# adajel/KNP-EMI-DG

Hardware: AMD Instinct MI355X
Metric: DoF-updates/sec per PDE timestep (higher is better)
Workload: dtype f64; 1 GPU; 3D idealized 4-axon mesh r=2 (995328 tets, 11943936 P1-DG DoFs: phi + K,Cl solved, Na eliminated), HH membranes + stimulus, full splitting step; parallelism=slab1

## Files before the change

### include/knpemi_hip.h

```cpp
#ifndef KNPEMI_HIP_H
#define KNPEMI_HIP_H
#include <stddef.h>
#include <stdint.h>

#ifdef __cplusplus
extern "C" {
#endif

typedef struct knp_ctx knp_ctx;

enum knp_field {
    KNP_F_PHI = 0,
    KNP_F_C = 1,
    KNP_F_C_PREV = 2,
    KNP_F_C_ELIM = 3,
    KNP_F_PHI_M = 4,
    KNP_F_I_CH = 5,
    KNP_F_E = 6,
    KNP_F_KAPPA = 7,
    KNP_F_DNPHI = 8,
    KNP_F_B_EMI = 9,
    KNP_F_B_KNP = 10,
    KNP_F_X = 11,
    KNP_F_Y = 12,
    KNP_F_FACET_TMP = 13,
    KNP_F_COUNT = 14
};

int knp_ctx_create(knp_ctx** out, int device, int dim, int degree, int n_ions,
                   int64_t nv, int64_t nc, int64_t nc_owned, int64_t nf,
                   const double* coords, const int32_t* cells, const uint32_t* cell_tags,
                   const int32_t* facet_cells, const int8_t* facet_local, const uint32_t* facet_tags,
                   int n_membrane_tags, const uint32_t* membrane_tags);
void knp_ctx_destroy(knp_ctx* ctx);
const char* knp_last_error(knp_ctx* ctx);

int knp_set_params(knp_ctx* ctx, double C_M, double dt, double F, double R, double T, double C_phi,
                   double tau_emi, double tau_knp, const double* z, const double* D, const double* rho,
                   const double* fsrc, int splitting);

int knp_set_geometry_classes(knp_ctx* ctx, int ncls, const uint16_t* cls, const double* table);

int knp_set_mms(knp_ctx* ctx, const double* C, const double* extra_emi, const double* extra_knp);

int knp_set_source(knp_ctx* ctx, const double* src);

enum knp_tab_slot {
    KNP_TAB_CELL_STIFF = 0,
    KNP_TAB_CELL_RHS_EMI = 1,
    KNP_TAB_CELL_MASS = 2,
    KNP_TAB_FACET_EMI = 3,
    KNP_TAB_FACET_MEM = 4,
    KNP_TAB_FACET_KNP = 5,
    KNP_TAB_FACET_RHS_EMI = 6,
    KNP_TAB_FACET_MEM_LIN = 7,
    KNP_TAB_FACET_MEM_KNP = 8,
    KNP_TAB_FACET_AVG = 9,
    KNP_TAB_FACET_NERNST = 10
};
int knp_set_tabulation(knp_ctx* ctx, int slot, int nloc, int nq, const double* w, const double* B, const double* dB);

int64_t knp_field_size(knp_ctx* ctx, int field);
int knp_upload(knp_ctx* ctx, int field, const double* src, int64_t offset, int64_t count);
int knp_download(knp_ctx* ctx, int field, double* dst, int64_t offset, int64_t count);
int knp_copy_field(knp_ctx* ctx, int dst_field, int src_field);

enum knp_debug_table_id {
    KNP_DT_CELLS = 0,
    KNP_DT_NBR = 1,
    KNP_DT_FLAG = 2,
    KNP_DT_CFACET = 3,
    KNP_DT_MF = 4,
    KNP_DT_HB_SRC = 5,
    KNP_DT_HB_LOC = 6,
    KNP_DT_META = 7
};
int64_t knp_debug_table_size(knp_ctx* ctx, int which);
int knp_debug_table(knp_ctx* ctx, int which, void* out, int64_t nbytes);

int knp_update_kappa(knp_ctx* ctx);
int knp_update_dnphi(knp_ctx* ctx);

int knp_emi_apply(knp_ctx* ctx, int fx, int fy);
int knp_knp_apply(knp_ctx* ctx, int fx, int fy);

int knp_emi_rhs(knp_ctx* ctx);
int knp_knp_rhs(knp_ctx* ctx);

int knp_emi_residual_target(knp_ctx* ctx, double r_abs);
int knp_knp_early_stop(knp_ctx* ctx, double factor);
int knp_knp_load_measure(knp_ctx* ctx, double* out);
int knp_emi_solve(knp_ctx* ctx, double rtol, double atol, int maxit, int check_every, int* niter, double* res);
int knp_knp_solve(knp_ctx* ctx, double rtol, double atol, int maxit, int min_it, int check_every, int* niter, double* res);
int knp_set_knp_krylov(knp_ctx* ctx, int method, int restart);
int knp_set_emi_dg_smoother(knp_ctx* ctx, int chebyshev);

int knp_amg_begin(knp_ctx* ctx, int which, int64_t ncg, const int32_t* dg2cg, const int32_t* cg_ptr, const int32_t* cg_idx);
int knp_amg_columns(knp_ctx* ctx, int which, int ncol);
int knp_amg_level(knp_ctx* ctx, int which, int64_t n, const int32_t* rowptrA, const int32_t* colA, const double* valA,
                  const double* dinv, double rho, int cheb_degree, double cheb_lower, int64_t ncoarse,
                  const int32_t* rowptrP, const int32_t* colP, const double* valP,
                  const int32_t* rowptrR, const int32_t* colR, const double* valR);
int knp_amg_finish(knp_ctx* ctx, int which, int64_t n, const double* pinv);
int knp_amg_finish_f32(knp_ctx* ctx, int which, int64_t n, const float* pinv);
int knp_amg_clear(knp_ctx* ctx, int which);
int knp_amg_interface(knp_ctx* ctx, int64_t n_local, int npeers, const int32_t* peers, const int64_t* counts, const int32_t* idx,
                      int64_t nuniq, const int32_t* uvtx, const int32_t* aptr, const int32_t* asrc);
int knp_amg_dist0(knp_ctx* ctx, int which);

int knp_step_updates(knp_ctx* ctx);
int knp_nernst(knp_ctx* ctx);
int knp_picard_updates(knp_ctx* ctx);
int knp_max_abs_diff(knp_ctx* ctx, int field_a, int field_b, double* out);
#define KNP_FACET_TMP_SLOTS 4
int knp_facet_trace(knp_ctx* ctx, int field, int species, int side, int slot);

int knp_rec_create(knp_ctx* ctx, int64_t capacity, int64_t n_points, const int32_t* point_cell, const double* point_w,
                   int64_t n_sets, const int64_t* set_ptr, const int32_t* set_facet, const double* set_w,
                   int n_regions, const uint8_t* region, const double* vol);
int knp_rec_sample(knp_ctx* ctx, double t);
int knp_rec_read(knp_ctx* ctx, int64_t* n_rows, double* t_out, double* rows_out);
int64_t knp_rec_channels(knp_ctx* ctx);
int knp_rec_add_states(knp_ctx* ctx, int64_t n_channels, const int64_t* chan_ptr, const int32_t* entry_handle, const int64_t* entry_row,
                       const int32_t* entry_col, const double* entry_w);
int knp_rec_add_map(knp_ctx* ctx, int64_t n, const int32_t* facets, double threshold, double repolarisation);
int knp_rec_map_arm(knp_ctx* ctx, double t0);
int knp_rec_map_read(knp_ctx* ctx, int64_t n, double* t_act, double* t_repol, double* peak, double* t_peak, int32_t* n_up);
int knp_rec_destroy(knp_ctx* ctx);
// ... 10 lines not shown
int64_t knp_state_describe(knp_ctx* ctx, knp_state_block* out, int64_t cap, int64_t* bytes);
int knp_state_save(knp_ctx* ctx, void* host_buf, size_t bytes);
int knp_state_load(knp_ctx* ctx, const void* host_buf, size_t bytes);
int knp_state_timing(knp_ctx* ctx, float* pack_ms, float* copy_ms);

int knp_ode_create(knp_ctx* ctx, int model, int64_t n, const int32_t* facets, int ns, int np, const double* states,
                   const double* params);
int knp_ode_table(knp_ctx* ctx, int handle, int what, int upload, double* host);
int knp_ode_exchange(knp_ctx* ctx, int handle, int what, int col, int field, int64_t offset, int to_facet);
int knp_ode_exchange_multi(knp_ctx* ctx, int handle, int n, const int32_t* what, const int32_t* col, const int32_t* field,
                           const int64_t* offset, int to_facet);
int knp_ode_set_stimulus(knp_ctx* ctx, int handle, int n_entries, const int32_t* cols, const double* values, const uint8_t* mask);
int knp_ode_step(knp_ctx* ctx, int handle, double t0, double dt, double rtol, double atol);
int knp_ode_rtc_compile(const char* src, const char* name, void** code, size_t* size, char* log, size_t logcap);
void knp_ode_rtc_free(void* code);
int knp_ode_register(knp_ctx* ctx, const void* code, size_t size, const char* kernel_name, int ns, int np);

int knp_host_spgemm(int64_t n, int64_t m, const int32_t* Ap, const int32_t* Aj, const double* Ax, const int32_t* Bp, const int32_t* Bj,
                    const double* Bx, int32_t* Cp, int32_t** Cj, double** Cx, int nthreads);
int knp_host_spmv(int64_t n, const int32_t* Ap, const int32_t* Aj, const double* Ax, const double* x, double* y, int nthreads);
void knp_host_free(void* p);
int knp_host_cell_gram(int64_t nc, int dim, const double* coords, const int32_t* cells, double* vol, double* G, int nthreads);
int knp_host_segment_sum(int64_t nseg, const int64_t* starts, const int64_t* order, const double* src, double* out, int nthreads);
int64_t knp_host_build_facets(int64_t nc, int nv, const int32_t* cells, int32_t* cell_facets, int32_t* facets, int32_t* facet_cells,
                              int8_t* facet_local);
int64_t knp_host_geometry_classes(int64_t nc, const double* coords, const int32_t* cells, const int32_t* nbr, const int8_t* nbj, double quantum,
                                  int64_t max_classes, int32_t* cls, int64_t* first, int nthreads);
int knp_host_block_pattern(int64_t nc, int nd, int64_t n, const int32_t* dof, int64_t* order, int64_t* starts, int32_t* cols, int32_t* indptr,
                           int64_t* nseg, int nthreads);
int knp_host_sym_to_f32(int64_t n, const double* a, float* out, double* maxabs, int nthreads);
int64_t knp_host_mis2_aggregate(int64_t n, const int32_t* indptr, const int32_t* indices, const double* key, int64_t* agg, int nthreads);
int knp_host_morton_order(int64_t n, int d, const double* pts, const int32_t* conn, int nv, const double* scale, int64_t* order, int nthreads);
int knp_host_cell_extent_median(int64_t nc, int nv, int d, const double* coords, const int32_t* cells, double* out);
int knp_host_cell_neighbours(int64_t nc, int nv, const int32_t* cell_facets, const int32_t* facet_cells, const int8_t* facet_local, int32_t* nb,
                             int8_t* nj, int nthreads);
int knp_host_box_marks(int64_t n, int d, const double* coords, const int32_t* conn, int nv, const double* a, const double* b, double eps, int mode,
                       uint8_t* out, int nthreads);
int knp_host_strength(int64_t n, const int32_t* Ap, const int32_t* Aj, const double* Ax, const double* diag, double theta, int32_t* Sp, int32_t** Sj,
                      int nthreads);
int knp_host_smooth_prolongator(int64_t n, int64_t m, const int32_t* Ap, const int32_t* Aj, const double* Ax, const double* v, const int32_t* Pp,
                                const int32_t* Pj, const double* Px, int32_t* Cp, int32_t** Cj, double** Cx, int nthreads);
int knp_host_truncate_prolongator(int64_t n, const int32_t* Pp, const int32_t* Pj, const double* Px, double trunc, const double* Bc, int32_t* Tp,
                                  int32_t** Tj, double** Tx, int nthreads);

int knp_sync(knp_ctx* ctx);
int knp_timer_begin(knp_ctx* ctx);
int knp_timer_end(knp_ctx* ctx, float* ms);
int knp_bench_apply(knp_ctx* ctx, int which, int reps, float* avg_ms);
int knp_apply_timing(knp_ctx* ctx, int enable);
int knp_apply_timing_read(knp_ctx* ctx, int which, float* avg_ms, int* count);

int knp_apply_variant(knp_ctx* ctx, int which);

int knp_probe_facet_contraction(knp_ctx* ctx, int variant, int64_t ncol, int reps, const double* in, double* out, float* avg_ms);

int knp_comm_unique_id(char* out128);
int knp_comm_init(knp_ctx* ctx, int rank, int nranks, const char* id128);
int knp_comm_init_halo(knp_ctx* ctx, const char* id128);
int knp_comm_init_shm(knp_ctx* ctx, int rank, int nranks, const char* name, int64_t red_doubles, int64_t out_doubles);
int knp_set_interior(knp_ctx* ctx, int64_t n_interior);
int knp_halo_tables(knp_ctx* ctx, int npeers, const int32_t* peers, const int64_t* send_counts,
                    const int32_t* send_cells, const int64_t* recv_offsets, const int64_t* recv_counts);
int knp_halo_exchange(knp_ctx* ctx, int field);
int knp_allreduce_sum(knp_ctx* ctx, double* values, int n);

#ifdef __cplusplus
}
#endif
#endif
```

### knp-emi-dg_amd/csrc/abi.hip

```cpp
#include "../../include/knpemi_hip.h"
#include "knpemi_internal.hpp"
#include <chrono>
#include <thread>
#include <cstdio>
#include <cstdlib>
#include "krylov.hpp"
#include <cstring>
#include <unordered_map>
#include <algorithm>
#include <cmath>

namespace {

struct Fields {
    double* f[KNP_F_COUNT] = {nullptr};
    int64_t n[KNP_F_COUNT] = {0};
    bjreal *binv_emi = nullptr, *binv_knp = nullptr;
    double *r = nullptr, *z = nullptr, *p = nullptr, *w = nullptr, *rhat = nullptr, *v = nullptr, *y = nullptr;
    double *hist_emi = nullptr, *hist_knp = nullptr;
    int bj_age_emi = 0, bj_age_knp = 0;
    double* tmp_knp = nullptr;
    double bj_lmax_knp = 0.0;
    int bj_lmax_age = 0;
    int it_ref_knp = 0, it_ref_emi = 0;
// ... 252 lines not shown
    stamp("mesh tables on the device");
    if (dim == 3 && degree == 1 && nc_owned > 0 && nc < (int64_t(1) << 29)) {
        const int64_t B = KNP_HALO_BLK, nblk = (nc_owned + B - 1) / B;
        std::vector<int32_t> hcnt(nblk, 0);
        std::vector<std::vector<int32_t>> lists((size_t)nblk);
        std::vector<uint16_t> hloc((size_t)nc_owned * 4, 0);
        int hmax = 0;
        for (int64_t b = 0; b < nblk; ++b) {
            auto& L = lists[(size_t)b];
            for (int64_t k = b * B; k < std::min(nc_owned, (b + 1) * B); ++k)
                for (int a = 0; a < 4; ++a) {
                    const uint32_t kind = (fb[k * 4 + a] >> 2) & 3u;
                    const int64_t nbk = nbr[k * 4 + a];
                    if ((kind != FK_SIPG && kind != FK_MEMBRANE) || nbk < 0) continue;
                    if (nbk / B == b) { hloc[k * 4 + a] = (uint16_t)(nbk - b * B); continue; }
                    hloc[k * 4 + a] = (uint16_t)(B + L.size());
                    L.push_back((int32_t)(nbk * 4 + (fb[k * 4 + a] & 3u)));
                }
            hmax = std::max(hmax, (int)L.size());
        }
        int64_t long0 = nblk;
        for (int64_t b = 0; b < nblk; ++b)
            if ((int64_t)lists[(size_t)b].size() > B) { long0 = b; break; }
        hmax = 0;
        for (int64_t b = 0; b < long0; ++b) hmax = std::max(hmax, (int)lists[(size_t)b].size());
        const int hs = ((hmax + 7) / 8) * 8;
        if (hs > 0 && long0 > 0) {
            std::vector<int32_t> hsrc((size_t)nblk * hs, -1);
            for (int64_t b = 0; b < long0; ++b) std::copy(lists[(size_t)b].begin(), lists[(size_t)b].end(), hsrc.begin() + b * hs);
            rc |= dev_alloc_copy(c, &m.hb_src, hsrc.data(), hsrc.size());
            rc |= dev_alloc_copy(c, &m.hb_loc, hloc.data(), hloc.size());
            rc |= dev_zeros(c, &c->halo_ctr, KNP_HALO_CTR_INTS);
            m.hb_stride = hs;
            m.hb_long0 = long0;
        }
    }
    if (rc) { g_err = c->err; delete c; return -2; }
    stamp("halo lists");

    Fields* fl = new Fields();
    const int64_t ndof = nc * ND, ns = c->p.n_sys;
    const int64_t sizes[KNP_F_COUNT] = {ndof, ns * ndof, ns * ndof, ndof, nf, n_ions * nf, n_ions * nf, ndof, ndof,
                                        ndof, ns * ndof, ns * ndof, ns * ndof, (int64_t)KNP_FACET_TMP_SLOTS * nf};
    for (int i = 0; i < KNP_F_COUNT; ++i) {
        fl->n[i] = sizes[i];
        rc |= dev_zeros(c, &fl->f[i], sizes[i]);
    }
    rc |= dev_zeros(c, &fl->binv_emi, ndof * ND);
    rc |= dev_zeros(c, &fl->binv_knp, ns * ndof * ND);
    double** wk[] = {&fl->r, &fl->z, &fl->p, &fl->w, &fl->rhat, &fl->v, &fl->y};
    for (auto pp : wk) rc |= dev_zeros(c, pp, ns * ndof);
    rc |= dev_zeros(c, &c->D, (size_t)n_ions * nc);
    rc |= dev_zeros(c, &c->rho, nc);
    c->partial_blocks = grid_for(nc_owned) + 8;
    rc |= dev_zeros(c, &c->partial, (size_t)c->partial_blocks * KNP_MAX_SYS * KNP_MAX_RED);
    rc |= dev_zeros(c, &c->scal, KNP_SCAL_DOUBLES);
    if (!rc && hipMalloc((void**)&c->status, sizeof(int) * KNP_STATUS_WORDS) != hipSuccess) rc = -2;
    if (!rc) hipMemset(c->status, 0, sizeof(int) * KNP_STATUS_WORDS);
    if (!rc && hipHostMalloc(&c->pinned, 4096) != hipSuccess) rc = -2;
    if (rc) { g_err = "device allocation failed: " + c->err; delete fl; delete c; return -2; }
    if (dev_alloc_copy(c, &fl->ivol, ivol.data(), ivol.size())) { g_err = "device allocation failed: " + c->err; delete fl; delete c; return -2; }
    g_fields[c] = fl;
    *out = c;
    stamp("fields allocated");
    return 0;
}

void knp_ctx_destroy(knp_ctx* c) {
    if (!c) return;
    hipSetDevice(c->device);
    hipDeviceSynchronize();
    for (auto& H : c->amg) amg_free(H);
    for (auto st : c->aux_streams) hipStreamDestroy(st);
    for (auto ev : c->aux_events) hipEventDestroy(ev);
    if (c->fork_event) hipEventDestroy(c->fork_event);
    ode_destroy_all(c);
    rec_destroy(c);
    state_destroy(c);
    tab_free(c);
    Fields* fl = g_fields[c];
    if (fl) {
        for (int i = 0; i < KNP_F_COUNT; ++i) hipFree(fl->f[i]);
        hipFree(fl->binv_emi); hipFree(fl->binv_knp); hipFree(fl->bj_idx); hipFree(fl->bj_tab); hipFree(fl->ivol);
        double* wk[] = {fl->r, fl->z, fl->p, fl->w, fl->rhat, fl->v, fl->y, fl->hist_emi, fl->hist_knp, fl->tmp_knp, fl->tmp_emi};
        for (auto p : wk) hipFree(p);
        delete fl;
        g_fields.erase(c);
    }
    ring_u_free(c);
    hipFree(c->m.hb_src); hipFree(c->m.hb_loc);
    hipFree(c->m.cls); hipFree(c->m.cls_table); hipFree(c->m.cls_ext); hipFree(c->m.coords); hipFree(c->m.h); hipFree(c->m.cells); hipFree(c->m.nbr); hipFree(c->m.fflag); hipFree(c->m.cfacet); hipFree(c->m.mf);
    hipFree(c->mat); hipFree(c->nmat4); hipFree(c->dtab); hipFree(c->halo_ctr);
    hipFree(c->D); hipFree(c->rho); hipFree(c->fsrc); hipFree(c->mms_C); hipFree(c->extra_emi); hipFree(c->extra_knp); hipFree(c->partial); hipFree(c->scal); hipFree(c->status); hipFree(c->gm_V);
    hipFree(c->halo_send_idx); hipFree(c->halo_sendbuf);
    if (c->pinned) hipHostFree(c->pinned);
    if (c->ev0) hipEventDestroy(c->ev0);
    if (c->ev1) hipEventDestroy(c->ev1);

    for (int w = 0; w < 2; ++w)
        for (auto& pr : c->tev[w]) { hipEventDestroy(pr.first); hipEventDestroy(pr.second); }
    comm_destroy(c);
    if (c->stream) hipStreamDestroy(c->stream);
    delete c;
}

int knp_set_params(knp_ctx* c, double C_M, double dt, double Fc, double R, double T, double C_phi, double tau_emi,
                   double tau_knp, const double* z, const double* D, const double* rho, const double* fsrc, int splitting) {
    if (!c || !z || !D) return -1;
    Params& p = c->p;
    p.C_M = C_M; p.dt = dt; p.F = Fc; p.R = R; p.T = T; p.C_phi = C_phi; p.psi = Fc / (R * T);
    p.tau_emi = tau_emi; p.tau_knp = tau_knp; p.splitting = splitting;
    if (splitting == 2 && !c->mms_C) { c->err = "MMS mode needs knp_set_mms first"; return -1; }
    if (g_fields.count(c)) reset_lagged(F(c));
    for (int i = 0; i < p.n_ions; ++i) {
        p.z[i] = z[i];
        if (z[i] == 0.0) { c->err = "ion valence z must be non-zero"; return -1; }
    }
    if (!(dt > 0.0)) { c->err = "dt must be positive"; return -1; }
    HIPCHK(c, hipMemcpy(c->D, D, sizeof(double) * p.n_ions * c->m.nc, hipMemcpyHostToDevice));
    if (g_fields.count(c)) F(c)->bj_tab_state = 0;
    {
        const int64_t nc = c->m.nc;
        const int ni = p.n_ions;
        c->h_mat.assign((size_t)nc, 0);
        std::vector<double> seen;
        bool ok = true;
        for (int64_t k = 0; k < nc && ok; ++k) {
            const int nm = (int)(seen.size() / ni);
            int id = -1;
            for (int q = nm - 1; q >= 0 && id < 0; --q) {
                bool same = true;
                for (int i = 0; i < ni && same; ++i) same = seen[(size_t)q * ni + i] == D[(int64_t)i * nc + k];
                if (same) id = q;
            }
            if (id < 0) {
                if (nm >= 256) { ok = false; break; }
                for (int i = 0; i < ni; ++i) seen.push_back(D[(int64_t)i * nc + k]);
                id = nm;
            }
            c->h_mat[(size_t)k] = (uint16_t)id;
        }
        if (!ok) c->h_mat.clear();
    }
    c->nmat = 0;
    if (c->m.dim == 3 && c->degree == 1 && c->m.hb_stride) {
        const int64_t nc = c->m.nc;
// ... 90 lines not shown
    c->m.ncls = ncls;
    return 0;
}

int knp_set_source(knp_ctx* c, const double* src) {
    if (!c) return -1;
    if (c->p.splitting == 2) { c->err = "knp_set_source: the manufactured-solution mode sets its own data terms"; return -1; }
    const int64_t n = (int64_t)c->p.n_sys * c->m.nc * c->nd;
    if (!src) {
        hipFree(c->extra_knp);
        c->extra_knp = nullptr;
        return 0;
    }
    if (!c->extra_knp) HIPCHK(c, hipMalloc((void**)&c->extra_knp, sizeof(double) * n));
    HIPCHK(c, hipMemcpy(c->extra_knp, src, sizeof(double) * n, hipMemcpyHostToDevice));
    return 0;
}

int knp_set_mms(knp_ctx* c, const double* C, const double* extra_emi, const double* extra_knp) {
    if (!c) return -1;
    const int64_t ndof = c->m.nc * c->nd, ns = c->p.n_sys;
    hipFree(c->mms_C); hipFree(c->extra_emi); hipFree(c->extra_knp);
    c->mms_C = c->extra_emi = c->extra_knp = nullptr;
    if (C) {
        HIPCHK(c, hipMalloc((void**)&c->mms_C, sizeof(double) * ns * c->m.nc));
        HIPCHK(c, hipMemcpy(c->mms_C, C, sizeof(double) * ns * c->m.nc, hipMemcpyHostToDevice));
    }
    if (extra_emi) {
        HIPCHK(c, hipMalloc((void**)&c->extra_emi, sizeof(double) * ndof));
        HIPCHK(c, hipMemcpy(c->extra_emi, extra_emi, sizeof(double) * ndof, hipMemcpyHostToDevice));
    }
    if (extra_knp) {
        HIPCHK(c, hipMalloc((void**)&c->extra_knp, sizeof(double) * ns * ndof));
        HIPCHK(c, hipMemcpy(c->extra_knp, extra_knp, sizeof(double) * ns * ndof, hipMemcpyHostToDevice));
    }
    return 0;
}

int64_t knp_field_size(knp_ctx* c, int field) { return chk_field(c, field) ? -1 : F(c)->n[field]; }

static int64_t debug_table_ptr(knp_ctx* c, int which, const void** p) {
    const MeshDev& m = c->m;
    const int64_t NV = m.dim + 1;
    const int64_t nblk = (m.nc_owned + KNP_HALO_BLK - 1) / KNP_HALO_BLK;
    switch (which) {
        case KNP_DT_CELLS: *p = m.cells; return m.nc * NV * 4;
        case KNP_DT_NBR: *p = m.nbr; return m.nc * NV * 4;
        case KNP_DT_FLAG: *p = m.fflag; return m.nc * 4;
        case KNP_DT_CFACET: *p = m.cfacet; return m.nc * NV * 4;
        case KNP_DT_MF: *p = m.mf; return m.nmf * 6 * 4;
        case KNP_DT_HB_SRC: *p = m.hb_src; return m.hb_src ? nblk * m.hb_stride * 4 : 0;
        case KNP_DT_HB_LOC: *p = m.hb_loc; return m.hb_loc ? m.nc_owned * 4 * 2 : 0;
        case KNP_DT_META: *p = nullptr; return 8 * 8;
        default: return -1;
    }
}
int64_t knp_debug_table_size(knp_ctx* c, int which) {
    const void* p = nullptr;
    return c ? debug_table_ptr(c, which, &p) : -1;
}
int knp_debug_table(knp_ctx* c, int which, void* out, int64_t nbytes) {
    if (!c) return -1;
    const void* p = nullptr;
    const int64_t n = debug_table_ptr(c, which, &p);
    if (n < 0 || nbytes != n || (n && !out)) { c->err = "debug_table: unknown table or size mismatch"; return -1; }
    if (which == KNP_DT_META) {
        const int64_t meta[8] = {c->m.nc, c->m.nc_owned, c->m.nf, c->m.nmf, c->m.hb_stride, c->m.hb_long0, c->m.n_interior, c->m.dim};
        memcpy(out, meta, sizeof(meta));
        return 0;
    }
    if (n) HIPCHK(c, hipMemcpy(out, p, (size_t)n, hipMemcpyDeviceToHost));
    return 0;
}

int knp_upload(knp_ctx* c, int field, const double* src, int64_t offset, int64_t count) {
    if (chk_field(c, field)) return -1;
    if (offset < 0 || count < 0 || offset + count > F(c)->n[field]) { c->err = "upload range out of bounds"; return -1; }
    HIPCHK(c, hipMemcpyAsync(F(c)->f[field] + offset, src, sizeof(double) * count, hipMemcpyHostToDevice, c->stream));
    HIPCHK(c, hipStreamSynchronize(c->stream));
    if (field == KNP_F_C || field == KNP_F_C_ELIM || field == KNP_F_PHI || field == KNP_F_KAPPA) reset_lagged(F(c));
    if (field == KNP_F_PHI) { F(c)->nh_emi = 0; c->last_peclet = -1.0f; }
    if (field == KNP_F_C) F(c)->nh_knp = 0;
    return 0;
}

int knp_download(knp_ctx* c, int field, double* dst, int64_t offset, int64_t count) {
    if (chk_field(c, field)) return -1;
    if (offset < 0 || count < 0 || offset + count > F(c)->n[field]) { c->err = "download range out of bounds"; return -1; }
    HIPCHK(c, hipMemcpyAsync(dst, F(c)->f[field] + offset, sizeof(double) * count, hipMemcpyDeviceToHost, c->stream));
    HIPCHK(c, hipStreamSynchronize(c->stream));
    return 0;
}

int knp_copy_field(knp_ctx* c, int dst, int src) {
    if (chk_field(c, dst) || chk_field(c, src)) return -1;
    if (F(c)->n[dst] != F(c)->n[src]) { c->err = "copy_field: size mismatch"; return -1; }
    HIPCHK(c, hipMemcpyAsync(F(c)->f[dst], F(c)->f[src], sizeof(double) * F(c)->n[src], hipMemcpyDeviceToDevice, c->stream));
    return 0;
}

int knp_update_kappa(knp_ctx* c) {
    if (!c) return -1;
    Fields* f = F(c);
    return launch_kappa(c, f->f[KNP_F_C], f->f[KNP_F_C_ELIM], f->f[KNP_F_KAPPA]);
}

// ... 6 lines not shown
        pe = (float)(scale * (hi - lo));
        if (!(pe >= 0.0f)) pe = 3.0e38f;
    }
#pragma unroll
    for (int off = 32; off > 0; off >>= 1) pe = fmaxf(pe, __shfl_down(pe, off, 64));
    __shared__ float s_pe[4];
    if ((threadIdx.x & 63) == 0) s_pe[threadIdx.x >> 6] = pe;
    __syncthreads();
    if (threadIdx.x == 0) {
        pe = fmaxf(fmaxf(s_pe[0], s_pe[1]), fmaxf(s_pe[2], s_pe[3]));
        const int bits = __float_as_int(pe);
        if (bits > __atomic_load_n(out, __ATOMIC_RELAXED)) atomicMax(out, bits);
    }
}

int knp_update_dnphi(knp_ctx* c) {
    if (!c) return -1;
    Fields* f = F(c);
    double zmax = 0.0;
    for (int i = 0; i < c->p.n_sys; ++i) zmax = std::max(zmax, std::fabs(c->p.z[i]));
    HIPCHK(c, hipMemsetAsync(c->status + KNP_PECLET_SLOT, 0, sizeof(int), c->stream));
    if (c->m.nc_owned)
        hipLaunchKernelGGL(k_cell_peclet, dim3((unsigned)((c->m.nc_owned + 255) / 256)), dim3(256), 0, c->stream, c->m.nc_owned, c->nd,
                           (const double*)f->f[KNP_F_PHI], c->p.psi * zmax, c->status + KNP_PECLET_SLOT);
    HIPCHK(c, hipGetLastError());
    if (c->dist) { int rc = allreduce_max_word(c, c->status + KNP_PECLET_SLOT); if (rc) return rc; }
    return launch_dnphi(c, f->f[KNP_F_PHI], f->f[KNP_F_DNPHI]);
}

int knp_allreduce_sum(knp_ctx* c, double* values, int n) {
    if (!c || !values) return -1;
    return allreduce_sum_host(c, values, n);
}

static int chk_vec(knp_ctx* c, int fx, int fy, int64_t need) {
    if (chk_field(c, fx) || chk_field(c, fy)) return -1;
    if (fx == fy) { c->err = "apply: input and output fields must differ"; return -1; }
    if (F(c)->n[fx] < need || F(c)->n[fy] < need) { c->err = "apply: field too small for this operator"; return -1; }
    return 0;
}

int knp_emi_apply(knp_ctx* c, int fx, int fy) {
    if (!c) return -1;
    if (chk_vec(c, fx, fy, c->m.nc * c->nd)) return -1;
    Fields* f = F(c);
    return dist_apply(c, 0, f->f[fx], f->f[KNP_F_KAPPA], f->f[fy]);
}

int knp_knp_apply(knp_ctx* c, int fx, int fy) {
    if (!c) return -1;
    if (chk_vec(c, fx, fy, (int64_t)c->p.n_sys * c->m.nc * c->nd)) return -1;
    Fields* f = F(c);
    return dist_apply(c, 1, f->f[fx], f->f[KNP_F_DNPHI], f->f[fy]);
}

int knp_emi_rhs(knp_ctx* c) {
    if (!c) return -1;
    Fields* f = F(c);
    return launch_emi_rhs(c, f->f[KNP_F_C], f->f[KNP_F_C_ELIM], f->f[KNP_F_PHI_M], f->f[KNP_F_I_CH], f->f[KNP_F_B_EMI]);
}

int knp_knp_rhs(knp_ctx* c) {
    if (!c) return -1;
    Fields* f = F(c);
    return launch_knp_rhs(c, f->f[KNP_F_C], f->f[KNP_F_C_PREV], f->f[KNP_F_C_ELIM], f->f[KNP_F_PHI], f->f[KNP_F_PHI_M],
                          f->f[KNP_F_I_CH], f->f[KNP_F_B_KNP]);
}

int knp_emi_residual_target(knp_ctx* c, double r_abs) {
    if (!c || !(r_abs >= 0.0)) return -1;
    F(c)->emi_r_abs = r_abs;
    return 0;
}

int knp_knp_early_stop(knp_ctx* c, double factor) {
    if (!c || !(factor >= 0.0) || factor >= 1.0) { if (c) c->err = "knp_knp_early_stop: factor must be in [0, 1)"; return -1; }
    c->knp_early = factor;
    return 0;
}

int knp_knp_load_measure(knp_ctx* c, double* out) {
    if (!c || !out) return -1;
    Fields* f = F(c);
    const bool d8 = env_int("KNP_KNP_NORM2", 0) != 1;
    return load_measure(c, f->f[KNP_F_B_KNP], f->ivol, d8, out);
}

int knp_emi_solve(knp_ctx* c, double rtol, double atol, int maxit, int check_every, int* niter, double* res) {
    if (!c || !niter || !res) return -1;
    Fields* f = F(c);
    static const int bj_lag = env_int("KNP_BJ_LAG", 8);
    int rc = 0;
    if (f->bj_age_emi % (bj_lag > 0 ? bj_lag : 1) == 0) rc = launch_emi_blockjacobi(c, f->f[KNP_F_KAPPA], f->binv_emi);
    ++f->bj_age_emi;
    if (rc) return rc;
    if ((rc = extrapolate_guess(c, f->f[KNP_F_PHI], &f->hist_emi, &f->nh_emi, f->n[KNP_F_PHI], true))) return rc;
    KrylovVecs kv{};
    kv.x = f->f[KNP_F_PHI]; kv.b = f->f[KNP_F_B_EMI]; kv.coef = f->f[KNP_F_KAPPA]; kv.binv = f->binv_emi;
    kv.ivol = f->ivol; kv.r_abs = f->emi_r_abs;
    kv.d8 = env_int("KNP_KNP_NORM2", 0) != 1;
    kv.r = f->r; kv.z = f->z; kv.p = f->p; kv.w = f->w; kv.rhat = f->rhat; kv.v = f->v; kv.y = f->y;
    static const int cheb_env_emi = env_int("KNP_EMI_CHEB", -1);
    const int cheb_emi = cheb_env_emi >= 0 ? cheb_env_emi : (c->emi_dg_cheb >= 0 ? c->emi_dg_cheb : (c->degree == 1 ? 1 : 0));
    if (cheb_emi && c->amg.size() && c->amg[0].ready) {
        if (!f->tmp_emi) HIPCHK(c, hipMalloc((void**)&f->tmp_emi, sizeof(double) * f->n[KNP_F_PHI]));
        kv.tmp = f->tmp_emi;
// ... 357 lines not shown
```

### knp-emi-dg_amd/csrc/apply_p1.hip

```cpp
#include "apply_p1_direct.hpp"
#include "apply_p1_cls.hpp"
#include "apply_p1_halo.hpp"
#include "apply_plan.hpp"

static_assert(APPLY_PLAN_BLK == KNP_HALO_BLK, "the plan counts head cells in blocks of the halo tables");

static inline int64_t grid8(int64_t n) { return ((grid_for(n) + 7) / 8) * 8; }

struct ApplyTimerScope {
    knp_ctx* c; int which; bool on;
    ApplyTimerScope(knp_ctx* ctx, int w) : c(ctx), which(w), on(ctx->time_applies) {
        if (!on) return;
        auto& pool = c->tev[which];
        if (c->tev_used[which] == pool.size()) {
            hipEvent_t a, b;
            if (hipEventCreate(&a) != hipSuccess || hipEventCreate(&b) != hipSuccess) { on = false; return; }
            pool.push_back({a, b});
        }
        hipEventRecord(pool[c->tev_used[which]].first, c->stream);
    }
    ~ApplyTimerScope() {
        if (!on) return;
        hipEventRecord(c->tev[which][c->tev_used[which]].second, c->stream);
        ++c->tev_used[which];
// ... 42 lines not shown
            case AF_RING_U: rc = ring_u_emi_apply(c, m, x, kappa, y, halo_reserve_cus(c)); break;
            case AF_CLS:
                hipLaunchKernelGGL((k_emi_apply_cls_staged<3, 256>), g, dim3(KNP_BLOCK), 0, c->stream, m, x, kappa, y, c->p.C_phi, c->p.tau_emi);
                HIPCHK(c, hipGetLastError());
                break;
            default: DISPATCH_DIM(c, k_emi_apply, g, m, x, kappa, y, c->p.C_phi, c->p.tau_emi);
        }
        if (rc) return rc;
    }
    return 0;
}

int launch_knp_apply(knp_ctx* c, const double* x, const double* gphi, double* y) {
    ApplyTimerScope t(c, 1);
    if (c->degree != 1) return p2_assembled(c) ? tab_apply(c, 1, x, y) : p2_knp_apply(c, x, gphi, y);
    if (c->m.c_end - c->m.c_begin <= 0) return 0;
    const KnpArgs ka = make_knp_args(c);
    size_t halo_lds = 0;
    const ApplyInputs in = apply_inputs(c, 1, &halo_lds);
    ApplySegment seg[2];
    const int nseg = apply_segments(plan_apply(in, 1), c->m.c_begin, c->m.c_end, seg);
    for (int i = 0; i < nseg; ++i) {
        MeshDev m = c->m;
        m.c_begin = seg[i].begin; m.c_end = seg[i].end;
        const dim3 g((unsigned)grid8(m.c_end - m.c_begin)), b(KNP_BLOCK);
        int rc = 0;
        switch (seg[i].family) {
            case AF_RING_KNP: rc = ring_knp_apply(c, m, x, gphi, y, ka, halo_reserve_cus(c)); break;
            case AF_RING_U: rc = ring_u_knp_apply(c, m, x, gphi, y, ka, halo_reserve_cus(c)); break;
            case AF_HALO:
            case AF_HALO_MAT: rc = knp_halo_launch(c, m, x, gphi, y, ka, halo_lds, in.halo_mat, halo_reserve_cus(c)); break;
            case AF_CLS:
                dispatch_nsys<3>(c->p.n_sys, [&](auto ns) {
                    hipLaunchKernelGGL((k_knp_apply_cls_staged<3, decltype(ns)::value, 256>), g, b, 0, c->stream, m, x, gphi, c->D, y, ka);
                    return 0;
                });
                HIPCHK(c, hipGetLastError());
                break;
            default:
                rc = dispatch_nsys<4>(c->p.n_sys, [&](auto ns) {
                    constexpr int NS = decltype(ns)::value;
                    if (c->m.dim == 3) hipLaunchKernelGGL((k_knp_apply<3, NS>), g, b, 0, c->stream, m, x, gphi, c->D, y, ka);
                    else hipLaunchKernelGGL((k_knp_apply<2, NS>), g, b, 0, c->stream, m, x, gphi, c->D, y, ka);
                    return 0;
                });
                if (rc) { c->err = "knp_apply supports 1..4 solved species"; return -1; }
                HIPCHK(c, hipGetLastError());
        }
        if (rc) return rc;
    }
    return 0;
}

int launch_emi_blockjacobi(knp_ctx* c, const double* kappa, bjreal* binv) {
    if (c->degree != 1) return p2_assembled(c) ? tab_block_inverse(c, 0, binv) : p2_block_inverse(c, 0, kappa, binv);
    const double shift = 0.0;
    DISPATCH_DIM(c, k_emi_blockjacobi, dim3((unsigned)grid_for(c->m.nc_owned)), c->m, kappa, binv, c->p.C_phi, c->p.tau_emi, shift);
    return 0;
}

int launch_knp_blockjacobi(knp_ctx* c, const double* gphi, bjreal* binv) {
    if (c->degree != 1) return p2_assembled(c) ? tab_block_inverse(c, 1, binv) : p2_block_inverse(c, 1, gphi, binv);
    const dim3 g((unsigned)grid_for(c->m.nc_owned), (unsigned)c->p.n_sys);
    DISPATCH_DIM(c, k_knp_blockjacobi, g, c->m, gphi, c->D, binv, make_knp_args(c));
    return 0;
}

int launch_neighbour_materials(knp_ctx* c) {
    const int64_t n = c->m.nc * 4;
    hipLaunchKernelGGL(k_neighbour_materials, dim3((unsigned)((n + 255) / 256)), dim3(256), 0, c->stream, c->m.nc, c->m.nbr, c->mat, c->nmat4);
    HIPCHK(c, hipGetLastError());
    HIPCHK(c, hipStreamSynchronize(c->stream));
    return 0;
}

int launch_dnphi(knp_ctx* c, const double* phi, double* gphi) {
    if (c->degree != 1) {
        if (p2_assembled(c)) return tab_assemble_knp(c, phi);
        HIPCHK(c, hipMemcpyAsync(gphi, phi, sizeof(double) * c->m.nc * c->nd, hipMemcpyDeviceToDevice, c->stream));
        return 0;
    }
    DISPATCH_DIM(c, k_gphi, dim3((unsigned)grid_for(c->m.nc)), c->m, phi, gphi);
    return 0;
}
```

### knp-emi-dg_amd/csrc/apply_plan.hpp

```cpp
#pragma once
#include <algorithm>
#include <cstdint>

enum ApplyFamily : int {
    AF_COORD = 0,
    AF_CLS = 1,
    AF_HALO = 2,
    AF_RING_EMI = 3,
    AF_HALO_MAT = 6,
    AF_RING_KNP = 7,
    AF_P2 = 8,
    AF_P2_ASSEMBLED = 9,
    AF_RING_U = 10
};

constexpr int64_t APPLY_PLAN_BLK = 256;
constexpr int64_t APPLY_ALL_CELLS = INT64_MAX;

struct ApplyInputs {
    int degree = 1, dim = 3;
    bool p2_assembled = false;
    bool cls = false;
    int ncls = 0, ncls_max = 0;
    int n_sys = 1;
    int64_t hb_long0 = 0;
    bool ring = false;
    int64_t ring_u_cells = 0;
    bool halo = false, halo_mat = false;
};

struct ApplyPlan { ApplyFamily head; int64_t head_cells; ApplyFamily tail; };

inline ApplyPlan plan_apply(const ApplyInputs& in, int which) {
    if (in.degree != 1) {
        const ApplyFamily f = in.p2_assembled ? AF_P2_ASSEMBLED : AF_P2;
        return {f, APPLY_ALL_CELLS, f};
    }
    const bool classed = in.dim == 3 && in.cls && in.ncls <= in.ncls_max && (which == 0 || in.n_sys <= 3);
    const ApplyFamily tail = classed ? AF_CLS : AF_COORD;
    const int64_t short_list_cells = in.hb_long0 * APPLY_PLAN_BLK;
    if (in.ring) return {which == 1 ? AF_RING_KNP : AF_RING_EMI, short_list_cells, tail};
    if (in.ring_u_cells > 0) return {AF_RING_U, in.ring_u_cells, tail};
    if (which == 1 && in.halo) return {in.halo_mat ? AF_HALO_MAT : AF_HALO, short_list_cells, tail};
    return {tail, APPLY_ALL_CELLS, tail};
}

struct ApplySegment { ApplyFamily family; int64_t begin, end; };

inline int apply_segments(const ApplyPlan& p, int64_t begin, int64_t end, ApplySegment seg[2]) {
    int n = 0;
    if (begin < end && begin < p.head_cells) {
        seg[n++] = {p.head, begin, std::min(end, p.head_cells)};
        begin = seg[0].end;
    }
    if (begin < end) seg[n++] = {p.tail, begin, end};
    return n;
}
```

### knp-emi-dg_amd/csrc/apply_ring.hip

```cpp
#include "cell_geom.hpp"
#include "ring_common.hpp"
#include <algorithm>
#include <cstdlib>
#include <map>

namespace {

using namespace ring;
constexpr int RH = 224;
constexpr int RHX = RH / 32;
constexpr int RENT = RB + RH;
constexpr int RSLOTS = 3;
constexpr int RLISTB = 1024;
constexpr int RNLIST = 4;
constexpr int RLOADERS = 4;
constexpr int META_F = 0, META_L = 1024, META_N = 3072, META_C = 4096, META_M = 5120, META_KNP = 6144, META_EMI = 5120;
constexpr int RCLS = 43;

__device__ __forceinline__ void dma_list(const MeshDev& m, int64_t b, unsigned dst, int lane) {
    const int off = lane * 4 < m.hb_stride ? lane * 4 : 0;
    glds16(m.hb_src + b * m.hb_stride + off, dst);
}
__device__ __forceinline__ void class_gram(const lds_double* rec, CellGeom<3>& K) {
    K.vol = rec[0];
    int q = 1;
#pragma unroll
    for (int a = 0; a < 4; ++a)
#pragma unroll
        for (int b = a; b < 4; ++b) { K.G[a][b] = rec[q]; K.G[b][a] = rec[q]; ++q; }
}

template <int NS> struct KnpRing {
    static constexpr int XB = RENT * 32;
    static constexpr int G0 = NS * XB;
    static constexpr int GH0 = G0 + RB * 32;
    static constexpr int META0 = GH0 + 4096;
    static constexpr int SLOT = META0 + META_KNP;
    static constexpr int NDATA = NS * 8 + NS * RHX + 8 + 4 + 6;
    static_assert(NDATA <= 63, "vmcnt is a 6-bit counter");
};

template <int NS, int I>
__device__ __forceinline__ void knp_facet_ring(const CellGeom<3>& K, uint32_t flags, unsigned loc, unsigned dsel, const double (*xv)[4],
                                               const double (*gx)[4], const double* gp, const double* Dk, const double* hvD,
                                               const double* zpsi, double tau,
                                               const lds_double* X, const lds_double* G, const lds_double* sD, const lds_double* ft,
                                               double (*y)[4]) {
    constexpr int D = 3, NV = 4;
    const uint32_t fb = (flags >> (8 * I)) & 0xffu;
    if (((fb >> 2) & 3u) != FK_SIPG) return;
    const unsigned j = fb & 3u;
    const double gr = ft[8 * I], pen_geo = ft[8 * I + 4], nLI_DV = ft[8 * I + 5];
    double cf[D];
#pragma unroll
// ... 11 lines not shown
    const double up_nb = fmax(-gp_nb, 0.0) * nLI_DV;
    const double penA = tau * pen_geo;
    const double hv = 0.5 * K.vol;
#pragma unroll
    for (int k = 0; k < NS; ++k) {
        double xr[NV], xf[D];
        lds_row(X + (unsigned)k * (RENT * NV), loc, xr);
        const double xap = pick_apex<D>(xr, (int)j);
#pragma unroll
        for (int mm = 0; mm < D; ++mm) xf[mm] = pick_facet<D>(xr, mm, (int)j);
        const double Dn = sD[(unsigned)k * KNP_MAX_MAT + dsel];
        const double s_own = gx[k][I];
        double s_nb = xap * gr;
#pragma unroll
        for (int mm = 0; mm < D; ++mm) s_nb = fma(xf[mm], cf[mm], s_nb);
        const double zp = zpsi[k];
        const double c_own = Dk[k] * fma(-zp, up_own, penA);
        const double c_nb = Dn * fma(-zp, up_nb, penA);
        double sdu = 0.0, w[D], sw = 0.0;
#pragma unroll
        for (int mm = 0; mm < D; ++mm) {
            const double xo = xv[k][mm + (mm >= I)];
            sdu += xo - xf[mm];
            w[mm] = fma(c_own, xo, -c_nb * xf[mm]);
            sw += w[mm];
        }
        const double t1m = fma(FacetConst<D>::mass, sw, hv * fma(Dk[k], s_own, Dn * s_nb));
        const double t2 = hvD[k] * sdu;
#pragma unroll
        for (int a = 0; a < NV; ++a) y[k][a] = fma(K.G[a][I], t2, y[k][a]);
#pragma unroll
        for (int mm = 0; mm < D; ++mm) y[k][mm + (mm >= I)] += fma(FacetConst<D>::mass, w[mm], t1m);
    }
}

struct CellMeta { uint32_t flags, nm; uint2 lw; unsigned cls, mymat; };
typedef __attribute__((address_space(3))) uint32_t lds_u32;
typedef __attribute__((address_space(3))) uint16_t lds_u16;
typedef __attribute__((address_space(3))) uint8_t lds_u8;
__device__ __forceinline__ CellMeta read_meta(const char* meta, unsigned t, bool knp) {
    CellMeta q;
    q.flags = ((const lds_u32*)(meta + META_F))[t];
    q.lw.x = ((const lds_u32*)(meta + META_L))[2 * t];
    q.lw.y = ((const lds_u32*)(meta + META_L))[2 * t + 1];
    q.cls = ((const lds_u16*)(meta + META_C))[t];
    q.nm = 0; q.mymat = 0;
    if (knp) {
        q.nm = ((const lds_u32*)(meta + META_N))[t];
        q.mymat = ((const lds_u8*)(meta + META_M))[t];
    }
    return q;
}

template <int NS, int NG>
__global__ __launch_bounds__(RB * NG + 64 * RLOADERS) void k_knp_apply_ring(MeshDev m, const double* __restrict__ x, const double* __restrict__ gphi,
                                                                 double* __restrict__ yout, KnpArgs ka, const uint8_t* __restrict__ mat,
                                                                 const uint8_t* __restrict__ nmat4, const double* __restrict__ dtab, int dbg) {
    typedef KnpRing<NS> R;
    constexpr int NV = 4, KS = NS / NG, NTHREADS = RB * NG + 64 * RLOADERS;
    static_assert(KS * NG == NS, "species split evenly over the consumer groups");
    extern __shared__ __attribute__((aligned(16))) char smem[];
    char* s_list = smem + RSLOTS * R::SLOT;
    double* s_cls = reinterpret_cast<double*>(s_list + RNLIST * RLISTB);
    double* s_D = s_cls + m.ncls * RCLS;
    const unsigned base = __builtin_amdgcn_readfirstlane((unsigned)(size_t)(lds_char*)smem);
    const unsigned list0 = base + RSLOTS * R::SLOT;
    const int wave = __builtin_amdgcn_readfirstlane((int)(threadIdx.x >> 6));
    const int lane = threadIdx.x & 63;
    const RingWalk w(m);
    if (w.blk(0) < 0) return;
    for (int i = threadIdx.x; i < m.ncls * 11; i += NTHREADS) s_cls[(i / 11) * RCLS + (i % 11)] = m.cls_table[(i / 11) * KNP_CLS_STRIDE + (i % 11)];
    for (int i = threadIdx.x; i < m.ncls * KNP_CLS_EXT; i += NTHREADS) s_cls[(i / KNP_CLS_EXT) * RCLS + 11 + (i % KNP_CLS_EXT)] = m.cls_ext[i];
    if (threadIdx.x < NS * KNP_MAX_MAT) s_D[threadIdx.x] = dtab[threadIdx.x];
    if (wave >= 4 * NG) {
        const int lw = wave - 4 * NG;
        constexpr int N0 = 8 + 3, N1 = (NS > 1 ? 8 : 0) + 3, N2 = 8 + 4, N3 = NS * RHX;
        auto list_dma = [&](int64_t n) {
            const int64_t b = w.blk(n);
            if (lw == 0 && b >= 0) dma_list(m, b, list0 + (unsigned)(n & (RNLIST - 1)) * RLISTB, lane);
        };
        auto data_dma = [&](int64_t n) {
            const int64_t b = w.blk(n);
            if (dbg & 4) return;
            const unsigned slot = base + (unsigned)(n % RSLOTS) * R::SLOT;
            const lds_int* L = (const lds_int*)(s_list + (n & (RNLIST - 1)) * RLISTB);
            const int64_t c0 = b * RB;
            if (lw == 0) {
                dma_own_rows(x, c0, m.nc, slot, lane);
                glds16(m.fflag + c0 + 4 * lane, slot + R::META0 + META_F);
                glds16(m.hb_loc + (c0 + 2 * lane) * 4, slot + R::META0 + META_L);
                glds16(m.hb_loc + (c0 + 128 + 2 * lane) * 4, slot + R::META0 + META_L + 1024);
            } else if (lw == 1) {
                if (NS > 1) dma_own_rows(x + m.nc * NV, c0, m.nc, slot + R::XB, lane);
                glds16(m.cls + c0 + 8 * lane, slot + R::META0 + META_C);
                glds16(nmat4 + (c0 + 4 * lane) * 4, slot + R::META0 + META_N);
                glds16(mat + c0 + 16 * lane, slot + R::META0 + META_M);
            } else if (lw == 2) {
                dma_own_rows(gphi, c0, m.nc, slot + R::G0, lane);
#pragma unroll
                for (int p = 0; p < 4; ++p) {
                    const int e = p * 64 + lane;
                    const int src = e < m.hb_stride ? L[e] : -1;
                    int64_t Kp = src >= 0 ? (int64_t)(src >> 2) : 0;
                    const int j = src >= 0 ? (src & 3) : 0;
                    if (dbg & 1) Kp = c0 + e < m.nc ? c0 + e : 0;
                    glds16(gphi + Kp * NV + (j >> 1) * 2, slot + R::GH0 + p * 1024);
                }
            } else {
#pragma unroll
                for (int p = 0; p < RHX; ++p) {
                    int64_t Kp = list_cell(L, p * 32 + (lane >> 1), m.hb_stride);
                    if (dbg & 1) Kp = c0 + p * 32 + (lane >> 1) < m.nc ? c0 + p * 32 + (lane >> 1) : 0;
#pragma unroll
                    for (int k = 0; k < NS; ++k) glds16(x + (int64_t)k * m.nc * NV + Kp * NV + swz_half(lane), slot + k * R::XB + RB * 32 + p * 1024);
                }
            }
        };
        auto wait_older = [&]() {
            if (lw == 0) wait_vm<N0>(); else if (lw == 1) wait_vm<N1>(); else if (lw == 2) wait_vm<N2>(); else wait_vm<N3>();
        };
        list_dma(0); list_dma(1);
        wait_vm<0>();
        ring_barrier();
        data_dma(0);
        list_dma(2);
        if (w.blk(1) >= 0) { data_dma(1); wait_older(); } else wait_vm<0>();
        ring_barrier();
        for (int64_t n = 0; w.blk(n) >= 0; ++n) {
            list_dma(n + 3);
            if (w.blk(n + 2) >= 0) { data_dma(n + 2); wait_older(); }
            else wait_vm<0>();
            ring_barrier();
        }
        return;
    }
    const unsigned t = threadIdx.x & (RB - 1);
    const int k0 = (wave >> 2) * KS;
    double zpsi[KS];
#pragma unroll
    for (int k = 0; k < KS; ++k) zpsi[k] = ka.z[k0 + k] * ka.psi;
    ring_barrier();
    ring_barrier();
    for (int64_t n = 0;; ++n) {
        const int64_t b = w.blk(n);
        if (b < 0) break;
        const int64_t c = b * RB + t;
        if (c >= m.c_begin && c < m.c_end) {
            const char* slot = smem + (n % RSLOTS) * R::SLOT;
            const CellMeta cur = read_meta(slot + R::META0, t, true);
            const lds_double* X = (const lds_double*)slot + k0 * (RENT * NV);
            const lds_double* G = (const lds_double*)(slot + R::G0);
            const lds_double* rec = TO_LDS(s_cls) + cur.cls * RCLS;
            const lds_double* sD = TO_LDS(s_D) + k0 * KNP_MAX_MAT;
            CellGeom<3> K;
            class_gram(rec, K);
            double xv[KS][NV], y[KS][NV], gp[NV], Dk[KS];
            lds_row(G, t, gp);
#pragma unroll
            for (int k = 0; k < KS; ++k) {
                lds_row(X + k * (RENT * NV), t, xv[k]);
                Dk[k] = sD[k * KNP_MAX_MAT + cur.mymat];
            }
            const double mw = ka.inv_dt * K.vol / 20.0;
            double gx[KS][NV], hvD[KS];
#pragma unroll
            for (int k = 0; k < KS; ++k) hvD[k] = 0.5 * K.vol * Dk[k];
#pragma unroll
            for (int k = 0; k < KS; ++k) {
                double sx = 0.0;
#pragma unroll
                for (int a = 0; a < NV; ++a) sx += xv[k][a];
                const double drift = zpsi[k] * Dk[k] * K.vol * sx / (double)NV;
                const double dv = Dk[k] * K.vol;
#pragma unroll
                for (int a = 0; a < NV; ++a) {
                    double sacc = 0.0;
#pragma unroll
                    for (int bb = 0; bb < NV; ++bb) sacc = fma(xv[k][bb], K.G[bb][a], sacc);
                    gx[k][a] = sacc;
                    y[k][a] = fma(mw, sx + xv[k][a], fma(dv, sacc, drift * gp[a]));
                }
            }
            const lds_double* ft = rec + 11;
            if (!(dbg & 2)) {
            knp_facet_ring<KS, 0>(K, cur.flags, cur.lw.x & 0xffffu, cur.nm & 0xffu, xv, gx, gp, Dk, hvD, zpsi, ka.tau, X, G, sD, ft, y);
            knp_facet_ring<KS, 1>(K, cur.flags, cur.lw.x >> 16, (cur.nm >> 8) & 0xffu, xv, gx, gp, Dk, hvD, zpsi, ka.tau, X, G, sD, ft, y);
            knp_facet_ring<KS, 2>(K, cur.flags, cur.lw.y & 0xffffu, (cur.nm >> 16) & 0xffu, xv, gx, gp, Dk, hvD, zpsi, ka.tau, X, G, sD, ft, y);
            knp_facet_ring<KS, 3>(K, cur.flags, cur.lw.y >> 16, cur.nm >> 24, xv, gx, gp, Dk, hvD, zpsi, ka.tau, X, G, sD, ft, y);
            }
#pragma unroll
            for (int k = 0; k < KS; ++k) store_nodal<3>(yout + (int64_t)(k0 + k) * m.nc * NV, c, y[k]);
        }
        ring_barrier();
    }
}

struct EmiRing {
    static constexpr int XB = RENT * 32;
    static constexpr int META0 = 2 * XB;
    static constexpr int SLOT = META0 + META_EMI;
    static constexpr int NDATA = 8 + 8 + 2 * RHX + 4;
};

template <int I>
__device__ __forceinline__ void emi_facet_ring(const CellGeom<3>& K, uint32_t flags, unsigned loc, const double* xv, const double* gx,
                                               const double* kv, double C_phi, double tau, const lds_double* X, const lds_double* KA,
                                               const lds_double* ft, double* y) {
    constexpr int D = 3, NV = 4;
    const uint32_t fb = (flags >> (8 * I)) & 0xffu;
    const uint32_t kind = (fb >> 2) & 3u;
    if (kind >= FK_EXTERIOR) return;
    const unsigned j = fb & 3u;
    double xr[NV], kr[NV], xf[D], knf[D];
    lds_row(X, loc, xr);
    lds_row(KA, loc, kr);
    const double xap = pick_apex<D>(xr, (int)j);
#pragma unroll
    for (int mm = 0; mm < D; ++mm) {
        xf[mm] = pick_facet<D>(xr, mm, (int)j);
        knf[mm] = pick_facet<D>(kr, mm, (int)j);
    }
    double du[D], sdu = 0.0;
#pragma unroll
    for (int mm = 0; mm < D; ++mm) {
        du[mm] = xv[mm + (mm >= I)] - xf[mm];
        sdu += du[mm];
    }
    const double sqG_DV = ft[8 * I + 6];
    if (kind == FK_MEMBRANE) {
        const double w = C_phi * sqG_DV * FacetConst<D>::mass;
#pragma unroll
        for (int mm = 0; mm < D; ++mm) y[mm + (mm >= I)] = fma(w, sdu + du[mm], y[mm + (mm >= I)]);
        return;
    }
    const double gr = ft[8 * I];
    const double s_own = gx[I];
    double s_nb = xap * gr;
#pragma unroll
    for (int mm = 0; mm < D; ++mm) s_nb = fma(xf[mm], ft[8 * I + 1 + mm], s_nb);
    double kf[D], sk = 0.0, skn = 0.0, q = 0.0;
#pragma unroll
    for (int mm = 0; mm < D; ++mm) {
        kf[mm] = kv[mm + (mm >= I)];
        sk += kf[mm];
        skn += knf[mm];
        q = fma(kf[mm], sdu + du[mm], q);
    }
    const double hm = 0.5 * (double)D * K.vol * FacetConst<D>::mass;
    q *= hm;
#pragma unroll
    for (int a = 0; a < NV; ++a) y[a] = fma(K.G[a][I], q, y[a]);
    const double pw = tau * ft[8 * I + 4] * FacetConst<D>::trip;
    double kb[D], skb = 0.0, skd = 0.0;
#pragma unroll
    for (int mm = 0; mm < D; ++mm) {
        kb[mm] = 0.5 * (kf[mm] + knf[mm]);
        skb += kb[mm];
        skd = fma(kb[mm], du[mm], skd);
    }
    const double bs = fma(skb, sdu, skd);
#pragma unroll
    for (int mm = 0; mm < D; ++mm) {
        const double t1 = hm * fma(s_own, sk + kf[mm], s_nb * (skn + knf[mm]));
        const double t3 = pw * (bs + fma(kb[mm], sdu, du[mm] * fma(2.0, kb[mm], skb)));
        y[mm + (mm >= I)] += t1 + t3;
    }
}

constexpr int EMI_SLOTS = 4;
__global__ __launch_bounds__(2 * RB + 64 * RLOADERS) void k_emi_apply_ring(MeshDev m, const double* __restrict__ x, const double* __restrict__ kappa,
                                                                double* __restrict__ yout, double C_phi, double tau) {
    typedef EmiRing R;
    constexpr int NV = 4, NTHREADS = 2 * RB + 64 * RLOADERS;
    extern __shared__ __attribute__((aligned(16))) char smem[];
    char* s_list = smem + EMI_SLOTS * R::SLOT;
    double* s_cls = reinterpret_cast<double*>(s_list + RNLIST * RLISTB);
    const unsigned base = __builtin_amdgcn_readfirstlane((unsigned)(size_t)(lds_char*)smem);
    const unsigned list0 = base + EMI_SLOTS * R::SLOT;
    const int wave = __builtin_amdgcn_readfirstlane((int)(threadIdx.x >> 6));
    const int lane = threadIdx.x & 63;
    const RingWalk w(m);
    if (w.blk(0) < 0) return;
    for (int i = threadIdx.x; i < m.ncls * 11; i += NTHREADS) s_cls[(i / 11) * RCLS + (i % 11)] = m.cls_table[(i / 11) * KNP_CLS_STRIDE + (i % 11)];
    for (int i = threadIdx.x; i < m.ncls * KNP_CLS_EXT; i += NTHREADS) s_cls[(i / KNP_CLS_EXT) * RCLS + 11 + (i % KNP_CLS_EXT)] = m.cls_ext[i];
    if (wave >= 8) {
        const int lw = wave - 8;
        constexpr int N0 = 8, N1 = 8, N2 = RHX + 2, N3 = RHX + 2;
        auto list_dma = [&](int64_t n) {
            const int64_t b = w.blk(n);
            if (lw == 0 && b >= 0) dma_list(m, b, list0 + (unsigned)(n & (RNLIST - 1)) * RLISTB, lane);
        };
        auto data_dma = [&](int64_t n) {
            const int64_t c0 = w.blk(n) * RB;
            const unsigned slot = base + (unsigned)(n & (EMI_SLOTS - 1)) * R::SLOT;
            const lds_int* L = (const lds_int*)(s_list + (n & (RNLIST - 1)) * RLISTB);
            if (lw == 0) dma_own_rows(x, c0, m.nc, slot, lane);
            else if (lw == 1) dma_own_rows(kappa, c0, m.nc, slot + R::XB, lane);
            else {
                const double* v = lw == 2 ? x : kappa;
                const unsigned dst = slot + (lw == 2 ? 0 : R::XB) + RB * 32;
#pragma unroll
                for (int p = 0; p < RHX; ++p) glds16(v + list_cell(L, p * 32 + (lane >> 1), m.hb_stride) * NV + swz_half(lane), dst + p * 1024);
                if (lw == 2) {
                    glds16(m.fflag + c0 + 4 * lane, slot + R::META0 + META_F);
                    glds16(m.cls + c0 + 8 * lane, slot + R::META0 + META_C);
                } else {
                    glds16(m.hb_loc + (c0 + 2 * lane) * 4, slot + R::META0 + META_L);
                    glds16(m.hb_loc + (c0 + 128 + 2 * lane) * 4, slot + R::META0 + META_L + 1024);
                }
            }
        };
        auto wait_older = [&]() {
            if (lw == 0) wait_vm<N0>(); else if (lw == 1) wait_vm<N1>(); else if (lw == 2) wait_vm<N2>(); else wait_vm<N3>();
        };
        list_dma(0); list_dma(1);
        wait_vm<0>();
        ring_barrier();
        data_dma(0);
        list_dma(2);
        if (w.blk(1) >= 0) { data_dma(1); wait_older(); } else wait_vm<0>();
        ring_barrier();
        for (int64_t n = 0;; ++n) {
            if (w.blk(n) < 0) { wait_vm<0>(); ring_barrier(); break; }
            list_dma(n + 3);
            if (w.blk(n + 2) >= 0) { data_dma(n + 2); wait_older(); }
            else wait_vm<0>();
            ring_barrier();
        }
        return;
    }
    const unsigned t = threadIdx.x & (RB - 1);
    const int g = wave >> 2;
    ring_barrier();
    ring_barrier();
    CellGeom<3> K;
    double xv[NV], kv[NV], yv[NV], gx[NV];
    const lds_double *X = nullptr, *KA = nullptr, *ft = nullptr;
    CellMeta cur;
    cur.flags = 0; cur.lw = make_uint2(0u, 0u); cur.cls = 0; cur.nm = 0; cur.mymat = 0;
    int64_t ccur = -1;
    bool valid = false;
    for (int64_t n = 0;; ++n) {
        const int64_t b = w.blk(n);
        if ((n & 1) == g) {
            if (b >= 0) {
                ccur = b * RB + t;
                valid = ccur >= m.c_begin && ccur < m.c_end;
                if (valid) {
                    const char* slot = smem + (n & (EMI_SLOTS - 1)) * R::SLOT;
                    cur = read_meta(slot + R::META0, t, false);
                    X = (const lds_double*)slot;
                    KA = (const lds_double*)(slot + R::XB);
                    const lds_double* rec = TO_LDS(s_cls) + cur.cls * RCLS;
                    ft = rec + 11;
                    class_gram(rec, K);
                    lds_row(X, t, xv);
                    lds_row(KA, t, kv);
                    double kbar = 0.0;
#pragma unroll
                    for (int a = 0; a < NV; ++a) kbar += kv[a];
                    kbar *= K.vol / (double)NV;
#pragma unroll
                    for (int a = 0; a < NV; ++a) {
                        double sa = 0.0;
#pragma unroll
                        for (int bb = 0; bb < NV; ++bb) sa = fma(xv[bb], K.G[bb][a], sa);
                        gx[a] = sa;
                        yv[a] = kbar * sa;
                    }
                    emi_facet_ring<0>(K, cur.flags, cur.lw.x & 0xffffu, xv, gx, kv, C_phi, tau, X, KA, ft, yv);
                    emi_facet_ring<1>(K, cur.flags, cur.lw.x >> 16, xv, gx, kv, C_phi, tau, X, KA, ft, yv);
                }
            }
        } else if (n >= 1 && valid) {
            emi_facet_ring<2>(K, cur.flags, cur.lw.y & 0xffffu, xv, gx, kv, C_phi, tau, X, KA, ft, yv);
            emi_facet_ring<3>(K, cur.flags, cur.lw.y >> 16, xv, gx, kv, C_phi, tau, X, KA, ft, yv);
            store_nodal<3>(yout, ccur, yv);
        }
        ring_barrier();
        if (b < 0) break;
    }
}

}

static size_t ring_lds_bytes(const knp_ctx* c, int which) {
    const size_t tables = RNLIST * RLISTB + sizeof(double) * (size_t)c->m.ncls * RCLS;
    if (which == 0) return (size_t)EMI_SLOTS * EmiRing::SLOT + tables;
    const size_t slot = c->p.n_sys == 1 ? KnpRing<1>::SLOT : KnpRing<2>::SLOT;
    return (size_t)RSLOTS * slot + tables + sizeof(double) * (size_t)c->p.n_sys * KNP_MAX_MAT;
}

bool ring_usable(const knp_ctx* c, int which) {
    if (c->degree != 1 || c->m.dim != 3 || !c->m.cls || c->m.ncls > CLS_MAX_LDS || !c->m.hb_src || c->m.hb_stride <= 0 || c->m.hb_stride > RH) return false;
    if (env_int("KNP_APPLY_RING", 1) == 0 || ring_lds_bytes(c, which) > RING_MAX_LDS) return false;
    if (which == 0) return env_int("KNP_EMI_RING", 1) != 0;
    return c->nmat > 0 && c->p.n_sys <= 2 && env_int("KNP_APPLY_MAT", 1) != 0 && env_int("KNP_APPLY_HALO", 1) != 0;
}

int ring_emi_apply(knp_ctx* c, const MeshDev& m, const double* x, const double* kappa, double* y, int reserve_cus) {
    const size_t lds = ring_lds_bytes(c, 0);
    if (!grant_lds(k_emi_apply_ring, lds)) { c->err = "hipFuncSetAttribute(k_emi_apply_ring) failed"; return -2; }
    hipLaunchKernelGGL(k_emi_apply_ring, ring_grid(m, c->device, reserve_cus), dim3(2 * RB + 64 * RLOADERS), lds, c->stream, m, x, kappa, y, c->p.C_phi, c->p.tau_emi);
    HIPCHK(c, hipGetLastError());
    return 0;
}

int ring_knp_apply(knp_ctx* c, const MeshDev& m, const double* x, const double* gphi, double* y, const KnpArgs& ka, int reserve_cus) {
    const int ns = c->p.n_sys;
    const size_t lds = ring_lds_bytes(c, 1);
    const dim3 g = ring_grid(m, c->device, reserve_cus);
    const bool split = ns == 2 && env_int("KNP_RING_SPLIT", 0) != 0;
#define RING_KNP_LAUNCH(NS_, NG_)                                                                                                     \
    do {                                                                                                                              \
        if (!grant_lds(k_knp_apply_ring<NS_, NG_>, lds)) { c->err = "hipFuncSetAttribute(k_knp_apply_ring) failed"; return -2; }  \
        hipLaunchKernelGGL((k_knp_apply_ring<NS_, NG_>), g, dim3(RB * NG_ + 64 * RLOADERS), lds, c->stream, m, x, gphi, y, ka, (const uint8_t*)c->mat,  \
                           (const uint8_t*)c->nmat4, (const double*)c->dtab, env_int("KNP_RING_DEBUG", 0));                     \
    } while (0)
    if (ns == 1) RING_KNP_LAUNCH(1, 1);
    else if (split) RING_KNP_LAUNCH(2, 2);
    else RING_KNP_LAUNCH(2, 1);
#undef RING_KNP_LAUNCH
    HIPCHK(c, hipGetLastError());
    return 0;
}
```

### knp-emi-dg_amd/csrc/cell_geom.hpp

```cpp
#pragma once
#include "knpemi_internal.hpp"

__device__ __forceinline__ double fast_rcp(double x) {
    double r = __builtin_amdgcn_rcp(x);
    r = fma(fma(-x, r, 1.0), r, r);
    r = fma(fma(-x, r, 1.0), r, r);
    return r;
}
__device__ __forceinline__ double fast_sqrt(double x) {
    double r = __builtin_amdgcn_rsq(x);
    double g = x * r, h = 0.5 * r;
    double e = fma(-h, g, 0.5);
    g = fma(g, e, g);
    h = fma(h, e, h);
    e = fma(-h, g, 0.5);
    g = fma(g, e, g);
    h = fma(h, e, h);
    g = fma(fma(-g, g, x), h, g);
    return g;
}

template <int D> struct CellGeom {
    static constexpr int NV = D + 1;
    double X0[D];
    double g[NV][D];
    double G[NV][NV];
    double vol;
};

template <int D> __device__ __forceinline__ void load_vertex(const double* __restrict__ coords, int v, double* out);
template <> __device__ __forceinline__ void load_vertex<3>(const double* __restrict__ coords, int v, double* out) {
    const double2 a = *reinterpret_cast<const double2*>(coords + 4 * (int64_t)v);
    const double b = coords[4 * (int64_t)v + 2];
    out[0] = a.x; out[1] = a.y; out[2] = b;
}
template <> __device__ __forceinline__ void load_vertex<2>(const double* __restrict__ coords, int v, double* out) {
    const double2 a = *reinterpret_cast<const double2*>(coords + 2 * (int64_t)v);
    out[0] = a.x; out[1] = a.y;
}

template <int D> __device__ __forceinline__ double dotD(const double* a, const double* b) {
    double s = a[0] * b[0];
#pragma unroll
    for (int k = 1; k < D; ++k) s = fma(a[k], b[k], s);
    return s;
}

template <int D> __device__ __forceinline__ void load_nodal(const double* __restrict__ p, int64_t c, double* v);
template <> __device__ __forceinline__ void load_nodal<3>(const double* __restrict__ p, int64_t c, double* v) {
    const double2 a = *reinterpret_cast<const double2*>(p + 4 * c);
    const double2 b = *reinterpret_cast<const double2*>(p + 4 * c + 2);
    v[0] = a.x; v[1] = a.y; v[2] = b.x; v[3] = b.y;
}
template <> __device__ __forceinline__ void load_nodal<2>(const double* __restrict__ p, int64_t c, double* v) {
    v[0] = p[3 * c]; v[1] = p[3 * c + 1]; v[2] = p[3 * c + 2];
}
template <int D> __device__ __forceinline__ void store_nodal(double* __restrict__ p, int64_t c, const double* v);
template <> __device__ __forceinline__ void store_nodal<3>(double* __restrict__ p, int64_t c, const double* v) {
    *reinterpret_cast<double2*>(p + 4 * c) = make_double2(v[0], v[1]);
    *reinterpret_cast<double2*>(p + 4 * c + 2) = make_double2(v[2], v[3]);
}
template <> __device__ __forceinline__ void store_nodal<2>(double* __restrict__ p, int64_t c, const double* v) {
    p[3 * c] = v[0]; p[3 * c + 1] = v[1]; p[3 * c + 2] = v[2];
}

template <int D> __device__ __forceinline__ void load_cell_ints(const int32_t* __restrict__ p, int64_t c, int* v);
template <> __device__ __forceinline__ void load_cell_ints<3>(const int32_t* __restrict__ p, int64_t c, int* v) {
    const int4 a = *reinterpret_cast<const int4*>(p + 4 * c);
    v[0] = a.x; v[1] = a.y; v[2] = a.z; v[3] = a.w;
}
template <> __device__ __forceinline__ void load_cell_ints<2>(const int32_t* __restrict__ p, int64_t c, int* v) {
    v[0] = p[3 * c]; v[1] = p[3 * c + 1]; v[2] = p[3 * c + 2];
// ... 116 lines not shown
```

### knp-emi-dg_amd/csrc/comm.hip

```cpp
#include "../../include/knpemi_hip.h"
#include "knpemi_internal.hpp"
#include "krylov.hpp"
#include <rccl/rccl.h>
#include <atomic>
#include <chrono>
#include <cstring>
#include <cstdlib>
#include <fcntl.h>
#include <sched.h>
#include <sys/mman.h>
#include <unistd.h>

#define NCCLCHK(ctx, call)                                                         \
    do {                                                                           \
        ncclResult_t r_ = (call);                                                  \
        if (r_ != ncclSuccess) {                                                   \
            (ctx)->err = std::string(#call) + ": " + ncclGetErrorString(r_);       \
            return -6;                                                             \
        }                                                                          \
    } while (0)

static_assert(sizeof(ncclUniqueId) <= 128, "unique id must fit the ABI buffer");

static void shm_destroy(knp_ctx* c);
// ... 267 lines not shown
    delete s;
    c->shm = nullptr;
}

int halo_exchange(knp_ctx* c, double* v, int nfields) {
    if (!c->dist) return 0;
    if (c->shm) {
        if (nfields > KNP_MAX_SYS) { c->err = "halo exchange: too many fields"; return -1; }
        return shm_halo_exchange(c, v, nfields, c->stream);
    }
    if (c->halo_peer.empty()) return 0;
    if (!c->comm) { c->err = "halo exchange without communicator"; return -6; }
    return halo_exchange_on(c, v, nfields, c->stream, (ncclComm_t)c->comm);
}

int dist_apply(knp_ctx* c, int which, double* x, const double* coef, double* y) {
    auto launch = [&]() { return which == 0 ? launch_emi_apply(c, x, coef, y) : launch_knp_apply(c, x, coef, y); };
    if (!c->dist) {
        const char* fs = getenv("KNP_FORCE_SPLIT");
        if (!(fs && atoi(fs) == 1) || c->m.n_interior >= c->m.nc_owned) return launch();
        const int64_t n_own = c->m.nc_owned;
        c->m.c_begin = 0; c->m.c_end = c->m.n_interior;
        int rc = launch();
        c->m.c_begin = c->m.n_interior; c->m.c_end = n_own;
        if (!rc) rc = launch();
        c->m.c_begin = 0; c->m.c_end = n_own;
        return rc;
    }
    const int nfields = which == 0 ? 1 : c->p.n_sys;
    int rc;
    const bool overlap = c->halo_stream && (c->shm || (c->comm_halo && !c->halo_peer.empty()));
    if (!overlap) {
        if ((rc = halo_exchange(c, x, nfields))) return rc;
        return launch();
    }
    HIPCHK(c, hipEventRecord(c->halo_ready, c->stream));
    HIPCHK(c, hipStreamWaitEvent(c->halo_stream, c->halo_ready, 0));
    const int64_t n_own = c->m.nc_owned;
    c->m.c_begin = 0; c->m.c_end = c->m.n_interior;
    rc = launch();
    c->m.c_begin = 0; c->m.c_end = n_own;
    if (rc) return rc;
    if (c->shm) rc = shm_halo_exchange(c, x, nfields, c->halo_stream);
    else rc = halo_exchange_on(c, x, nfields, c->halo_stream, (ncclComm_t)c->comm_halo);
    if (rc) return rc;
    HIPCHK(c, hipEventRecord(c->halo_done, c->halo_stream));
    HIPCHK(c, hipStreamWaitEvent(c->stream, c->halo_done, 0));
    c->m.c_begin = c->m.n_interior; c->m.c_end = n_own;
    rc = launch();
    c->m.c_begin = 0; c->m.c_end = n_own;
    return rc;
}

static int halo_exchange_on(knp_ctx* c, double* v, int nfields, hipStream_t st, ncclComm_t comm) {
    if (nfields > KNP_MAX_SYS) { c->err = "halo exchange: too many fields"; return -1; }
    const int NV = c->nd;
    const int64_t stride = c->m.nc * NV;
    const int np = (int)c->halo_peer.size();
    for (int p = 0; p < np; ++p) {
        const int64_t cnt = c->halo_send_cnt[p];
        if (!cnt) continue;
        const int64_t n = cnt * NV;
        hipLaunchKernelGGL(k_halo_pack, dim3((unsigned)((n + 255) / 256)), dim3(256), 0, st, (const double*)v,
                           (const int32_t*)(c->halo_send_idx + c->halo_send_off[p]), cnt, nfields, stride, NV,
                           c->halo_sendbuf + c->halo_send_off[p] * KNP_MAX_SYS * NV);
    }
    HIPCHK(c, hipGetLastError());
    NCCLCHK(c, ncclGroupStart());
    for (int p = 0; p < np; ++p) {
        const int peer = c->halo_peer[p];
        for (int f = 0; f < nfields && c->halo_send_cnt[p]; ++f)
            NCCLCHK(c, ncclSend(c->halo_sendbuf + c->halo_send_off[p] * KNP_MAX_SYS * NV + (int64_t)f * c->halo_send_cnt[p] * NV,
                                (size_t)(c->halo_send_cnt[p] * NV), ncclDouble, peer, comm, st));
        for (int f = 0; f < nfields && c->halo_recv_cnt[p]; ++f)
            NCCLCHK(c, ncclRecv(v + (int64_t)f * stride + c->halo_recv_off[p] * NV, (size_t)(c->halo_recv_cnt[p] * NV), ncclDouble,
                                peer, comm, st));
    }
    NCCLCHK(c, ncclGroupEnd());
    return 0;
}

static hipError_t create_halo_stream(knp_ctx* c) {
    int lo = 0, hi = 0;
    if (hipDeviceGetStreamPriorityRange(&lo, &hi) != hipSuccess) { lo = hi = 0; }
    return hipStreamCreateWithPriority(&c->halo_stream, hipStreamNonBlocking, hi);
}

extern "C" {

int knp_comm_unique_id(char* out128) {
    if (!out128) return -1;
    ncclUniqueId id;
    if (ncclGetUniqueId(&id) != ncclSuccess) return -6;
    memset(out128, 0, 128);
    memcpy(out128, &id, sizeof(id));
    return 0;
}

int knp_comm_init(knp_ctx* c, int rank, int nranks, const char* id128) {
    if (!c || !id128 || nranks < 1 || rank < 0 || rank >= nranks) return -1;
    c->rank = rank;
    c->nranks = nranks;
    if (nranks == 1 && env_int("KNP_FORCE_COMM", 0) != 1) return 0;
    ncclUniqueId id;
    memcpy(&id, id128, sizeof(id));
    HIPCHK(c, hipSetDevice(c->device));
// ... 166 lines not shown
```

### knp-emi-dg_amd/csrc/knpemi_internal.hpp

```cpp
#pragma once
#include <hip/hip_runtime.h>
#include <cstdint>
#include <cstdlib>
#include <string>
#include <type_traits>
#include <vector>
#include <map>
#include "amg.hpp"

typedef float bjreal;

#define KNP_MAX_IONS 8
#define KNP_MAX_SYS 7
#define KNP_BLOCK 256
#define KNP_MAX_RED 8
#define KNP_ODE_FAIL_SLOT (2 * KNP_MAX_SYS)
#define KNP_PECLET_SLOT (2 * KNP_MAX_SYS + 1)
#define KNP_STATUS_WORDS (2 * KNP_MAX_SYS + 2)

enum : uint32_t { FK_SIPG = 0u, FK_MEMBRANE = 1u, FK_EXTERIOR = 2u, FK_INACTIVE = 3u };

struct MeshDev {
    int dim = 0;
    int64_t nv = 0, nc = 0, nc_owned = 0, nf = 0, nmf = 0;
// ... 63 lines not shown
    std::vector<uint8_t> h_mf_mask;
    int* halo_ctr = nullptr;
    int halo_flip[2] = {0, 0};
    double* rho = nullptr;
    double* fsrc = nullptr;
    double* mms_C = nullptr;
    double* extra_emi = nullptr;
    double* extra_knp = nullptr;
    TabRule tab[KNP_TAB_COUNT];
    double* tab_mem[KNP_TAB_COUNT] = {nullptr};
    double* blk_emi = nullptr;
    double* blk_knp = nullptr;
    std::map<int, double*> vecs;
    std::map<int, int64_t> vlen;
    int next_handle = 1;
    double* partial = nullptr;
    int64_t partial_blocks = 0;
    double* scal = nullptr;
    int* status = nullptr;
    void* pinned = nullptr;
    hipEvent_t ev0 = nullptr, ev1 = nullptr;
    int emi_dg_cheb = -1;
    int knp_krylov = 0;
    int gm_restart = 30;
    double* gm_V = nullptr;
    int gm_alloc = 0;
    int last_it_emi = 0, last_it_knp = 0;
    double knp_early = 0.0;
    float last_peclet = -1.0f;
    std::vector<AmgHierarchy> amg;
    std::vector<hipStream_t> aux_streams;
    std::vector<hipEvent_t> aux_events;
    hipEvent_t fork_event = nullptr;
    void* comm = nullptr;
    void* comm_halo = nullptr;
    void* shm = nullptr;
    hipStream_t halo_stream = nullptr;
    hipEvent_t halo_ready = nullptr, halo_done = nullptr;
    int rank = 0, nranks = 1;
    bool dist = false;
    std::vector<int> halo_peer;
    std::vector<int64_t> halo_send_off, halo_send_cnt, halo_recv_off, halo_recv_cnt;
    int32_t* halo_send_idx = nullptr;
    double* halo_sendbuf = nullptr;
    int64_t halo_send_total = 0;
    std::vector<int> if_peer;
    std::vector<int64_t> if_off, if_cnt;
    int64_t if_total = 0, if_nuniq = 0;
    int32_t* if_idx = nullptr;
    int32_t* if_uvtx = nullptr;
    int32_t* if_aptr = nullptr;
    int32_t* if_asrc = nullptr;
    double *if_send = nullptr, *if_recv = nullptr;
    bool time_applies = false;
    std::vector<std::pair<hipEvent_t, hipEvent_t>> tev[2];
    size_t tev_used[2] = {0, 0};
    std::string err;
};

#define HIPCHK(ctx, call)                                                        \
    do {                                                                         \
        hipError_t e_ = (call);                                                  \
        if (e_ != hipSuccess) {                                                  \
            (ctx)->err = std::string(#call) + ": " + hipGetErrorString(e_);      \
            return -2;                                                           \
        }                                                                        \
    } while (0)

struct KnpArgs {
    int ns;
    double inv_dt, psi, tau;
    double z[KNP_MAX_SYS];
};
template <int D> struct FacetConst;
template <> struct FacetConst<3> { static constexpr double mass = 1.0 / 12.0, trip = 1.0 / 60.0; };
template <> struct FacetConst<2> { static constexpr double mass = 1.0 / 6.0, trip = 1.0 / 24.0; };

inline int env_int(const char* name, int dflt) {
    const char* v = getenv(name);
    return v ? atoi(v) : dflt;
}
inline bool env_flag(const char* name, bool dflt) { return env_int(name, dflt ? 1 : 0) != 0; }

inline int64_t grid_for(int64_t n) { return (n + KNP_BLOCK - 1) / KNP_BLOCK; }

#define DISPATCH_DIM(c, KERN, grid, ...)                                                         \
    do {                                                                                         \
        if ((c)->m.dim == 3) hipLaunchKernelGGL(KERN<3>, grid, dim3(KNP_BLOCK), 0, (c)->stream, __VA_ARGS__); \
        else hipLaunchKernelGGL(KERN<2>, grid, dim3(KNP_BLOCK), 0, (c)->stream, __VA_ARGS__);    \
        HIPCHK(c, hipGetLastError());                                                            \
    } while (0)

template <int MAXNS, typename F> int dispatch_nsys(int n_sys, F&& f) {
    static_assert(MAXNS >= 1 && MAXNS <= 4, "instances exist for at most four solved species");
    if (n_sys == 1) return f(std::integral_constant<int, 1>());
    if constexpr (MAXNS >= 2) if (n_sys == 2) return f(std::integral_constant<int, 2>());
    if constexpr (MAXNS >= 3) if (n_sys == 3) return f(std::integral_constant<int, 3>());
    if constexpr (MAXNS >= 4) if (n_sys == 4) return f(std::integral_constant<int, 4>());
    return -1;
}

int launch_emi_apply(knp_ctx* c, const double* x, const double* kappa, double* y);
int launch_knp_apply(knp_ctx* c, const double* x, const double* dnphi, double* y);
int launch_emi_blockjacobi(knp_ctx* c, const double* kappa, bjreal* binv);
int launch_knp_blockjacobi(knp_ctx* c, const double* dnphi, bjreal* binv);
int launch_dnphi(knp_ctx* c, const double* phi, double* dnphi);
int launch_neighbour_materials(knp_ctx* c);
int apply_variant(knp_ctx* c, int which);
int launch_kappa(knp_ctx* c, const double* cc, const double* celim, double* kappa);
int launch_emi_rhs(knp_ctx* c, const double* cc, const double* celim, const double* phiM,
                   const double* Ich, double* b);
int launch_knp_rhs(knp_ctx* c, const double* cc, const double* cprev, const double* celim,
                   const double* phi, const double* phiM, const double* Ich, double* b);
int launch_step_updates(knp_ctx* c, const double* cc, double* celim, const double* phi,
                        double* phiM, double* E);
int launch_facet_trace(knp_ctx* c, const double* nodal, int side, double* out);

int tab_kappa(knp_ctx* c, const double* cc, const double* celim, double* kappa);
int tab_assemble_knp(knp_ctx* c, const double* phi);
int tab_apply(knp_ctx* c, int which, const double* x, double* y);
int tab_block_inverse(knp_ctx* c, int which, bjreal* binv);
int tab_emi_rhs(knp_ctx* c, const double* cc, const double* celim, const double* phiM, const double* Ich, double* b);
int tab_knp_rhs(knp_ctx* c, const double* cc, const double* cprev, const double* celim, const double* phi, const double* phiM,
                const double* Ich, double* b);
int tab_step_updates(knp_ctx* c, const double* cc, double* celim, const double* phi, double* phiM, double* E, bool do_celim);
int tab_facet_trace(knp_ctx* c, const double* nodal, int side, double* out);
void tab_free(knp_ctx* c);
inline bool p2_assembled(const knp_ctx* c) { return c->p2_assembled; }

bool ring_usable(const knp_ctx* c, int which);
int64_t ring_u_cells(knp_ctx* c, int which);
void ring_u_free(knp_ctx* c);
int ring_u_emi_apply(knp_ctx* c, const MeshDev& m, const double* x, const double* kappa, double* y, int reserve_cus);
int ring_u_knp_apply(knp_ctx* c, const MeshDev& m, const double* x, const double* gphi, double* y, const KnpArgs& ka, int reserve_cus);
int ring_emi_apply(knp_ctx* c, const MeshDev& m, const double* x, const double* kappa, double* y, int reserve_cus);
int ring_knp_apply(knp_ctx* c, const MeshDev& m, const double* x, const double* gphi, double* y, const KnpArgs& ka, int reserve_cus);

int p2_emi_apply(knp_ctx* c, const double* x, const double* kappa, double* y);
int p2_knp_apply(knp_ctx* c, const double* x, const double* phi, double* y);
int p2_block_inverse(knp_ctx* c, int which, const double* coef, bjreal* binv);

int halo_exchange(knp_ctx* c, double* v, int nfields);
int dist_apply(knp_ctx* c, int which, double* x, const double* coef, double* y);

int launch_nernst_only(knp_ctx* c, const double* cc, const double* celim, double* E);
void comm_destroy(knp_ctx* c);
int allreduce_red(knp_ctx* c, double* red, int count);
int allreduce_max(knp_ctx* c, double* host_value);
int allreduce_max_word(knp_ctx* c, int* dev_word);
int allreduce_sum_host(knp_ctx* c, double* host_values, int n);
int interface_accumulate(knp_ctx* c, double* v, int64_t n, int ncol);
int max_abs_diff(knp_ctx* c, const double* a, const double* b, int nsys, double* out);
struct StateBlk {
    int id = 0, kind = 0, type = 0, ncomp = 1;
    int64_t count = 0, width = 1;
    void* dev = nullptr;
    std::vector<char> host;
    void (*apply)(knp_ctx*, int id, const char* data) = nullptr;
};
int fields_state_blocks(knp_ctx* c, std::vector<StateBlk>& out);
int fields_state_prepare_load(knp_ctx* c);
int ode_state_blocks(knp_ctx* c, std::vector<StateBlk>& out);
int rec_state_blocks(knp_ctx* c, std::vector<StateBlk>& out);
void state_destroy(knp_ctx* c);
template <typename T> inline void state_push_host(StateBlk& b, const T* v, int64_t n) {
    b.count = n;
    b.host.assign((const char*)v, (const char*)v + sizeof(T) * (size_t)n);
}

void rec_destroy(knp_ctx* c);
int ode_check_failed(knp_ctx* c);
```

### knp-emi-dg_amd/csrc/krylov.hip

```cpp
#include "krylov_reduce.hpp"
#include <cstdlib>
#include <cstring>

template <int NV> __device__ __forceinline__ void prolong_cell(const int32_t* __restrict__ dg2cg, const double* __restrict__ e,
                                                                int64_t c, double* add, int nil = 1) {
#pragma unroll
    for (int a = 0; a < NV; ++a) add[a] = e[(int64_t)dg2cg[c * NV + a] * nil];
}

#define SYS_PTR(p, s) ((p) + (int64_t)(s) * d.nc * NV)

template <int NV>
__global__ __launch_bounds__(KNP_BLOCK) void k_cg_init(VecDims d, const double* __restrict__ b, const double* __restrict__ w,
                                                       const bjreal* __restrict__ binv, double* __restrict__ r,
                                                       double* __restrict__ z, double* __restrict__ p, double* __restrict__ partial) {
    const int64_t c = (int64_t)blockIdx.x * KNP_BLOCK + threadIdx.x;
    double acc[4] = {0.0, 0.0, 0.0, 0.0};
    if (c < d.nc_owned) {
        double bv[NV], wv[NV], rv[NV], zv[NV], zb[NV];
        ldv<NV>(b, c, bv);
        ldv<NV>(w, c, wv);
#pragma unroll
        for (int a = 0; a < NV; ++a) rv[a] = bv[a] - wv[a];
        block_matvec<NV>(binv, c, rv, zv);
// ... 365 lines not shown
        stv<NV>(SYS_PTR(x, s), c, xv);
        stv<NV>(SYS_PTR(r, s), c, rv);
    }
    write_partials<2>(partial, d.nsys, acc);
}

__global__ __launch_bounds__(KNP_BLOCK) void k_max_abs_diff(int64_t n_owned, int64_t stride, int nsys, const double* __restrict__ a,
                                                            const double* __restrict__ b, double* __restrict__ partial) {
    __shared__ double lds[KNP_BLOCK / 64];
    double v = 0.0;
    for (int s = 0; s < nsys; ++s)
        for (int64_t i = (int64_t)blockIdx.x * KNP_BLOCK + threadIdx.x; i < n_owned; i += (int64_t)gridDim.x * KNP_BLOCK)
            v = fmax(v, fabs(a[s * stride + i] - b[s * stride + i]));
#pragma unroll
    for (int off = 32; off > 0; off >>= 1) v = fmax(v, __shfl_down(v, off, 64));
    if ((threadIdx.x & 63) == 0) lds[threadIdx.x >> 6] = v;
    __syncthreads();
    if (threadIdx.x == 0) {
        for (int w = 1; w < KNP_BLOCK / 64; ++w) v = fmax(v, lds[w]);
        partial[blockIdx.x] = v;
    }
}

int max_abs_diff(knp_ctx* c, const double* a, const double* b, int nsys, double* out) {
    const int nb = 256;
    const int64_t n_owned = c->m.nc_owned * c->nd, stride = c->m.nc * c->nd;
    hipLaunchKernelGGL(k_max_abs_diff, dim3(nb), dim3(KNP_BLOCK), 0, c->stream, n_owned, stride, nsys, a, b, c->partial);
    HIPCHK(c, hipGetLastError());
    std::vector<double> h(nb);
    HIPCHK(c, hipMemcpyAsync(h.data(), c->partial, sizeof(double) * nb, hipMemcpyDeviceToHost, c->stream));
    HIPCHK(c, hipStreamSynchronize(c->stream));
    double m = 0.0;
    for (double v : h) m = v > m ? v : m;
    if (c->dist) {
        int rc = allreduce_max(c, &m);
        if (rc) return rc;
    }
    *out = m;
    return 0;
}


template <typename F> static int dispatch_nd(knp_ctx* c, const char* unsupported, F&& f) {
    switch (c->nd) {
        case 3: return f(std::integral_constant<int, 3>());
        case 4: return f(std::integral_constant<int, 4>());
        case 6: return f(std::integral_constant<int, 6>());
        case 10: return f(std::integral_constant<int, 10>());
    }
    if (unsupported) c->err = unsupported;
    return -1;
}

static int finalize(knp_ctx* c, int op, int nsys, int nred, const StopTest& st, int aux = 0) {
    const int64_t nb = grid_for(c->m.nc_owned);
    double* red = krylov_red(c);
    const int dop = c->dist ? 0 : op;
    const bool deep = nb > 8192;
#define KNP_REDUCE(NR_)                                                                                                                  \
    do {                                                                                                                                 \
        if (deep) hipLaunchKernelGGL((k_reduce<NR_, 8>), dim3(nsys), dim3(KNP_REDUCE_BLOCK), 0, c->stream, c->partial, nb, nsys, red, dop,  \
                                     c->scal, c->status, st, aux);                                                                       \
        else hipLaunchKernelGGL((k_reduce<NR_, 4>), dim3(nsys), dim3(KNP_REDUCE_BLOCK), 0, c->stream, c->partial, nb, nsys, red, dop,       \
                                c->scal, c->status, st, aux);                                                                            \
    } while (0)
    switch (nred) {
        case 1: KNP_REDUCE(1); break;
        case 2: KNP_REDUCE(2); break;
        case 3: KNP_REDUCE(3); break;
        case 4: KNP_REDUCE(4); break;
        case 8: KNP_REDUCE(8); break;
        default: c->err = "finalize: unsupported number of partial sums"; return -1;
    }
#undef KNP_REDUCE
    if (c->dist) {
        int rc = allreduce_red(c, red, nsys * KNP_MAX_RED);
        if (rc) return rc;
        hipLaunchKernelGGL(k_scalar_op, dim3(1), dim3(64), 0, c->stream, op, nsys, red, c->scal, c->status, st, aux);
    }
    HIPCHK(c, hipGetLastError());
    return 0;
}

static int poll_status(knp_ctx* c, int nsys, int* host_status) {
    HIPCHK(c, hipMemcpyAsync(c->pinned, c->status, sizeof(int) * KNP_STATUS_WORDS, hipMemcpyDeviceToHost, c->stream));
    HIPCHK(c, hipStreamSynchronize(c->stream));
    for (int i = 0; i < 2 * nsys; ++i) host_status[i] = ((int*)c->pinned)[i];
    { int bits = ((int*)c->pinned)[KNP_PECLET_SLOT]; float pe; memcpy(&pe, &bits, sizeof(pe)); c->last_peclet = pe; }
    if (((int*)c->pinned)[KNP_ODE_FAIL_SLOT]) {
        hipMemsetAsync(c->status + KNP_ODE_FAIL_SLOT, 0, sizeof(int), c->stream);
        c->err = "ODE integrator did not reach the end time";
        return -4;
    }
    return 0;
}

static int poll_tail() {
    return env_int("KNP_POLL_TAIL", 1);
}
static inline int next_chunk(int it, int maxit, int check_every, int predicted) {
    int chunk = check_every;
    if (predicted > 0) {
        const int ahead = predicted - 1 - it;
        const int tail = poll_tail();
        chunk = ahead > 0 ? (ahead < 4 * check_every ? ahead : 4 * check_every)
                          : (tail > 0 ? tail : (predicted <= 2 ? 1 : 2));
    }
    return (maxit - it < chunk) ? (maxit - it) : chunk;
}

static bool knp_hybrid() {
    static const bool on = env_flag("KNP_HYBRID", true);
    return on;
}
template <bool EMI> static double bj_lmin_frac() {
    static const double v = getenv("KNP_BJ_LMIN") ? atof(getenv("KNP_BJ_LMIN")) : 0.05;
    return v;
}
template <bool EMI> static double bj_theta(const KrylovVecs& kv) { return 0.5 * (1.0 + bj_lmin_frac<EMI>()) * kv.bj_lmax; }

template <int NV, bool EMI>
static int bj_cheb2(knp_ctx* c, const VecDims& d, const KrylovVecs& kv, const double* r, double* y, bool use_status = true,
                    AmgHierarchy* Hfuse = nullptr, double ct_restrict = 0.0) {
    int rc;
    if ((rc = dist_apply(c, EMI ? 0 : 1, y, kv.coef, kv.tmp))) return rc;
    const double lmin_frac = bj_lmin_frac<EMI>();
    const double lmax = kv.bj_lmax, lmin = lmin_frac * lmax;
    const double theta = 0.5 * (lmax + lmin), delta = 0.5 * (lmax - lmin), sigma = theta / delta, rho0 = 1.0 / sigma;
    const double rho1 = 1.0 / (2.0 * sigma - rho0);
    const double cr = (1.0 + rho1 * rho0) / theta + 2.0 * rho1 / delta, ctt = (2.0 * rho1 / delta) / theta;
    const int* st = use_status ? (const int*)c->status : (const int*)nullptr;
    if (Hfuse) {
        AmgHierarchy& H = *Hfuse;
        if ((rc = amg_restrict_tiles_prepare(c, H))) return rc;
        hipLaunchKernelGGL(k_bj_cheb2_restrict<NV>, dim3((unsigned)H.ntiles, (unsigned)d.nsys), dim3(256), sizeof(double) * H.tile_cells * NV,
                           c->stream, d, st, kv.binv, r, (const double*)kv.tmp, y, cr, ctt, H.tile_cells, (const int32_t*)H.tile_off,
                           (const int32_t*)H.slot_ptr, (const uint16_t*)H.slot_idx, H.part, H.nslots, ct_restrict);
        return amg_restrict_finish(c, H);
    }
    const dim3 g((unsigned)grid_for(c->m.nc_owned), (unsigned)d.nsys), b(KNP_BLOCK);
    hipLaunchKernelGGL(k_bj_cheb2<NV>, g, b, 0, c->stream, d, st, kv.binv, r, (const double*)kv.tmp, y, cr, ctt);
    return 0;
}
static bool fuse_restrict(const knp_ctx* c, const KrylovVecs& kv, const AmgHierarchy& H, int nsys) {
    const bool on = env_flag("KNP_FUSE_RESTRICT", true);
    return on && kv.bj_lmax > 0.0 && H.ready && H.ntiles > 0 && H.ncol == nsys && H.tile_cells * c->nd * sizeof(double) <= 65536;
}

static bool fuse_update_restrict(const knp_ctx* c, const AmgHierarchy& H) {
    return env_flag("KNP_FUSE_CG_RESTRICT", true) && H.ready && H.ntiles > 0 && H.ncol == 1 && H.tile_cells * c->nd * sizeof(double) <= 65536;
}

template <int NV, bool EMI>
static int bj_lambda_max_impl(knp_ctx* c, KrylovVecs& kv, int iters, double* out) {
    const int ns = EMI ? 1 : c->p.n_sys;
    if (ns > 4) { *out = 0.0; return 0; }
    VecDims d{c->m.nc_owned, c->m.nc, ns, EMI ? nullptr : kv.bj_idx, EMI ? nullptr : kv.bj_tab, kv.ivol, 0};
    const dim3 g((unsigned)grid_for(c->m.nc_owned), (unsigned)ns), b(KNP_BLOCK);
    const int64_t n_owned = c->m.nc_owned * NV, stride = c->m.nc * NV;
    const dim3 gs((unsigned)((n_owned + 255) / 256), (unsigned)ns);
    int rc;
    HIPCHK(c, hipMemsetAsync(kv.z, 0, sizeof(double) * ns * stride, c->stream));
    HIPCHK(c, hipMemcpyAsync(kv.v, kv.b, sizeof(double) * ns * stride, hipMemcpyDeviceToDevice, c->stream));
    double lam = 0.0, nv = 0.0;
    if ((rc = max_abs_diff(c, kv.v, kv.z, ns, &nv))) return rc;
    if (!(nv > 0.0)) { *out = 0.0; return 0; }
    for (int it = 0; it < iters; ++it) {
        if ((rc = dist_apply(c, EMI ? 0 : 1, kv.v, kv.coef, kv.w))) return rc;
        for (int s = 0; s < ns; ++s)
            hipLaunchKernelGGL(k_bj_apply<NV>, dim3(g.x), b, 0, c->stream, d, (const bjreal*)kv.binv,
                               (const double*)(kv.w + (int64_t)s * stride), kv.y + (int64_t)s * stride, s);
        double ny = 0.0;
        if ((rc = max_abs_diff(c, kv.y, kv.z, ns, &ny))) return rc;
        lam = ny / nv;
        if (!(ny > 0.0)) break;
        const double a = 1.0 / ny;
        hipLaunchKernelGGL(k_scale_sys, gs, dim3(256), 0, c->stream, n_owned, stride, (const double*)kv.y, a, a, a, a, kv.v);
        nv = 1.0;
    }
    *out = lam;
    return 0;
}

int knp_bj_lambda_max(knp_ctx* c, KrylovVecs& kv, int iters, double* out, bool emi) {
    return dispatch_nd(c, nullptr, [&](auto nv) {
        constexpr int NV = decltype(nv)::value;
        return emi ? bj_lambda_max_impl<NV, true>(c, kv, iters, out) : bj_lambda_max_impl<NV, false>(c, kv, iters, out);
    });
}

template <int NV>
static int emi_precondition_residual(knp_ctx* c, const VecDims& d, const KrylovVecs& kv, AmgHierarchy* H) {
    const dim3 g((unsigned)grid_for(c->m.nc_owned)), b(KNP_BLOCK);
    const bool cheb = kv.bj_lmax > 0.0;
    int rc;
    if (H && !cheb && fuse_update_restrict(c, *H)) {
        if ((rc = amg_restrict_tiles_prepare(c, *H))) return rc;
        hipLaunchKernelGGL(k_cg_update_restrict<NV>, dim3((unsigned)H->ntiles), dim3(256), sizeof(double) * H->tile_cells * NV, c->stream, d,
                           c->scal, c->status, kv.p, kv.w, kv.binv, kv.x, kv.r, kv.z, H->tile_cells, (const int32_t*)H->tile_off,
                           (const int32_t*)H->slot_ptr, (const uint16_t*)H->slot_idx, H->part);
        if ((rc = amg_restrict_finish(c, *H))) return rc;
    } else {
        hipLaunchKernelGGL(k_cg_update<NV>, g, b, 0, c->stream, d, c->scal, c->status, kv.p, kv.w, kv.binv, kv.x, kv.r, kv.z, c->partial);
        if (!H) return 0;
        if (fuse_restrict(c, kv, *H, 1)) {
            if ((rc = bj_cheb2<NV, true>(c, d, kv, kv.r, kv.z, true, H, 0.0))) return rc;
        } else {
            if (cheb && (rc = bj_cheb2<NV, true>(c, d, kv, kv.r, kv.z))) return rc;
            if ((rc = amg_restrict_from_dg(c, *H, kv.r))) return rc;
        }
    }
    if ((rc = amg_vcycle(c, *H))) return rc;
    hipLaunchKernelGGL((k_prolong_dot<NV, 3>), g, b, 0, c->stream, d, c->status, 1, H->dg2cg, H->levels[0].x, kv.r, kv.z,
                       (const double*)nullptr, (double*)nullptr, c->partial);
    return 0;
}

template <int NV>
static int pcg_impl(knp_ctx* c, KrylovVecs& kv, double rtol, double atol, int maxit, int check_every, int* niter, double* res) {
    VecDims d{c->m.nc_owned, c->m.nc, 1, nullptr, nullptr, kv.ivol, (kv.d8 && kv.ivol) ? 1 : 0};
    const StopTest stop{rtol, atol, kv.r_abs, 0, d.d8};
    const dim3 g((unsigned)grid_for(c->m.nc_owned)), b(KNP_BLOCK);
    int rc;
    if ((rc = dist_apply(c, 0, kv.x, kv.coef, kv.w))) return rc;
    AmgHierarchy* H = (c->amg.size() && c->amg[0].ready) ? &c->amg[0] : nullptr;
    hipLaunchKernelGGL(k_cg_init<NV>, g, b, 0, c->stream, d, kv.b, kv.w, kv.binv, kv.r, kv.z, kv.p, c->partial);
    if (H) {
        hipLaunchKernelGGL(k_bj_apply<NV>, g, b, 0, c->stream, d, kv.binv, kv.b, kv.y);
        if (kv.bj_lmax > 0.0) {
            if ((rc = bj_cheb2<NV, true>(c, d, kv, kv.b, kv.y, false))) return rc;
            if ((rc = bj_cheb2<NV, true>(c, d, kv, kv.r, kv.z, false))) return rc;
        }
        if ((rc = amg_restrict_from_dg(c, *H, kv.b))) return rc;
        if ((rc = amg_vcycle(c, *H))) return rc;
        HIPCHK(c, hipMemcpyAsync(kv.v, H->levels[0].x, sizeof(double) * H->ncg, hipMemcpyDeviceToDevice, c->stream));
        if ((rc = amg_restrict_from_dg(c, *H, kv.r))) return rc;
        if ((rc = amg_vcycle(c, *H))) return rc;
        hipLaunchKernelGGL((k_prolong_dot<NV, 4>), g, b, 0, c->stream, d, c->status, 0, H->dg2cg, H->levels[0].x, kv.r, kv.z,
                           kv.v, kv.y, c->partial);
        HIPCHK(c, hipMemcpyAsync(kv.p, kv.z, sizeof(double) * c->m.nc * NV, hipMemcpyDeviceToDevice, c->stream));
    }
    if ((rc = finalize(c, OP_CG_INIT, 1, 4, stop))) return rc;
    if (kv.r_abs > 0.0) {
        hipLaunchKernelGGL(k_dot2<NV>, dim3(g.x, 1), b, 0, c->stream, d, kv.x, kv.w, (const double*)nullptr, (const double*)nullptr, c->partial,
                           c->status);
        if ((rc = finalize(c, OP_CG_XA, 1, 1, stop))) return rc;
    }
    int hs[2] = {0, 0};
    int it = 0;
    if ((rc = poll_status(c, 1, hs))) return rc;
    while (!hs[0] && it < maxit) {
        const int chunk = next_chunk(it, maxit, check_every, c->last_it_emi);
        for (int k = 0; k < chunk; ++k) {
            if ((rc = dist_apply(c, 0, kv.p, kv.coef, kv.w))) return rc;
            hipLaunchKernelGGL(k_dot2<NV>, dim3(g.x, 1), b, 0, c->stream, d, kv.p, kv.w, (const double*)nullptr,
                               (const double*)nullptr, c->partial, c->status);
            if ((rc = finalize(c, OP_CG_ALPHA, 1, 1, stop))) return rc;
            if ((rc = emi_precondition_residual<NV>(c, d, kv, H))) return rc;
            if ((rc = finalize(c, OP_CG_BETA, 1, 3, stop))) return rc;
            hipLaunchKernelGGL(k_cg_p<NV>, g, b, 0, c->stream, d, c->scal, c->status, kv.z, kv.p);
        }
        it += chunk;
        if ((rc = poll_status(c, 1, hs))) return rc;
    }
    double hscal[KS_N];
    HIPCHK(c, hipMemcpy(hscal, krylov_scal(c), sizeof(double) * KS_N, hipMemcpyDeviceToHost));
    *niter = hs[1];
    c->last_it_emi = hs[1];
    res[0] = kv.r_abs > 0.0 ? hscal[KS_CG_RN0] : hscal[KS_RES0];
    res[1] = kv.r_abs > 0.0 ? hscal[KS_RNORM] : hscal[KS_RES];
    res[2] = kv.r_abs > 0.0 ? hscal[KS_CG_EST] / sqrt(fmax(fmax(hscal[KS_CG_XA], hscal[KS_CG_SUM]), 1.0e-300)) : hscal[KS_BNORM];
    if (hs[0] == KS_NAN) { c->err = "EMI PCG: NaN residual"; return -4; }
    if (hs[0] != KS_CONVERGED) { c->err = "EMI PCG did not converge"; return -3; }
    return 0;
}

int pcg_solve(knp_ctx* c, KrylovVecs& kv, double rtol, double atol, int maxit, int check_every, int* niter, double* res) {
    if (check_every < 1) check_every = 1;
    return dispatch_nd(c, "pcg: unsupported dofs per cell",
                       [&](auto nv) { return pcg_impl<decltype(nv)::value>(c, kv, rtol, atol, maxit, check_every, niter, res); });
}

template <int NV>
static int knp_coarse_correction(knp_ctx* c, const VecDims& d, const double* in, double* out, const double* t = nullptr, double ct = 0.0,
                                 bool restricted = false) {
    const dim3 g1((unsigned)grid_for(c->m.nc_owned)), b(KNP_BLOCK);
    int active[KNP_MAX_SYS], na = 0;
    for (int s = 0; s < d.nsys; ++s)
        if ((int)c->amg.size() > 1 + s && c->amg[1 + s].ready) active[na++] = s;
    if (!na) return 0;
    int rc;
    if (c->amg[1].ready && c->amg[1].ncol == d.nsys) {
        AmgHierarchy& H = c->amg[1];
        if (!restricted && (rc = amg_restrict_from_dg(c, H, in, nullptr, d.nc * NV, t, ct))) return rc;
        if ((rc = amg_vcycle(c, H))) return rc;
        if (d.nsys % 2 == 0)
            hipLaunchKernelGGL(k_prolong_add_pair<NV>, dim3(g1.x, (unsigned)(d.nsys / 2)), b, 0, c->stream, d, c->status, H.dg2cg,
                               H.levels[0].x, H.ncg, out);
        else
            hipLaunchKernelGGL(k_prolong_add<NV>, dim3(g1.x, (unsigned)d.nsys), b, 0, c->stream, d, c->status, -1, H.dg2cg, H.levels[0].x,
                               H.ncg, out);
        return 0;
    }
    const bool fork = na > 1 && !c->dist && c->amg[1 + active[0]].graph_tried && c->amg[1 + active[0]].graph_exec;
    if (!fork) {
        for (int i = 0; i < na; ++i) {
            const int s = active[i];
            if ((rc = amg_restrict_from_dg(c, c->amg[1 + s], in + (int64_t)s * d.nc * NV, nullptr, 0, t ? t + (int64_t)s * d.nc * NV : nullptr, ct))) return rc;
        }
    } else {
        while ((int)c->aux_streams.size() < na - 1) {
            hipStream_t st; hipEvent_t ev;
            HIPCHK(c, hipStreamCreate(&st));
            HIPCHK(c, hipEventCreateWithFlags(&ev, hipEventDisableTiming));
            c->aux_streams.push_back(st);
            c->aux_events.push_back(ev);
        }
        if (!c->fork_event) HIPCHK(c, hipEventCreateWithFlags(&c->fork_event, hipEventDisableTiming));
        HIPCHK(c, hipEventRecord(c->fork_event, c->stream));
    }
    for (int i = na - 1; i >= 0; --i) {
        const int s = active[i];
        AmgHierarchy& H = c->amg[1 + s];
        hipStream_t st = nullptr;
        if (fork && i > 0 && H.graph_exec) {
            st = c->aux_streams[i - 1];
            HIPCHK(c, hipStreamWaitEvent(st, c->fork_event, 0));
        }
        if (fork && (rc = amg_restrict_from_dg(c, H, in + (int64_t)s * d.nc * NV, st, 0, t ? t + (int64_t)s * d.nc * NV : nullptr, ct))) return rc;
        if ((rc = amg_vcycle(c, H, st))) return rc;
        hipLaunchKernelGGL(k_prolong_add<NV>, g1, b, 0, st ? st : c->stream, d, c->status, s, H.dg2cg, H.levels[0].x, H.ncg,
                           out + (int64_t)s * d.nc * NV);
        if (st) HIPCHK(c, hipEventRecord(c->aux_events[i - 1], st));
    }
    for (int i = 1; i < na; ++i)
        if (fork && c->amg[1 + active[i]].graph_exec) HIPCHK(c, hipStreamWaitEvent(c->stream, c->aux_events[i - 1], 0));
    return 0;
}

template <int NV>
static int knp_precondition(knp_ctx* c, const VecDims& d, const KrylovVecs& kv, const double* in, double* out) {
    int rc;
    const bool hyb = kv.bj_lmax > 0.0 && knp_hybrid();
    const double ct = hyb ? 1.0 / bj_theta<false>(kv) : 0.0;
    const bool fuse = (int)c->amg.size() > 1 && fuse_restrict(c, kv, c->amg[1], d.nsys);
    if (kv.bj_lmax > 0.0 && (rc = bj_cheb2<NV, false>(c, d, kv, in, out, true, fuse ? &c->amg[1] : nullptr, ct))) return rc;
    return knp_coarse_correction<NV>(c, d, in, out, hyb ? kv.tmp : nullptr, ct, fuse);
}

static int knp_solve_epilogue(knp_ctx* c, int ns, const int* hs, int* niter, double* res, const char* method) {
    double hscal[KNP_MAX_SYS * KS_N];
    HIPCHK(c, hipMemcpy(hscal, krylov_scal(c), sizeof(double) * KS_N * ns, hipMemcpyDeviceToHost));
    int bad = 0;
    for (int s = 0; s < ns; ++s) {
        const double* S = scal_row(hscal, s);
        niter[s] = hs[2 * s + 1];
        if (s == 0 || niter[s] > c->last_it_knp) c->last_it_knp = niter[s];
        res[3 * s + 0] = S[KS_RES0];
        res[3 * s + 1] = S[KS_RES];
        res[3 * s + 2] = S[KS_BNORM];
        if (hs[2 * s] != KS_CONVERGED) bad = hs[2 * s] ? hs[2 * s] : -1;
    }
    if (bad) { c->err = std::string("KNP ") + method + " did not converge (status " + std::to_string(bad) + ")"; return -3; }
    return 0;
}

static bool bi_first_form() {
    return env_flag("KNP_FUSE_BI_FIRST", true);
}

template <int NV>
static int bicgstab_impl(knp_ctx* c, KrylovVecs& kv, double rtol, double atol, int maxit, int min_it, int check_every,
                         int* niter, double* res) {
    const int ns = c->p.n_sys;
    VecDims d{c->m.nc_owned, c->m.nc, ns, kv.bj_idx, kv.bj_tab, kv.ivol, (kv.d8 && kv.ivol) ? 1 : 0};
    const StopTest stop{rtol, atol, c->knp_early, min_it, d.d8};
    const dim3 g((unsigned)grid_for(c->m.nc_owned), (unsigned)ns), b(KNP_BLOCK);
    int rc;
    if ((rc = dist_apply(c, 1, kv.x, kv.coef, kv.w))) return rc;
    const bool first_form = bi_first_form();
    if (first_form) hipLaunchKernelGGL((k_bi_init<NV, false>), g, b, 0, c->stream, d, kv.b, kv.w, kv.r, kv.rhat, kv.p, kv.v, c->partial);
    else hipLaunchKernelGGL((k_bi_init<NV, true>), g, b, 0, c->stream, d, kv.b, kv.w, kv.r, kv.rhat, kv.p, kv.v, c->partial);
    if ((rc = finalize(c, OP_BI_INIT, ns, 3, stop))) return rc;
    int hs[2 * KNP_MAX_SYS];
    auto all_done = [&]() { for (int s = 0; s < ns; ++s) if (!hs[2 * s]) return false; return true; };
    if ((rc = poll_status(c, ns, hs))) return rc;
    int it = 0;
    while (!all_done() && it < maxit) {
        const int chunk = next_chunk(it, maxit, check_every, c->last_it_knp);
        for (int k = 0; k < chunk; ++k) {
            if (first_form && it + k == 0)
                hipLaunchKernelGGL((k_bi_p<NV, true>), g, b, 0, c->stream, d, c->scal, c->status, kv.r, kv.v, kv.binv, kv.p, kv.y);
            else
                hipLaunchKernelGGL((k_bi_p<NV, false>), g, b, 0, c->stream, d, c->scal, c->status, kv.r, kv.v, kv.binv, kv.p, kv.y);
            if ((rc = knp_precondition<NV>(c, d, kv, kv.p, kv.y))) return rc;
            if ((rc = dist_apply(c, 1, kv.y, kv.coef, kv.v))) return rc;
            hipLaunchKernelGGL(k_dot2<NV>, g, b, 0, c->stream, d, kv.rhat, kv.v, (const double*)nullptr, (const double*)nullptr,
                               c->partial, c->status);
            if ((rc = finalize(c, OP_BI_ALPHA, ns, 1, stop))) return rc;
            hipLaunchKernelGGL(k_bi_s<NV>, g, b, 0, c->stream, d, c->scal, c->status, kv.v, kv.binv, kv.r, kv.z);
            if ((rc = knp_precondition<NV>(c, d, kv, kv.r, kv.z))) return rc;
            if ((rc = dist_apply(c, 1, kv.z, kv.coef, kv.w))) return rc;
            hipLaunchKernelGGL(k_dot2<NV>, g, b, 0, c->stream, d, kv.w, kv.r, kv.w, kv.w, c->partial, c->status);
            if ((rc = finalize(c, OP_BI_OMEGA, ns, 2, stop))) return rc;
            hipLaunchKernelGGL(k_bi_x<NV>, g, b, 0, c->stream, d, c->scal, c->status, kv.y, kv.z, kv.w, kv.rhat, kv.x, kv.r,
                               c->partial);
            if ((rc = finalize(c, OP_BI_RHO, ns, 2, stop))) return rc;
        }
        it += chunk;
        if ((rc = poll_status(c, ns, hs))) return rc;
    }
    return knp_solve_epilogue(c, ns, hs, niter, res, "BiCGStab");
}


template <int NV>
__global__ __launch_bounds__(KNP_BLOCK) void k_gm_binv(VecDims d, const int* __restrict__ status, const bjreal* __restrict__ binv,
                                                       const double* __restrict__ v, double* __restrict__ y) {
    const int s = blockIdx.y;
    if (status[2 * s]) return;
    const int64_t c = (int64_t)blockIdx.x * KNP_BLOCK + threadIdx.x;
    if (c >= d.nc_owned) return;
    double vv[NV], yv[NV];
    ldv<NV>(SYS_PTR(v, s), c, vv);
    block_matvec<NV>(bj_block<NV>(d, binv, s, c), 0, vv, yv);
    stv<NV>(SYS_PTR(y, s), c, yv);
}

template <int NV>
__global__ __launch_bounds__(KNP_BLOCK) void k_gm_scale_binv(VecDims d, const int* __restrict__ status, const double* __restrict__ scal, int slot,
                                                             const bjreal* __restrict__ binv, double* __restrict__ v, double* __restrict__ y) {
    const int s = blockIdx.y;
    if (status[2 * s]) return;
    const double a = scal_row(scal, s)[slot];
    const int64_t c = (int64_t)blockIdx.x * KNP_BLOCK + threadIdx.x;
    if (c >= d.nc_owned) return;
    double vv[NV], yv[NV];
    ldv<NV>(SYS_PTR(v, s), c, vv);
#pragma unroll
    for (int a_ = 0; a_ < NV; ++a_) vv[a_] *= a;
    block_matvec<NV>(bj_block<NV>(d, binv, s, c), 0, vv, yv);
    stv<NV>(SYS_PTR(v, s), c, vv);
    stv<NV>(SYS_PTR(y, s), c, yv);
}

template <int NV>
__global__ __launch_bounds__(KNP_BLOCK) void k_gm_dots(VecDims d, const int* __restrict__ status, const double* __restrict__ w,
                                                       const double* __restrict__ V, int64_t vstride, int j0, int cnt,
                                                       double* __restrict__ partial) {
    const int s = blockIdx.y;
    const int64_t c = (int64_t)blockIdx.x * KNP_BLOCK + threadIdx.x;
    double acc[8] = {0, 0, 0, 0, 0, 0, 0, 0};
    if (!status[2 * s] && c < d.nc_owned) {
        double wv[NV], vv[NV];
        ldv<NV>(SYS_PTR(w, s), c, wv);
#pragma unroll
        for (int r = 0; r < 8; ++r)
// ... 120 lines not shown
            if ((rc = poll_status(c, ns, hs))) return rc;
        }
        hipLaunchKernelGGL(k_scalar_op, dim3(1), dim3(64), 0, c->stream, (int)OP_GM_SOLVE, ns, (const double*)krylov_red(c), c->scal, c->status,
                           stop, 0);
        hipLaunchKernelGGL(k_gm_lincomb<NV>, g, b, 0, c->stream, d, (const int*)c->status, (const double*)c->scal, (const double*)Z, vstride, kv.x);
        if ((rc = residual(OP_GM_RESTART))) return rc;
        if ((rc = poll_status(c, ns, hs))) return rc;
    }
    return knp_solve_epilogue(c, ns, hs, niter, res, "GMRES");
}

int gmres_solve(knp_ctx* c, KrylovVecs& kv, double rtol, double atol, int maxit, int min_it, int check_every, int* niter, double* res) {
    if (check_every < 1) check_every = 1;
    if (!kv.gm_V || kv.gm_m < 2 || kv.gm_m > KNP_GM_MAX) { c->err = "gmres: no basis storage"; return -1; }
    return dispatch_nd(c, "gmres: unsupported dofs per cell",
                       [&](auto nv) { return gmres_impl<decltype(nv)::value>(c, kv, rtol, atol, maxit, min_it, check_every, niter, res); });
}

template <int NV>
__global__ __launch_bounds__(KNP_BLOCK) void k_load_measure(VecDims d, const double* __restrict__ b, double* __restrict__ partial) {
    const int s = blockIdx.y;
    const int64_t c = (int64_t)blockIdx.x * KNP_BLOCK + threadIdx.x;
    double acc[1] = {0.0};
    if (c < d.nc_owned) {
        double bv[NV], bb = 0.0;
        ldv<NV>(SYS_PTR(b, s), c, bv);
#pragma unroll
        for (int a = 0; a < NV; ++a) bb += bv[a] * bv[a];
        acc[0] = residual_measure(d, c, bb);
    }
    write_partials<1>(partial, d.nsys, acc);
}

int load_measure(knp_ctx* c, const double* b, const float* ivol, bool d8, double* out) {
    const int ns = c->p.n_sys;
    VecDims d{c->m.nc_owned, c->m.nc, ns, nullptr, nullptr, ivol, (d8 && ivol) ? 1 : 0};
    const dim3 g((unsigned)grid_for(c->m.nc_owned), (unsigned)ns), blk(KNP_BLOCK);
    const int rc = dispatch_nd(c, "load_measure: unsupported dofs per cell", [&](auto nv) {
        hipLaunchKernelGGL(k_load_measure<decltype(nv)::value>, g, blk, 0, c->stream, d, b, c->partial);
        return 0;
    });
    if (rc) return rc;
    const int64_t nb = grid_for(c->m.nc_owned);
    double* red = krylov_red(c);
    hipLaunchKernelGGL((k_reduce<1, 8>), dim3(ns), dim3(KNP_REDUCE_BLOCK), 0, c->stream, c->partial, nb, ns, red, 0, c->scal, c->status, StopTest{}, 0);
    HIPCHK(c, hipGetLastError());
    double h[KNP_MAX_SYS * KNP_MAX_RED];
    HIPCHK(c, hipMemcpyAsync(h, red, sizeof(double) * (size_t)ns * KNP_MAX_RED, hipMemcpyDeviceToHost, c->stream));
    HIPCHK(c, hipStreamSynchronize(c->stream));
    for (int s = 0; s < ns; ++s) out[s] = h[s * KNP_MAX_RED];
    return 0;
}

int bicgstab_solve(knp_ctx* c, KrylovVecs& kv, double rtol, double atol, int maxit, int min_it, int check_every, int* niter,
                   double* res) {
    if (check_every < 1) check_every = 1;
    return dispatch_nd(c, "bicgstab: unsupported dofs per cell",
                       [&](auto nv) { return bicgstab_impl<decltype(nv)::value>(c, kv, rtol, atol, maxit, min_it, check_every, niter, res); });
}
```

### knp-emi-dg_amd/csrc/krylov.hpp

```cpp
#pragma once
#include "knpemi_internal.hpp"

enum { KS_RHO = 0, KS_RHO_OLD, KS_ALPHA, KS_BETA, KS_OMEGA, KS_RES, KS_RES0, KS_BNORM, KS_TOL, KS_RNORM, KS_GM_T2, KS_GM_K, KS_N = 12 };
enum { KS_CG_XA = KS_RHO_OLD, KS_CG_EST = KS_OMEGA, KS_CG_SUM = KS_GM_T2, KS_CG_RN0 = KS_GM_K };

#define KNP_GM_MAX 30
struct GmLayout {
    static constexpr int M = KNP_GM_MAX, LDH = M + 1;
    static constexpr int CS = LDH * M, SN = CS + M, G = SN + M, Y = G + M + 1, SIZE = Y + M + 5;
};
template <typename T> struct GmState : GmLayout {
    T* base;
    __host__ __device__ explicit GmState(T* b) : base(b) {}
    __host__ __device__ T& H(int i, int j) const { return base[i + LDH * j]; }
    __host__ __device__ T* cs() const { return base + CS; }
    __host__ __device__ T* sn() const { return base + SN; }
    __host__ __device__ T* g() const { return base + G; }
    __host__ __device__ T* y() const { return base + Y; }
    __host__ __device__ T& cg_log_beta() const { return base[0]; }
};
#define KNP_GM_STRIDE (GmLayout::SIZE)

#define KNP_RED_OFFSET (KNP_MAX_SYS * KS_N)
#define KNP_GM_OFFSET (KNP_RED_OFFSET + KNP_MAX_SYS * KNP_MAX_RED)
#define KNP_SCAL_DOUBLES (KNP_GM_OFFSET + KNP_MAX_SYS * KNP_GM_STRIDE)
static_assert(KNP_GM_STRIDE == 1056 && KNP_GM_OFFSET == KNP_MAX_SYS * (KS_N + KNP_MAX_RED) &&
              KNP_SCAL_DOUBLES == KNP_MAX_SYS * (KS_N + KNP_MAX_RED + GmLayout::SIZE), "regions of knp_ctx::scal");
template <typename T> __host__ __device__ inline T* scal_row(T* scal, int s) { return scal + s * KS_N; }
template <typename T> __host__ __device__ inline T* scal_red(T* scal) { return scal + KNP_RED_OFFSET; }
template <typename T> __host__ __device__ inline T* scal_gm(T* scal, int s) { return scal + KNP_GM_OFFSET + s * KNP_GM_STRIDE; }
inline double* krylov_scal(const knp_ctx* c, int s = 0) { return scal_row(c->scal, s); }
inline double* krylov_red(const knp_ctx* c) { return scal_red(c->scal); }
inline double* krylov_gm(const knp_ctx* c, int s) { return scal_gm(c->scal, s); }

struct KrylovVecs {
    double *x, *b, *coef;
    bjreal* binv;
    const uint16_t* bj_idx = nullptr;
    const bjreal* bj_tab = nullptr;
    double *r, *z, *p, *w;
    double *rhat, *v, *y;
    double* tmp = nullptr;
    double bj_lmax = 0.0;
    const float* ivol = nullptr;
    bool d8 = false;
    double* gm_V = nullptr;
    int gm_m = 0;
    double r_abs = 0.0;
};

struct StopTest {
    double rtol, atol, rabs;
    int min_it, norm8;
};

int load_measure(knp_ctx* c, const double* b, const float* ivol, bool d8, double* out);
int pcg_solve(knp_ctx* c, KrylovVecs& kv, double rtol, double atol, int maxit, int check_every, int* niter, double* res);
int knp_bj_lambda_max(knp_ctx* c, KrylovVecs& kv, int iters, double* out, bool emi = false);
int bicgstab_solve(knp_ctx* c, KrylovVecs& kv, double rtol, double atol, int maxit, int min_it, int check_every, int* niter,
                   double* res);
int gmres_solve(knp_ctx* c, KrylovVecs& kv, double rtol, double atol, int maxit, int min_it, int check_every, int* niter, double* res);
```

### knp-emi-dg_amd/csrc/krylov_reduce.hpp

```cpp
#pragma once
#include "cell_geom.hpp"
#include "krylov_scalar.hpp"

__device__ __forceinline__ double wave_sum(double v) {
#pragma unroll
    for (int off = 32; off > 0; off >>= 1) v += __shfl_down(v, off, 64);
    return v;
}

template <int NR> __device__ __forceinline__ void block_sum(double* v, double* out) {
    __shared__ double lds[KNP_BLOCK / 64][NR];
    const int lane = threadIdx.x & 63, wv = threadIdx.x >> 6;
#pragma unroll
    for (int r = 0; r < NR; ++r) {
        const double s = wave_sum(v[r]);
        if (lane == 0) lds[wv][r] = s;
    }
    __syncthreads();
    if (threadIdx.x == 0) {
#pragma unroll
        for (int r = 0; r < NR; ++r) {
            double s = lds[0][r];
#pragma unroll
            for (int w = 1; w < KNP_BLOCK / 64; ++w) s += lds[w][r];
            out[r] = s;
        }
    }
}

template <int NR> __device__ __forceinline__ void write_partials(double* partial, int nsys, double* v) {
    double out[NR];
    block_sum<NR>(v, out);
    if (threadIdx.x == 0) {
        double* p = partial + ((int64_t)blockIdx.x * nsys + blockIdx.y) * KNP_MAX_RED;
#pragma unroll
        for (int r = 0; r < NR; ++r) p[r] = out[r];
    }
}

template <int NV> __device__ __forceinline__ void ldv(const double* p, int64_t c, double* v) {
    if constexpr (NV <= 4) {
        load_nodal<NV - 1>(p, c, v);
    } else {
        static_assert(NV % 2 == 0, "P2 cell vectors are read as double2");
        const double2* q = reinterpret_cast<const double2*>(p + (int64_t)NV * c);
#pragma unroll
        for (int k = 0; k < NV / 2; ++k) { const double2 t = q[k]; v[2 * k] = t.x; v[2 * k + 1] = t.y; }
    }
}
template <int NV> __device__ __forceinline__ void stv(double* p, int64_t c, const double* v) {
    if constexpr (NV <= 4) {
        store_nodal<NV - 1>(p, c, v);
    } else {
        double2* q = reinterpret_cast<double2*>(p + (int64_t)NV * c);
#pragma unroll
        for (int k = 0; k < NV / 2; ++k) q[k] = make_double2(v[2 * k], v[2 * k + 1]);
    }
}

template <int NV> __device__ __forceinline__ void block_matvec(const bjreal* __restrict__ binv, int64_t c, const double* r, double* z) {
    const bjreal* B = binv + c * NV * NV;
// ... 87 lines not shown
```

### knp-emi-dg_amd/csrc/ring_common.hpp

```cpp
#pragma once
#include "cell_geom.hpp"
#include <algorithm>
#include <map>

namespace ring {

constexpr int RB = 256;
static_assert(RB == KNP_HALO_BLK, "the halo tables are built for 256-cell blocks");

__device__ __forceinline__ void glds16(const void* gsrc, unsigned lds_dst) {
    asm volatile("s_mov_b32 m0, %1\n\ts_nop 0\n\tglobal_load_lds_dwordx4 %0, off" : : "v"(gsrc), "s"(lds_dst) : "memory", "m0");
}
__device__ __forceinline__ void glds16_run4(const void* gsrc, unsigned lds_dst) {
    asm volatile("s_mov_b32 m0, %1\n\ts_nop 0\n\tglobal_load_lds_dwordx4 %0, off\n\tglobal_load_lds_dwordx4 %0, off offset:1024\n\t"
                 "global_load_lds_dwordx4 %0, off offset:2048\n\tglobal_load_lds_dwordx4 %0, off offset:3072"
                 : : "v"(gsrc), "s"(lds_dst) : "memory", "m0");
}
template <int N> __device__ __forceinline__ void wait_vm() { asm volatile("s_waitcnt vmcnt(%0)" : : "n"(N) : "memory"); }
__device__ __forceinline__ void ring_barrier() {
    asm volatile("s_waitcnt lgkmcnt(0)" ::: "memory");
    __builtin_amdgcn_s_barrier();
    asm volatile("" ::: "memory");
}

struct RingWalk {
    int64_t b_lo, first, last, member, members;
    __device__ __forceinline__ explicit RingWalk(const MeshDev& m) {
        b_lo = m.c_begin / RB;
        const int64_t nblk = (m.c_end - 1) / RB - b_lo + 1;
        const int64_t chunk = (nblk + 7) / 8;
        first = (int64_t)(blockIdx.x & 7u) * chunk;
        last = first + chunk < nblk ? first + chunk : nblk;
        member = blockIdx.x >> 3;
        members = gridDim.x >> 3;
    }
    __device__ __forceinline__ int64_t blk(int64_t n) const {
        const int64_t b = first + member + n * members;
        return b < last ? b_lo + b : -1;
    }
};

__device__ __forceinline__ int swz_half(int lane) { return ((lane & 1) ^ ((lane >> 4) & 1)) * 2; }
__device__ __forceinline__ void dma_own_rows(const double* __restrict__ v, int64_t c0, int64_t nc, unsigned dst, int lane) {
    if (c0 + RB <= nc) {
        const double* src = v + (c0 + (lane >> 1)) * 4 + swz_half(lane);
        glds16_run4(src, dst);
        glds16_run4(src + 128 * 4, dst + 4096);
        return;
    }
#pragma unroll
    for (int p = 0; p < 8; ++p) {
        int64_t row = c0 + p * 32 + (lane >> 1);
        row = row < nc ? row : 0;
        glds16(v + row * 4 + swz_half(lane), dst + p * 1024);
    }
}
__device__ __forceinline__ void lds_row(const lds_double* base, unsigned R, double* r) {
    typedef double __attribute__((ext_vector_type(2))) vdouble2;
    typedef __attribute__((address_space(3))) vdouble2 lds_vdouble2;
    const unsigned s = (R >> 3) & 1u;
    const vdouble2 a = *(const lds_vdouble2*)(base + 4 * R + 2 * s);
    const vdouble2 b = *(const lds_vdouble2*)(base + 4 * R + 2 * (s ^ 1u));
    r[0] = a.x; r[1] = a.y; r[2] = b.x; r[3] = b.y;
}
__device__ __forceinline__ int64_t list_cell(const lds_int* L, int e, int hs) {
    const int src = e < hs ? L[e] : -1;
    return src >= 0 ? (int64_t)(src >> 2) : 0;
}

constexpr size_t RING_MAX_LDS = 160 * 1024;
inline int device_cus(int device) {
    static int ncu = 0;
    if (!ncu) {
        hipDeviceProp_t prop;
        ncu = (hipGetDeviceProperties(&prop, device) == hipSuccess && prop.multiProcessorCount > 0) ? prop.multiProcessorCount : 256;
    }
    return ncu;
}

template <typename KernelT> bool grant_lds(KernelT kernel, size_t lds) {
    static std::map<const void*, size_t> granted;
    auto it = granted.find((const void*)kernel);
    if (it != granted.end() && it->second >= lds) return true;
    if (hipFuncSetAttribute((const void*)kernel, hipFuncAttributeMaxDynamicSharedMemorySize, (int)lds) != hipSuccess) return false;
    granted[(const void*)kernel] = lds;
    return true;
}

inline dim3 ring_grid(const MeshDev& m, int device, int reserve_cus) {
    const int64_t nblk = (m.c_end - 1) / RB - m.c_begin / RB + 1;
    const int cus = std::max(device_cus(device) - std::max(reserve_cus, 0), 8);
    int64_t per_xcd = std::max<int64_t>(1, std::min<int64_t>(cus / 8, (nblk + 7) / 8));
    const int wg = env_int("KNP_RING_WG", 0);
    if (wg >= 8) per_xcd = std::min<int64_t>(per_xcd, wg / 8);
    return dim3((unsigned)(8 * per_xcd));
}

}
```

### knp-emi-dg_amd/knpemidg/_abi.py

```python
import ctypes as C
import os

import numpy as np

_HERE = os.path.dirname(os.path.abspath(__file__))
LIB_PATH = os.environ.get("KNP_LIB_PATH") or os.path.join(_HERE, "libknpemi_hip.so")

F_PHI, F_C, F_C_PREV, F_C_ELIM, F_PHI_M, F_I_CH, F_E, F_KAPPA, F_DNPHI, F_B_EMI, F_B_KNP, F_X, F_Y, \
    F_FACET_TMP = range(14)

FACET_TMP_SLOTS = 4
DT_CELLS, DT_NBR, DT_FLAG, DT_CFACET, DT_MF, DT_HB_SRC, DT_HB_LOC, DT_META = range(8)

_f64p = C.POINTER(C.c_double)
_i32p = C.POINTER(C.c_int32)
_i64p = C.POINTER(C.c_int64)
_u32p = C.POINTER(C.c_uint32)
_i8p = C.POINTER(C.c_int8)
_f32p = C.POINTER(C.c_float)
_ctxp = C.c_void_p

SIGNATURES = {
    "knp_ctx_create": (C.c_int, [C.POINTER(_ctxp), C.c_int, C.c_int, C.c_int, C.c_int, C.c_int64, C.c_int64,
                                 C.c_int64, C.c_int64, _f64p, _i32p, _u32p, _i32p, _i8p, _u32p, C.c_int, _u32p]),
    "knp_ctx_destroy": (None, [_ctxp]),
    "knp_last_error": (C.c_char_p, [_ctxp]),
    "knp_set_params": (C.c_int, [_ctxp] + [C.c_double] * 8 + [_f64p, _f64p, _f64p, _f64p, C.c_int]),
    "knp_set_geometry_classes": (C.c_int, [_ctxp, C.c_int, C.POINTER(C.c_uint16), _f64p]),
    "knp_set_tabulation": (C.c_int, [_ctxp, C.c_int, C.c_int, C.c_int, _f64p, _f64p, _f64p]),
    "knp_set_mms": (C.c_int, [_ctxp, _f64p, _f64p, _f64p]),
    "knp_set_source": (C.c_int, [_ctxp, _f64p]),
    "knp_field_size": (C.c_int64, [_ctxp, C.c_int]),
    "knp_debug_table_size": (C.c_int64, [_ctxp, C.c_int]),
    "knp_debug_table": (C.c_int, [_ctxp, C.c_int, C.c_void_p, C.c_int64]),
    "knp_upload": (C.c_int, [_ctxp, C.c_int, _f64p, C.c_int64, C.c_int64]),
    "knp_download": (C.c_int, [_ctxp, C.c_int, _f64p, C.c_int64, C.c_int64]),
    "knp_copy_field": (C.c_int, [_ctxp, C.c_int, C.c_int]),
    "knp_update_kappa": (C.c_int, [_ctxp]),
    "knp_update_dnphi": (C.c_int, [_ctxp]),
    "knp_emi_apply": (C.c_int, [_ctxp, C.c_int, C.c_int]),
    "knp_knp_apply": (C.c_int, [_ctxp, C.c_int, C.c_int]),
    "knp_emi_rhs": (C.c_int, [_ctxp]),
    "knp_knp_rhs": (C.c_int, [_ctxp]),
    "knp_emi_residual_target": (C.c_int, [_ctxp, C.c_double]),
    "knp_knp_load_measure": (C.c_int, [_ctxp, _f64p]),
    "knp_knp_early_stop": (C.c_int, [_ctxp, C.c_double]),
    "knp_emi_solve": (C.c_int, [_ctxp, C.c_double, C.c_double, C.c_int, C.c_int, C.POINTER(C.c_int), _f64p]),
    "knp_knp_solve": (C.c_int, [_ctxp, C.c_double, C.c_double, C.c_int, C.c_int, C.c_int, C.POINTER(C.c_int), _f64p]),
    "knp_set_knp_krylov": (C.c_int, [_ctxp, C.c_int, C.c_int]),
    "knp_set_emi_dg_smoother": (C.c_int, [_ctxp, C.c_int]),
    "knp_step_updates": (C.c_int, [_ctxp]),
    "knp_nernst": (C.c_int, [_ctxp]),
    "knp_picard_updates": (C.c_int, [_ctxp]),
    "knp_max_abs_diff": (C.c_int, [_ctxp, C.c_int, C.c_int, _f64p]),
    "knp_facet_trace": (C.c_int, [_ctxp, C.c_int, C.c_int, C.c_int, C.c_int]),
    "knp_sync": (C.c_int, [_ctxp]),
    "knp_timer_begin": (C.c_int, [_ctxp]),
    "knp_timer_end": (C.c_int, [_ctxp, C.POINTER(C.c_float)]),
    "knp_bench_apply": (C.c_int, [_ctxp, C.c_int, C.c_int, C.POINTER(C.c_float)]),
    "knp_probe_facet_contraction": (C.c_int, [_ctxp, C.c_int, C.c_int64, C.c_int, _f64p, _f64p, C.POINTER(C.c_float)]),
    "knp_apply_timing": (C.c_int, [_ctxp, C.c_int]),
    "knp_apply_timing_read": (C.c_int, [_ctxp, C.c_int, C.POINTER(C.c_float), C.POINTER(C.c_int)]),
    "knp_apply_variant": (C.c_int, [_ctxp, C.c_int]),
    "knp_host_spgemm": (C.c_int, [C.c_int64, C.c_int64, _i32p, _i32p, _f64p, _i32p, _i32p, _f64p, _i32p, C.POINTER(_i32p),
                                  C.POINTER(_f64p), C.c_int]),
    "knp_host_spmv": (C.c_int, [C.c_int64, _i32p, _i32p, _f64p, _f64p, _f64p, C.c_int]),
    "knp_host_free": (None, [C.c_void_p]),
    "knp_host_cell_gram": (C.c_int, [C.c_int64, C.c_int, _f64p, _i32p, _f64p, _f64p, C.c_int]),
    "knp_host_segment_sum": (C.c_int, [C.c_int64, _i64p, _i64p, _f64p, _f64p, C.c_int]),
    "knp_host_build_facets": (C.c_int64, [C.c_int64, C.c_int, _i32p, _i32p, _i32p, _i32p, _i8p]),
    "knp_host_geometry_classes": (C.c_int64, [C.c_int64, _f64p, _i32p, _i32p, _i8p, C.c_double, C.c_int64, _i32p, _i64p, C.c_int]),
    "knp_host_block_pattern": (C.c_int, [C.c_int64, C.c_int, C.c_int64, _i32p, _i64p, _i64p, _i32p, _i32p, _i64p, C.c_int]),
    "knp_comm_unique_id": (C.c_int, [C.c_char_p]),
    "knp_comm_init": (C.c_int, [_ctxp, C.c_int, C.c_int, C.c_char_p]),
    "knp_comm_init_halo": (C.c_int, [_ctxp, C.c_char_p]),
    "knp_comm_init_shm": (C.c_int, [_ctxp, C.c_int, C.c_int, C.c_char_p, C.c_int64, C.c_int64]),
    "knp_set_interior": (C.c_int, [_ctxp, C.c_int64]),
    "knp_halo_tables": (C.c_int, [_ctxp, C.c_int, _i32p, _i64p, _i32p, _i64p, _i64p]),
    "knp_halo_exchange": (C.c_int, [_ctxp, C.c_int]),
    "knp_allreduce_sum": (C.c_int, [_ctxp, _f64p, C.c_int]),
    "knp_ode_create": (C.c_int, [_ctxp, C.c_int, C.c_int64, _i32p, C.c_int, C.c_int, _f64p, _f64p]),
    "knp_ode_table": (C.c_int, [_ctxp, C.c_int, C.c_int, C.c_int, _f64p]),
    "knp_ode_exchange": (C.c_int, [_ctxp, C.c_int, C.c_int, C.c_int, C.c_int, C.c_int64, C.c_int]),
    "knp_ode_exchange_multi": (C.c_int, [_ctxp, C.c_int, C.c_int, _i32p, _i32p, _i32p, _i64p, C.c_int]),
    "knp_ode_set_stimulus": (C.c_int, [_ctxp, C.c_int, C.c_int, _i32p, _f64p, C.POINTER(C.c_uint8)]),
    "knp_ode_step": (C.c_int, [_ctxp, C.c_int, C.c_double, C.c_double, C.c_double, C.c_double]),
    "knp_ode_rtc_compile": (C.c_int, [C.c_char_p, C.c_char_p, C.POINTER(C.c_void_p), C.POINTER(C.c_size_t), C.c_char_p, C.c_size_t]),
    "knp_ode_rtc_free": (None, [C.c_void_p]),
    "knp_ode_register": (C.c_int, [_ctxp, C.c_char_p, C.c_size_t, C.c_char_p, C.c_int, C.c_int]),
    "knp_amg_begin": (C.c_int, [_ctxp, C.c_int, C.c_int64, _i32p, _i32p, _i32p]),
    "knp_amg_columns": (C.c_int, [_ctxp, C.c_int, C.c_int]),
    "knp_amg_level": (C.c_int, [_ctxp, C.c_int, C.c_int64, _i32p, _i32p, _f64p, _f64p, C.c_double, C.c_int, C.c_double,
                                C.c_int64, _i32p, _i32p, _f64p, _i32p, _i32p, _f64p]),
    "knp_amg_finish": (C.c_int, [_ctxp, C.c_int, C.c_int64, _f64p]),
    "knp_amg_finish_f32": (C.c_int, [_ctxp, C.c_int, C.c_int64, _f32p]),
    "knp_host_sym_to_f32": (C.c_int, [C.c_int64, _f64p, _f32p, _f64p, C.c_int]),
    "knp_host_morton_order": (C.c_int, [C.c_int64, C.c_int, _f64p, _i32p, C.c_int, _f64p, _i64p, C.c_int]),
    "knp_host_cell_extent_median": (C.c_int, [C.c_int64, C.c_int, C.c_int, _f64p, _i32p, _f64p]),
    "knp_host_cell_neighbours": (C.c_int, [C.c_int64, C.c_int, _i32p, _i32p, _i8p, _i32p, _i8p, C.c_int]),
    "knp_host_box_marks": (C.c_int, [C.c_int64, C.c_int, _f64p, _i32p, C.c_int, _f64p, _f64p, C.c_double, C.c_int, C.POINTER(C.c_uint8), C.c_int]),
    "knp_host_strength": (C.c_int, [C.c_int64, _i32p, _i32p, _f64p, _f64p, C.c_double, _i32p, C.POINTER(_i32p), C.c_int]),
    "knp_host_smooth_prolongator": (C.c_int, [C.c_int64, C.c_int64, _i32p, _i32p, _f64p, _f64p, _i32p, _i32p, _f64p, _i32p, C.POINTER(_i32p),
                                            C.POINTER(_f64p), C.c_int]),
    "knp_host_truncate_prolongator": (C.c_int, [C.c_int64, _i32p, _i32p, _f64p, C.c_double, _f64p, _i32p, C.POINTER(_i32p), C.POINTER(_f64p), C.c_int]),
    "knp_host_mis2_aggregate": (C.c_int64, [C.c_int64, _i32p, _i32p, _f64p, _i64p, C.c_int]),
    "knp_amg_clear": (C.c_int, [_ctxp, C.c_int]),
    "knp_amg_interface": (C.c_int, [_ctxp, C.c_int64, C.c_int, _i32p, _i64p, _i32p, C.c_int64, _i32p, _i32p, _i32p]),
    "knp_amg_dist0": (C.c_int, [_ctxp, C.c_int]),
    "knp_rec_create": (C.c_int, [_ctxp, C.c_int64, C.c_int64, _i32p, _f64p, C.c_int64, _i64p, _i32p, _f64p, C.c_int, C.POINTER(C.c_uint8), _f64p]),
    "knp_rec_sample": (C.c_int, [_ctxp, C.c_double]),
    "knp_rec_read": (C.c_int, [_ctxp, _i64p, _f64p, _f64p]),
    "knp_rec_channels": (C.c_int64, [_ctxp]),
    "knp_rec_destroy": (C.c_int, [_ctxp]),
    "knp_rec_add_states": (C.c_int, [_ctxp, C.c_int64, _i64p, _i32p, _i64p, _i32p, _f64p]),
    "knp_rec_add_map": (C.c_int, [_ctxp, C.c_int64, _i32p, C.c_double, C.c_double]),
    "knp_rec_map_arm": (C.c_int, [_ctxp, C.c_double]),
# ... 365 lines not shown

    def set_params(self, C_M, dt, F, R, T, C_phi, tau_emi, tau_knp, z, D, rho=None, fsrc=None, splitting=True):
        z = np.ascontiguousarray(z, dtype=np.float64)
        D = np.asarray(D, dtype=np.float64)
        assert z.shape == (self.n_ions,) and D.shape == (self.n_ions, self.nc)
        o = self.cell_order
        D = np.ascontiguousarray(D[:, o])
        rho = None if rho is None else np.ascontiguousarray(np.asarray(rho, dtype=np.float64)[o])
        fsrc = None if fsrc is None else np.ascontiguousarray(np.asarray(fsrc, dtype=np.float64)[:, o])
        self._chk(self.lib.knp_set_params(self.ctx, C_M, dt, F, R, T, C_phi, tau_emi, tau_knp, _p(z, _f64p), _p(D, _f64p),
                                          _p(rho, _f64p), _p(fsrc, _f64p), int(splitting)), "knp_set_params")

    def set_mms(self, C, extra_emi, extra_knp):
        o = self.cell_order
        C_ = np.ascontiguousarray(np.asarray(C, dtype=np.float64)[:, o])
        ee = np.ascontiguousarray(np.asarray(extra_emi, dtype=np.float64).reshape(self.nc, self.nd)[o])
        ek = np.ascontiguousarray(np.asarray(extra_knp, dtype=np.float64).reshape(self.n_sys, self.nc, self.nd)[:, o])
        self._chk(self.lib.knp_set_mms(self.ctx, _p(C_, _f64p), _p(ee, _f64p), _p(ek, _f64p)), "knp_set_mms")

    def set_source(self, src):
        if src is not None:
            src = np.ascontiguousarray(np.asarray(src, dtype=np.float64).reshape(self.n_sys, self.nc, self.nd)[:, self.cell_order])
        self._chk(self.lib.knp_set_source(self.ctx, _p(src, _f64p)), "knp_set_source")

    def size(self, field):
        return int(self.lib.knp_field_size(self.ctx, field))

    _FACET_FIELDS = (F_PHI_M, F_I_CH, F_E, F_FACET_TMP)

    def _nodal_blocks(self, field, offset, count):
        ndof = self.nc * self.nd
        if field in self._FACET_FIELDS:
            return None
        if offset % ndof or count % ndof:
            raise KnpError("nodal field transfers must cover whole [nc*nd] blocks")
        return count // ndof

    def upload(self, field, a, offset=0):
        a = np.ascontiguousarray(a, dtype=np.float64).ravel()
        nb = self._nodal_blocks(field, offset, a.size)
        if nb is not None:
            a = np.ascontiguousarray(a.reshape(nb, self.nc, self.nd)[:, self.cell_order]).ravel()
        self._chk(self.lib.knp_upload(self.ctx, field, _p(a, _f64p), offset, a.size), "knp_upload")

    def download(self, field, offset=0, count=None):
        n = self.size(field) - offset if count is None else count
        out = np.empty(n, dtype=np.float64)
        self._chk(self.lib.knp_download(self.ctx, field, _p(out, _f64p), offset, n), "knp_download")
        nb = self._nodal_blocks(field, offset, n)
        if nb is not None:
            out = np.ascontiguousarray(out.reshape(nb, self.nc, self.nd)[:, self.cell_rank]).ravel()
        return out

    _DT_DTYPE = {0: np.int32, 1: np.int32, 2: np.uint32, 3: np.int32, 4: np.int32, 5: np.int32, 6: np.uint16, 7: np.int64}

    def debug_table(self, which):
        n = int(self.lib.knp_debug_table_size(self.ctx, which))
        if n < 0:
            raise KnpError("unknown debug table %d" % which)
        out = np.zeros(n // np.dtype(self._DT_DTYPE[which]).itemsize, dtype=self._DT_DTYPE[which])
        self._chk(self.lib.knp_debug_table(self.ctx, which, out.ctypes.data_as(C.c_void_p), n), "knp_debug_table")
        return out

    def copy_field(self, dst, src):
        self._chk(self.lib.knp_copy_field(self.ctx, dst, src), "knp_copy_field")

    def update_kappa(self):
        self._chk(self.lib.knp_update_kappa(self.ctx), "knp_update_kappa")

    def update_dnphi(self):
        self._chk(self.lib.knp_update_dnphi(self.ctx), "knp_update_dnphi")

    def emi_apply(self, fx=F_X, fy=F_Y):
        self._chk(self.lib.knp_emi_apply(self.ctx, fx, fy), "knp_emi_apply")

    def knp_apply(self, fx=F_X, fy=F_Y):
        self._chk(self.lib.knp_knp_apply(self.ctx, fx, fy), "knp_knp_apply")

    def emi_rhs(self):
        self._chk(self.lib.knp_emi_rhs(self.ctx), "knp_emi_rhs")

    def knp_rhs(self):
        self._chk(self.lib.knp_knp_rhs(self.ctx), "knp_knp_rhs")

    def emi_residual_target(self, r_abs):
        self._chk(self.lib.knp_emi_residual_target(self.ctx, float(r_abs)), "knp_emi_residual_target")

    def emi_solve(self, rtol, atol=1e-40, maxit=1000, check_every=25):
        it = C.c_int(0)
        res = np.zeros(3)
        rc = self.lib.knp_emi_solve(self.ctx, rtol, atol, maxit, check_every, C.byref(it), _p(res, _f64p))
        self._chk(rc, "knp_emi_solve")
        return it.value, res

    def knp_solve(self, rtol, atol=1e-40, maxit=1000, min_it=5, check_every=10):
        it = (C.c_int * max(self.n_sys, 1))()
        res = np.zeros(3 * self.n_sys)
        rc = self.lib.knp_knp_solve(self.ctx, rtol, atol, maxit, min_it, check_every, it, _p(res, _f64p))
        self._chk(rc, "knp_knp_solve")
        return list(it)[:self.n_sys], res.reshape(self.n_sys, 3)

    def set_knp_krylov(self, method, restart=30):
        code = {"bicgstab": 0, "gmres": 1}[method] if isinstance(method, str) else int(method)
        self._chk(self.lib.knp_set_knp_krylov(self.ctx, code, int(restart)), "knp_set_knp_krylov")

    def set_emi_dg_smoother(self, chebyshev):
        self._chk(self.lib.knp_set_emi_dg_smoother(self.ctx, -1 if chebyshev is None else int(bool(chebyshev))), "knp_set_emi_dg_smoother")

    def step_updates(self):
        self._chk(self.lib.knp_step_updates(self.ctx), "knp_step_updates")

    def picard_updates(self):
        self._chk(self.lib.knp_picard_updates(self.ctx), "knp_picard_updates")

    def max_abs_diff(self, fa, fb):
        out = np.zeros(1)
        self._chk(self.lib.knp_max_abs_diff(self.ctx, fa, fb, _p(out, _f64p)), "knp_max_abs_diff")
        return float(out[0])

    def nernst(self):
        self._chk(self.lib.knp_nernst(self.ctx), "knp_nernst")

    def facet_trace(self, field, species, side, download=True):
        self._tmp_slot = slot = (self._tmp_slot + 1) % FACET_TMP_SLOTS
        if any(f == F_FACET_TMP and off == slot * self.nf for (_, _, _, _, f, off) in self._pending):
            self._flush()
        self._tmp_gen[slot] += 1
        self._chk(self.lib.knp_facet_trace(self.ctx, field, species, side, slot), "knp_facet_trace")
        if download:
            return self.download(F_FACET_TMP, slot * self.nf, self.nf)
        return slot, self._tmp_gen[slot]

    def tmp_slot_valid(self, slot, gen):
        return self._tmp_gen[slot] == gen

    def sync(self):
        self._chk(self.lib.knp_sync(self.ctx), "knp_sync")

    def timer_begin(self):
        self._chk(self.lib.knp_timer_begin(self.ctx), "knp_timer_begin")

    def timer_end(self):
        ms = C.c_float(0)
        self._chk(self.lib.knp_timer_end(self.ctx, C.byref(ms)), "knp_timer_end")
        return ms.value

    def bench_apply(self, which, reps):
        ms = C.c_float(0)
        self._chk(self.lib.knp_bench_apply(self.ctx, which, reps, C.byref(ms)), "knp_bench_apply")
        return ms.value

    def apply_timing(self, enable):
        self._chk(self.lib.knp_apply_timing(self.ctx, int(bool(enable))), "knp_apply_timing")

    def apply_variant(self, which):
        return int(self.lib.knp_apply_variant(self.ctx, which))

    def apply_timing_read(self, which):
        ms, n = C.c_float(0), C.c_int(0)
        self._chk(self.lib.knp_apply_timing_read(self.ctx, which, C.byref(ms), C.byref(n)), "knp_apply_timing_read")
        return ms.value, n.value

    def probe_facet_contraction(self, variant, inputs, reps=20):
        a = np.ascontiguousarray(inputs, dtype=np.float64)
        assert a.ndim == 2 and a.shape[1] == 26
        out = np.empty((a.shape[0], 9))
        ms = C.c_float(0)
        self._chk(self.lib.knp_probe_facet_contraction(self.ctx, int(variant), a.shape[0], int(reps), _p(a, _f64p), _p(out, _f64p),
                                                       C.byref(ms)), "knp_probe_facet_contraction")
        return out, ms.value

    def comm_init(self, rank, nranks, uid, uid_halo=None):
        self._chk(self.lib.knp_comm_init(self.ctx, rank, nranks, uid), "knp_comm_init")
        self.nranks = int(nranks)
        if uid_halo is not None:
            self._chk(self.lib.knp_comm_init_halo(self.ctx, uid_halo), "knp_comm_init_halo")

    def comm_init_shm(self, rank, nranks, name, red_doubles, out_doubles):
        self._chk(self.lib.knp_comm_init_shm(self.ctx, rank, nranks, name.encode(), int(red_doubles), int(out_doubles)), "knp_comm_init_shm")
        self.nranks = int(nranks)

    def set_interior(self, n_interior):
        self._chk(self.lib.knp_set_interior(self.ctx, int(n_interior)), "knp_set_interior")

    def halo_tables(self, peers, send_lists, recv_offsets, recv_counts):
        peers = np.ascontiguousarray(peers, dtype=np.int32)
        sc = np.ascontiguousarray([len(s) for s in send_lists], dtype=np.int64)
        cells = np.concatenate(send_lists) if len(send_lists) else np.zeros(0, dtype=np.int64)
        cells = np.ascontiguousarray(self.cell_rank[np.asarray(cells, dtype=np.int64)], dtype=np.int32)
        ro = np.ascontiguousarray(recv_offsets, dtype=np.int64)
        rcnt = np.ascontiguousarray(recv_counts, dtype=np.int64)
        self._chk(self.lib.knp_halo_tables(self.ctx, len(peers), _p(peers, _i32p), _p(sc, _i64p), _p(cells, _i32p),
                                           _p(ro, _i64p), _p(rcnt, _i64p)), "knp_halo_tables")

    def ode_create(self, model, facets, states, params):
        facets = np.ascontiguousarray(facets, dtype=np.int32)
        states = np.ascontiguousarray(states, dtype=np.float64)
        params = np.ascontiguousarray(params, dtype=np.float64)
        h = self.lib.knp_ode_create(self.ctx, int(model), len(facets), _p(facets, _i32p), states.shape[1], params.shape[1],
                                    _p(states, _f64p), _p(params, _f64p))
        if h < 0:
            self._chk(h, "knp_ode_create")
        return h

    def ode_table(self, handle, what, shape, upload=None):
        a = np.empty(shape, dtype=np.float64) if upload is None else np.ascontiguousarray(upload, dtype=np.float64)
        self._chk(self.lib.knp_ode_table(self.ctx, handle, what, 0 if upload is None else 1, _p(a, _f64p)), "knp_ode_table")
        return a

# ... 153 lines not shown

    def rec_map_arm(self, t0):
        self._chk(self.lib.knp_rec_map_arm(self.ctx, float(t0)), "knp_rec_map_arm")

    def rec_map_read(self):
        n = getattr(self, "_rec_map_n", 0)
        out = [np.empty(n) for _ in range(4)] + [np.empty(n, dtype=np.int32)]
        self._chk(self.lib.knp_rec_map_read(self.ctx, n, *[_p(a, _f64p) for a in out[:4]], _p(out[4], _i32p)), "knp_rec_map_read")
        return tuple(out)

    def rec_destroy(self):
        self._chk(self.lib.knp_rec_destroy(self.ctx), "knp_rec_destroy")

    def state_describe(self):
        from knpemidg.checkpoint import BLOCK_DTYPE
        nbytes = C.c_int64(0)
        n = int(self.lib.knp_state_describe(self.ctx, None, 0, C.byref(nbytes)))
        if n < 0:
            self._chk(n, "knp_state_describe")
        table = np.zeros(n, dtype=BLOCK_DTYPE)
        n2 = int(self.lib.knp_state_describe(self.ctx, table.ctypes.data_as(C.c_void_p), n, C.byref(nbytes)))
        if n2 != n:
            self._chk(n2 if n2 < 0 else -1, "knp_state_describe")
        return table, int(nbytes.value)

    def state_save(self):
        _, nbytes = self.state_describe()
        buf = np.zeros(nbytes, dtype=np.uint8)
        self._chk(self.lib.knp_state_save(self.ctx, buf.ctypes.data_as(C.c_void_p), nbytes), "knp_state_save")
        return buf

    def state_load(self, buf):
        buf = np.ascontiguousarray(buf, dtype=np.uint8)
        self._chk(self.lib.knp_state_load(self.ctx, buf.ctypes.data_as(C.c_void_p), buf.size), "knp_state_load")

    def state_timing(self):
        a, b = C.c_float(0), C.c_float(0)
        self._chk(self.lib.knp_state_timing(self.ctx, C.byref(a), C.byref(b)), "knp_state_timing")
        return a.value, b.value


def _flushing(fn):
    def wrapped(self, *a, **k):
        if self._pending:
            self._flush()
        return fn(self, *a, **k)
    wrapped.__name__, wrapped.__doc__ = fn.__name__, fn.__doc__
    return wrapped


for _name in ("close", "set_params", "set_mms", "upload", "download", "copy_field", "update_kappa", "update_dnphi", "emi_apply",
              "knp_apply", "emi_rhs", "knp_rhs", "emi_solve", "knp_solve", "step_updates", "picard_updates", "max_abs_diff",
              "nernst", "sync", "timer_begin", "timer_end", "bench_apply", "ode_table", "ode_step", "ode_set_stimulus",
              "amg_upload", "amg_interface", "halo_exchange", "knp_load_measure", "apply_timing_read", "comm_init", "set_interior", "rec_sample",
              "rec_read", "rec_add_states", "rec_map_arm", "rec_map_read", "state_save", "state_load"):
    setattr(Device, _name, _flushing(getattr(Device, _name)))


def comm_unique_id():
    buf = C.create_string_buffer(128)
    if load().knp_comm_unique_id(buf) != 0:
        raise KnpError("knp_comm_unique_id failed")
    return buf.raw
```

Measured before the change: 2.490 billion DoF/s.

## Fuse Krylov dot products into ring matrix-free apply kernels

Adds a templated DOT path to the ring EMI and KNP apply kernels so each wave accumulates y·a (and optionally y·y) right after storing y, writing per-wave partials into the reduction buffer. BiCGStab then skips the separate k_dot2 pass when the fused path is available. This removes a full re-read of y and a, plus one kernel launch, per apply. The status words and Krylov scalars now share one allocation, likely so a single readback can poll both. In exchange it adds register pressure and extra global loads inside the apply kernels, and the partial buffer is sized for the ring grid.

```diff
diff --git a/include/knpemi_hip.h b/include/knpemi_hip.h
--- a/include/knpemi_hip.h
+++ b/include/knpemi_hip.h
@@ -73,7 +73,8 @@
     KNP_DT_MF = 4,
     KNP_DT_HB_SRC = 5,
     KNP_DT_HB_LOC = 6,
-    KNP_DT_META = 7
+    KNP_DT_META = 7,
+    KNP_DT_KRYLOV_SCAL = 8
 };
 int64_t knp_debug_table_size(knp_ctx* ctx, int which);
 int knp_debug_table(knp_ctx* ctx, int which, void* out, int64_t nbytes);
@@ -190,6 +191,9 @@
 
 int knp_apply_variant(knp_ctx* ctx, int which);
 
+int64_t knp_fused_dot_count(knp_ctx* ctx);
+int knp_debug_apply_dot(knp_ctx* ctx, int which, int field_x, int field_y, int field_a, int with_yy, double* out);
+
 int knp_probe_facet_contraction(knp_ctx* ctx, int variant, int64_t ncol, int reps, const double* in, double* out, float* avg_ms);
 
 int knp_comm_unique_id(char* out128);
diff --git a/knp-emi-dg_amd/csrc/abi.hip b/knp-emi-dg_amd/csrc/abi.hip
--- a/knp-emi-dg_amd/csrc/abi.hip
+++ b/knp-emi-dg_amd/csrc/abi.hip
@@ -328,11 +328,12 @@
     for (auto pp : wk) rc |= dev_zeros(c, pp, ns * ndof);
     rc |= dev_zeros(c, &c->D, (size_t)n_ions * nc);
     rc |= dev_zeros(c, &c->rho, nc);
-    c->partial_blocks = grid_for(nc_owned) + 8;
+    c->partial_blocks = std::max<int64_t>(grid_for(nc_owned) + 8, ring_dot_rows_max(c->device));
     rc |= dev_zeros(c, &c->partial, (size_t)c->partial_blocks * KNP_MAX_SYS * KNP_MAX_RED);
-    rc |= dev_zeros(c, &c->scal, KNP_SCAL_DOUBLES);
-    if (!rc && hipMalloc((void**)&c->status, sizeof(int) * KNP_STATUS_WORDS) != hipSuccess) rc = -2;
-    if (!rc) hipMemset(c->status, 0, sizeof(int) * KNP_STATUS_WORDS);
+    double* poll_block = nullptr;
+    rc |= dev_zeros(c, &poll_block, KNP_STATUS_DOUBLES + KNP_SCAL_DOUBLES);
+    c->status = reinterpret_cast<int*>(poll_block);
+    c->scal = poll_block ? poll_block + KNP_STATUS_DOUBLES : nullptr;
     if (!rc && hipHostMalloc(&c->pinned, 4096) != hipSuccess) rc = -2;
     if (rc) { g_err = "device allocation failed: " + c->err; delete fl; delete c; return -2; }
     if (dev_alloc_copy(c, &fl->ivol, ivol.data(), ivol.size())) { g_err = "device allocation failed: " + c->err; delete fl; delete c; return -2; }
@@ -367,7 +368,7 @@
     hipFree(c->m.hb_src); hipFree(c->m.hb_loc);
     hipFree(c->m.cls); hipFree(c->m.cls_table); hipFree(c->m.cls_ext); hipFree(c->m.coords); hipFree(c->m.h); hipFree(c->m.cells); hipFree(c->m.nbr); hipFree(c->m.fflag); hipFree(c->m.cfacet); hipFree(c->m.mf);
     hipFree(c->mat); hipFree(c->nmat4); hipFree(c->dtab); hipFree(c->halo_ctr);
-    hipFree(c->D); hipFree(c->rho); hipFree(c->fsrc); hipFree(c->mms_C); hipFree(c->extra_emi); hipFree(c->extra_knp); hipFree(c->partial); hipFree(c->scal); hipFree(c->status); hipFree(c->gm_V);
+    hipFree(c->D); hipFree(c->rho); hipFree(c->fsrc); hipFree(c->mms_C); hipFree(c->extra_emi); hipFree(c->extra_knp); hipFree(c->partial); hipFree(c->status); hipFree(c->gm_V);
     hipFree(c->halo_send_idx); hipFree(c->halo_sendbuf);
     if (c->pinned) hipHostFree(c->pinned);
     if (c->ev0) hipEventDestroy(c->ev0);
@@ -564,6 +565,7 @@
         case KNP_DT_HB_SRC: *p = m.hb_src; return m.hb_src ? nblk * m.hb_stride * 4 : 0;
         case KNP_DT_HB_LOC: *p = m.hb_loc; return m.hb_loc ? m.nc_owned * 4 * 2 : 0;
         case KNP_DT_META: *p = nullptr; return 8 * 8;
+        case KNP_DT_KRYLOV_SCAL: *p = c->scal; return (int64_t)KNP_MAX_SYS * KS_N * 8;
         default: return -1;
     }
 }
@@ -676,6 +678,16 @@
     if (chk_vec(c, fx, fy, (int64_t)c->p.n_sys * c->m.nc * c->nd)) return -1;
     Fields* f = F(c);
     return dist_apply(c, 1, f->f[fx], f->f[KNP_F_DNPHI], f->f[fy]);
+}
+
+int64_t knp_fused_dot_count(knp_ctx* c) { return c ? c->fused_dots : -1; }
+
+int knp_debug_apply_dot(knp_ctx* c, int which, int fx, int fy, int fa, int with_yy, double* out) {
+    if (!c || !out || (which != 0 && which != 1)) return -1;
+    const int64_t need = (int64_t)(which == 0 ? 1 : c->p.n_sys) * c->m.nc * c->nd;
+    if (chk_vec(c, fx, fy, need) || chk_vec(c, fa, fy, need)) return -1;
+    Fields* f = F(c);
+    return debug_apply_dot(c, which, f->f[fx], f->f[which == 0 ? KNP_F_KAPPA : KNP_F_DNPHI], f->f[fy], f->f[fa], with_yy != 0, out);
 }
 
 int knp_emi_rhs(knp_ctx* c) {
diff --git a/knp-emi-dg_amd/csrc/apply_p1.hip b/knp-emi-dg_amd/csrc/apply_p1.hip
--- a/knp-emi-dg_amd/csrc/apply_p1.hip
+++ b/knp-emi-dg_amd/csrc/apply_p1.hip
@@ -118,6 +118,22 @@
     return 0;
 }
 
+int launch_apply_dot(knp_ctx* c, int which, const double* x, const double* coef, double* y, const double* a, bool with_yy, int64_t* rows, double* partial) {
+    *rows = 0;
+    if (c->degree != 1 || c->m.c_end - c->m.c_begin <= 0) return 0;
+    if (!plan_fused_dot(plan_apply(apply_inputs(c, which), which), c->m.c_begin, c->m.c_end)) return 0;
+    const int reserve = halo_reserve_cus(c);
+    const int64_t n = fused_dot_rows(which, ring_workgroups(c, c->m, reserve), c->partial_blocks);
+    if (!n) return 0;
+    const RingDot dot{a, partial, which == 0 ? 1 : c->p.n_sys, with_yy ? 1 : 0};
+    ApplyTimerScope t(c, which);
+    const int rc = which == 0 ? ring_emi_apply(c, c->m, x, coef, y, reserve, &dot) : ring_knp_apply(c, c->m, x, coef, y, make_knp_args(c), reserve, &dot);
+    if (rc) return rc;
+    ++c->fused_dots;
+    *rows = n;
+    return 0;
+}
+
 int launch_emi_blockjacobi(knp_ctx* c, const double* kappa, bjreal* binv) {
     if (c->degree != 1) return p2_assembled(c) ? tab_block_inverse(c, 0, binv) : p2_block_inverse(c, 0, kappa, binv);
     const double shift = 0.0;
diff --git a/knp-emi-dg_amd/csrc/apply_plan.hpp b/knp-emi-dg_amd/csrc/apply_plan.hpp
--- a/knp-emi-dg_amd/csrc/apply_plan.hpp
+++ b/knp-emi-dg_amd/csrc/apply_plan.hpp
@@ -56,3 +56,13 @@
     if (begin < end) seg[n++] = {p.tail, begin, end};
     return n;
 }
+
+inline bool plan_fused_dot(const ApplyPlan& p, int64_t begin, int64_t end) {
+    ApplySegment seg[2];
+    return begin == 0 && apply_segments(p, begin, end, seg) == 1 && (seg[0].family == AF_RING_KNP || seg[0].family == AF_RING_EMI);
+}
+constexpr int FUSED_DOT_WAVES[2] = {8, 4};
+inline int64_t fused_dot_rows(int which, int64_t workgroups, int64_t capacity) {
+    const int64_t rows = workgroups * FUSED_DOT_WAVES[which];
+    return rows > 0 && rows <= capacity ? rows : 0;
+}
diff --git a/knp-emi-dg_amd/csrc/apply_ring.hip b/knp-emi-dg_amd/csrc/apply_ring.hip
--- a/knp-emi-dg_amd/csrc/apply_ring.hip
+++ b/knp-emi-dg_amd/csrc/apply_ring.hip
@@ -1,5 +1,6 @@
 #include "cell_geom.hpp"
 #include "ring_common.hpp"
+#include "apply_plan.hpp"
 #include <algorithm>
 #include <cstdlib>
 #include <map>
@@ -117,10 +118,11 @@
     return q;
 }
 
-template <int NS, int NG>
+template <int NS, int NG, bool DOT>
 __global__ __launch_bounds__(RB * NG + 64 * RLOADERS) void k_knp_apply_ring(MeshDev m, const double* __restrict__ x, const double* __restrict__ gphi,
                                                                  double* __restrict__ yout, KnpArgs ka, const uint8_t* __restrict__ mat,
-                                                                 const uint8_t* __restrict__ nmat4, const double* __restrict__ dtab, int dbg) {
+                                                                 const uint8_t* __restrict__ nmat4, const double* __restrict__ dtab, int dbg,
+                                                                 RingDotArg<DOT> dot) {
     typedef KnpRing<NS> R;
     constexpr int NV = 4, KS = NS / NG, NTHREADS = RB * NG + 64 * RLOADERS;
     static_assert(KS * NG == NS, "species split evenly over the consumer groups");
@@ -133,7 +135,17 @@
     const int wave = __builtin_amdgcn_readfirstlane((int)(threadIdx.x >> 6));
     const int lane = threadIdx.x & 63;
     const RingWalk w(m);
-    if (w.blk(0) < 0) return;
+    double dsum[KS][2];
+#pragma unroll
+    for (int k = 0; k < KS; ++k) dsum[k][0] = dsum[k][1] = 0.0;
+    if (w.blk(0) < 0) {
+        if constexpr (DOT) {
+            if (wave < 4 * NG)
+#pragma unroll
+                for (int k = 0; k < KS; ++k) ring_dot_write(dot, (int64_t)blockIdx.x * 4 + (wave & 3), (wave >> 2) * KS + k, dsum[k]);
+        }
+        return;
+    }
     for (int i = threadIdx.x; i < m.ncls * 11; i += NTHREADS) s_cls[(i / 11) * RCLS + (i % 11)] = m.cls_table[(i / 11) * KNP_CLS_STRIDE + (i % 11)];
     for (int i = threadIdx.x; i < m.ncls * KNP_CLS_EXT; i += NTHREADS) s_cls[(i / KNP_CLS_EXT) * RCLS + 11 + (i % KNP_CLS_EXT)] = m.cls_ext[i];
     if (threadIdx.x < NS * KNP_MAX_MAT) s_D[threadIdx.x] = dtab[threadIdx.x];
@@ -211,6 +223,11 @@
         if (b < 0) break;
         const int64_t c = b * RB + t;
         if (c >= m.c_begin && c < m.c_end) {
+            double av[KS][NV];
+            if constexpr (DOT) {
+#pragma unroll
+                for (int k = 0; k < KS; ++k) load_nodal<3>(dot.a + (int64_t)(k0 + k) * m.nc * NV, c, av[k]);
+            }
             const char* slot = smem + (n % RSLOTS) * R::SLOT;
             const CellMeta cur = read_meta(slot + R::META0, t, true);
             const lds_double* X = (const lds_double*)slot + k0 * (RENT * NV);
@@ -255,8 +272,16 @@
             }
 #pragma unroll
             for (int k = 0; k < KS; ++k) store_nodal<3>(yout + (int64_t)(k0 + k) * m.nc * NV, c, y[k]);
+            if constexpr (DOT) {
+#pragma unroll
+                for (int k = 0; k < KS; ++k) ring_dot_add(y[k], av[k], dot.with_yy, dsum[k]);
+            }
         }
         ring_barrier();
+    }
+    if constexpr (DOT) {
+#pragma unroll
+        for (int k = 0; k < KS; ++k) ring_dot_write(dot, (int64_t)blockIdx.x * 4 + (wave & 3), k0 + k, dsum[k]);
     }
 }
 
@@ -333,8 +358,9 @@
 }
 
 constexpr int EMI_SLOTS = 4;
+template <bool DOT>
 __global__ __launch_bounds__(2 * RB + 64 * RLOADERS) void k_emi_apply_ring(MeshDev m, const double* __restrict__ x, const double* __restrict__ kappa,
-                                                                double* __restrict__ yout, double C_phi, double tau) {
+                                                                double* __restrict__ yout, double C_phi, double tau, RingDotArg<DOT> dot) {
     typedef EmiRing R;
     constexpr int NV = 4, NTHREADS = 2 * RB + 64 * RLOADERS;
     extern __shared__ __attribute__((aligned(16))) char smem[];
@@ -345,7 +371,13 @@
     const int wave = __builtin_amdgcn_readfirstlane((int)(threadIdx.x >> 6));
     const int lane = threadIdx.x & 63;
     const RingWalk w(m);
-    if (w.blk(0) < 0) return;
+    double dsum[2] = {0.0, 0.0};
+    if (w.blk(0) < 0) {
+        if constexpr (DOT) {
+            if (wave < 8) ring_dot_write(dot, (int64_t)blockIdx.x * 8 + wave, 0, dsum);
+        }
+        return;
+    }
     for (int i = threadIdx.x; i < m.ncls * 11; i += NTHREADS) s_cls[(i / 11) * RCLS + (i % 11)] = m.cls_table[(i / 11) * KNP_CLS_STRIDE + (i % 11)];
     for (int i = threadIdx.x; i < m.ncls * KNP_CLS_EXT; i += NTHREADS) s_cls[(i / KNP_CLS_EXT) * RCLS + 11 + (i % KNP_CLS_EXT)] = m.cls_ext[i];
     if (wave >= 8) {
@@ -399,7 +431,7 @@
     ring_barrier();
     ring_barrier();
     CellGeom<3> K;
-    double xv[NV], kv[NV], yv[NV], gx[NV];
+    double xv[NV], kv[NV], yv[NV], gx[NV], av[NV];
     const lds_double *X = nullptr, *KA = nullptr, *ft = nullptr;
     CellMeta cur;
     cur.flags = 0; cur.lw = make_uint2(0u, 0u); cur.cls = 0; cur.nm = 0; cur.mymat = 0;
@@ -412,6 +444,7 @@
                 ccur = b * RB + t;
                 valid = ccur >= m.c_begin && ccur < m.c_end;
                 if (valid) {
+                    if constexpr (DOT) load_nodal<3>(dot.a, ccur, av);
                     const char* slot = smem + (n & (EMI_SLOTS - 1)) * R::SLOT;
                     cur = read_meta(slot + R::META0, t, false);
                     X = (const lds_double*)slot;
@@ -441,10 +474,12 @@
             emi_facet_ring<2>(K, cur.flags, cur.lw.y & 0xffffu, xv, gx, kv, C_phi, tau, X, KA, ft, yv);
             emi_facet_ring<3>(K, cur.flags, cur.lw.y >> 16, xv, gx, kv, C_phi, tau, X, KA, ft, yv);
             store_nodal<3>(yout, ccur, yv);
+            if constexpr (DOT) ring_dot_add(yv, av, dot.with_yy, dsum);
         }
         ring_barrier();
         if (b < 0) break;
     }
+    if constexpr (DOT) ring_dot_write(dot, (int64_t)blockIdx.x * 8 + wave, 0, dsum);
 }
 
 }
@@ -463,29 +498,46 @@
     return c->nmat > 0 && c->p.n_sys <= 2 && env_int("KNP_APPLY_MAT", 1) != 0 && env_int("KNP_APPLY_HALO", 1) != 0;
 }
 
-int ring_emi_apply(knp_ctx* c, const MeshDev& m, const double* x, const double* kappa, double* y, int reserve_cus) {
+int64_t ring_workgroups(const knp_ctx* c, const MeshDev& m, int reserve_cus) { return (int64_t)ring_grid(m, c->device, reserve_cus).x; }
+
+static_assert(FUSED_DOT_WAVES[0] == 8 && FUSED_DOT_WAVES[1] == 4, "rows the fused kernels write per workgroup: 8 blockIdx.x + wave (EMI), 4 blockIdx.x + (wave & 3) (KNP)");
+int ring_dot_rows_max(int device) { return std::max(device_cus(device), 8) * 8; }
+
+int ring_emi_apply(knp_ctx* c, const MeshDev& m, const double* x, const double* kappa, double* y, int reserve_cus, const RingDot* dot) {
     const size_t lds = ring_lds_bytes(c, 0);
-    if (!grant_lds(k_emi_apply_ring, lds)) { c->err = "hipFuncSetAttribute(k_emi_apply_ring) failed"; return -2; }
-    hipLaunchKernelGGL(k_emi_apply_ring, ring_grid(m, c->device, reserve_cus), dim3(2 * RB + 64 * RLOADERS), lds, c->stream, m, x, kappa, y, c->p.C_phi, c->p.tau_emi);
+    const dim3 g = ring_grid(m, c->device, reserve_cus), b(2 * RB + 64 * RLOADERS);
+    if (dot) {
+        if (!grant_lds(k_emi_apply_ring<true>, lds)) { c->err = "hipFuncSetAttribute(k_emi_apply_ring) failed"; return -2; }
+        hipLaunchKernelGGL(k_emi_apply_ring<true>, g, b, lds, c->stream, m, x, kappa, y, c->p.C_phi, c->p.tau_emi, *dot);
+    } else {
+        if (!grant_lds(k_emi_apply_ring<false>, lds)) { c->err = "hipFuncSetAttribute(k_emi_apply_ring) failed"; return -2; }
+        hipLaunchKernelGGL(k_emi_apply_ring<false>, g, b, lds, c->stream, m, x, kappa, y, c->p.C_phi, c->p.tau_emi, RingNoDot{});
+    }
     HIPCHK(c, hipGetLastError());
     return 0;
 }
 
-int ring_knp_apply(knp_ctx* c, const MeshDev& m, const double* x, const double* gphi, double* y, const KnpArgs& ka, int reserve_cus) {
+int ring_knp_apply(knp_ctx* c, const MeshDev& m, const double* x, const double* gphi, double* y, const KnpArgs& ka, int reserve_cus, const RingDot* dot) {
     const int ns = c->p.n_sys;
     const size_t lds = ring_lds_bytes(c, 1);
     const dim3 g = ring_grid(m, c->device, reserve_cus);
     const bool split = ns == 2 && env_int("KNP_RING_SPLIT", 0) != 0;
+#define RING_KNP_LAUNCH_(NS_, NG_, DOT_, ARG_)                                                                                        \
+    do {                                                                                                                              \
+        if (!grant_lds(k_knp_apply_ring<NS_, NG_, DOT_>, lds)) { c->err = "hipFuncSetAttribute(k_knp_apply_ring) failed"; return -2; }  \
+        hipLaunchKernelGGL((k_knp_apply_ring<NS_, NG_, DOT_>), g, dim3(RB * NG_ + 64 * RLOADERS), lds, c->stream, m, x, gphi, y, ka, (const uint8_t*)c->mat,  \
+                           (const uint8_t*)c->nmat4, (const double*)c->dtab, env_int("KNP_RING_DEBUG", 0), ARG_);               \
+    } while (0)
 #define RING_KNP_LAUNCH(NS_, NG_)                                                                                                     \
     do {                                                                                                                              \
-        if (!grant_lds(k_knp_apply_ring<NS_, NG_>, lds)) { c->err = "hipFuncSetAttribute(k_knp_apply_ring) failed"; return -2; }  \
-        hipLaunchKernelGGL((k_knp_apply_ring<NS_, NG_>), g, dim3(RB * NG_ + 64 * RLOADERS), lds, c->stream, m, x, gphi, y, ka, (const uint8_t*)c->mat,  \
-                           (const uint8_t*)c->nmat4, (const double*)c->dtab, env_int("KNP_RING_DEBUG", 0));                     \
+        if (dot) RING_KNP_LAUNCH_(NS_, NG_, true, *dot);                                                                              \
+        else RING_KNP_LAUNCH_(NS_, NG_, false, RingNoDot{});                                                                          \
     } while (0)
     if (ns == 1) RING_KNP_LAUNCH(1, 1);
     else if (split) RING_KNP_LAUNCH(2, 2);
     else RING_KNP_LAUNCH(2, 1);
 #undef RING_KNP_LAUNCH
+#undef RING_KNP_LAUNCH_
     HIPCHK(c, hipGetLastError());
     return 0;
 }
diff --git a/knp-emi-dg_amd/csrc/cell_geom.hpp b/knp-emi-dg_amd/csrc/cell_geom.hpp
--- a/knp-emi-dg_amd/csrc/cell_geom.hpp
+++ b/knp-emi-dg_amd/csrc/cell_geom.hpp
@@ -18,6 +18,12 @@
     h = fma(h, e, h);
     g = fma(fma(-g, g, x), h, g);
     return g;
+}
+
+__device__ __forceinline__ double wave_sum(double v) {
+#pragma unroll
+    for (int off = 32; off > 0; off >>= 1) v += __shfl_down(v, off, 64);
+    return v;
 }
 
 template <int D> struct CellGeom {
diff --git a/knp-emi-dg_amd/csrc/comm.hip b/knp-emi-dg_amd/csrc/comm.hip
--- a/knp-emi-dg_amd/csrc/comm.hip
+++ b/knp-emi-dg_amd/csrc/comm.hip
@@ -343,6 +343,16 @@
     return rc;
 }
 
+int dist_apply_dot(knp_ctx* c, int which, double* x, const double* coef, double* y, const double* a, bool with_yy, int64_t* rows, double* partial) {
+    *rows = 0;
+    const char* fs = getenv("KNP_FORCE_SPLIT");
+    if (!c->dist && !(fs && atoi(fs) == 1)) {
+        const int rc = launch_apply_dot(c, which, x, coef, y, a, with_yy, rows, partial ? partial : c->partial);
+        if (rc || *rows) return rc;
+    }
+    return dist_apply(c, which, x, coef, y);
+}
+
 static int halo_exchange_on(knp_ctx* c, double* v, int nfields, hipStream_t st, ncclComm_t comm) {
     if (nfields > KNP_MAX_SYS) { c->err = "halo exchange: too many fields"; return -1; }
     const int NV = c->nd;
diff --git a/knp-emi-dg_amd/csrc/knpemi_internal.hpp b/knp-emi-dg_amd/csrc/knpemi_internal.hpp
--- a/knp-emi-dg_amd/csrc/knpemi_internal.hpp
+++ b/knp-emi-dg_amd/csrc/knpemi_internal.hpp
@@ -139,6 +139,7 @@
     int32_t* if_aptr = nullptr;
     int32_t* if_asrc = nullptr;
     double *if_send = nullptr, *if_recv = nullptr;
+    int64_t fused_dots = 0;
     bool time_applies = false;
     std::vector<std::pair<hipEvent_t, hipEvent_t>> tev[2];
     size_t tev_used[2] = {0, 0};
@@ -158,6 +159,11 @@
     int ns;
     double inv_dt, psi, tau;
     double z[KNP_MAX_SYS];
+};
+struct RingDot {
+    const double* a;
+    double* partial;
+    int nsys, with_yy;
 };
 template <int D> struct FacetConst;
 template <> struct FacetConst<3> { static constexpr double mass = 1.0 / 12.0, trip = 1.0 / 60.0; };
@@ -220,8 +226,11 @@
 void ring_u_free(knp_ctx* c);
 int ring_u_emi_apply(knp_ctx* c, const MeshDev& m, const double* x, const double* kappa, double* y, int reserve_cus);
 int ring_u_knp_apply(knp_ctx* c, const MeshDev& m, const double* x, const double* gphi, double* y, const KnpArgs& ka, int reserve_cus);
-int ring_emi_apply(knp_ctx* c, const MeshDev& m, const double* x, const double* kappa, double* y, int reserve_cus);
-int ring_knp_apply(knp_ctx* c, const MeshDev& m, const double* x, const double* gphi, double* y, const KnpArgs& ka, int reserve_cus);
+int ring_emi_apply(knp_ctx* c, const MeshDev& m, const double* x, const double* kappa, double* y, int reserve_cus, const RingDot* dot = nullptr);
+int ring_knp_apply(knp_ctx* c, const MeshDev& m, const double* x, const double* gphi, double* y, const KnpArgs& ka, int reserve_cus,
+                   const RingDot* dot = nullptr);
+int64_t ring_workgroups(const knp_ctx* c, const MeshDev& m, int reserve_cus);
+int ring_dot_rows_max(int device);
 
 int p2_emi_apply(knp_ctx* c, const double* x, const double* kappa, double* y);
 int p2_knp_apply(knp_ctx* c, const double* x, const double* phi, double* y);
@@ -229,6 +238,11 @@
 
 int halo_exchange(knp_ctx* c, double* v, int nfields);
 int dist_apply(knp_ctx* c, int which, double* x, const double* coef, double* y);
+int dist_apply_dot(knp_ctx* c, int which, double* x, const double* coef, double* y, const double* a, bool with_yy, int64_t* rows,
+                   double* partial = nullptr);
+int launch_apply_dot(knp_ctx* c, int which, const double* x, const double* coef, double* y, const double* a, bool with_yy, int64_t* rows,
+                     double* partial);
+int debug_apply_dot(knp_ctx* c, int which, double* x, const double* coef, double* y, const double* a, bool with_yy, double* out);
 
 int launch_nernst_only(knp_ctx* c, const double* cc, const double* celim, double* E);
 void comm_destroy(knp_ctx* c);
diff --git a/knp-emi-dg_amd/csrc/krylov.hip b/knp-emi-dg_amd/csrc/krylov.hip
--- a/knp-emi-dg_amd/csrc/krylov.hip
+++ b/knp-emi-dg_amd/csrc/krylov.hip
@@ -441,16 +441,17 @@
     return -1;
 }
 
-static int finalize(knp_ctx* c, int op, int nsys, int nred, const StopTest& st, int aux = 0) {
-    const int64_t nb = grid_for(c->m.nc_owned);
+static int finalize(knp_ctx* c, int op, int nsys, int nred, const StopTest& st, int aux = 0, int64_t rows = 0, const double* partial = nullptr) {
+    const int64_t nb = rows > 0 ? rows : grid_for(c->m.nc_owned);
+    if (!partial) partial = c->partial;
     double* red = krylov_red(c);
     const int dop = c->dist ? 0 : op;
     const bool deep = nb > 8192;
 #define KNP_REDUCE(NR_)                                                                                                                  \
     do {                                                                                                                                 \
-        if (deep) hipLaunchKernelGGL((k_reduce<NR_, 8>), dim3(nsys), dim3(KNP_REDUCE_BLOCK), 0, c->stream, c->partial, nb, nsys, red, dop,  \
+        if (deep) hipLaunchKernelGGL((k_reduce<NR_, 8>), dim3(nsys), dim3(KNP_REDUCE_BLOCK), 0, c->stream, partial, nb, nsys, red, dop,     \
                                      c->scal, c->status, st, aux);                                                                       \
-        else hipLaunchKernelGGL((k_reduce<NR_, 4>), dim3(nsys), dim3(KNP_REDUCE_BLOCK), 0, c->stream, c->partial, nb, nsys, red, dop,       \
+        else hipLaunchKernelGGL((k_reduce<NR_, 4>), dim3(nsys), dim3(KNP_REDUCE_BLOCK), 0, c->stream, partial, nb, nsys, red, dop,          \
                                 c->scal, c->status, st, aux);                                                                            \
     } while (0)
     switch (nred) {
@@ -471,8 +472,13 @@
     return 0;
 }
 
+constexpr size_t POLL_SCAL_OFFSET = sizeof(double) * KNP_STATUS_DOUBLES;
+static_assert(POLL_SCAL_OFFSET + sizeof(double) * KS_N * KNP_MAX_SYS <= 4096, "regions of knp_ctx::pinned");
+static const double* polled_scalars(const knp_ctx* c) { return (const double*)((const char*)c->pinned + POLL_SCAL_OFFSET); }
+
 static int poll_status(knp_ctx* c, int nsys, int* host_status) {
-    HIPCHK(c, hipMemcpyAsync(c->pinned, c->status, sizeof(int) * KNP_STATUS_WORDS, hipMemcpyDeviceToHost, c->stream));
+    if ((const void*)krylov_scal(c) != (const void*)(c->status + KNP_STATUS_WORDS)) { c->err = "poll_status: scalars not behind the status words"; return -1; }
+    HIPCHK(c, hipMemcpyAsync(c->pinned, c->status, POLL_SCAL_OFFSET + sizeof(double) * KS_N * nsys, hipMemcpyDeviceToHost, c->stream));
     HIPCHK(c, hipStreamSynchronize(c->stream));
     for (int i = 0; i < 2 * nsys; ++i) host_status[i] = ((int*)c->pinned)[i];
     { int bits = ((int*)c->pinned)[KNP_PECLET_SLOT]; float pe; memcpy(&pe, &bits, sizeof(pe)); c->last_peclet = pe; }
@@ -578,6 +584,13 @@
     });
 }
 
+static int apply_dot(knp_ctx* c, int which, double* x, const double* coef, double* y, const double* a, bool with_yy, int64_t* rows,
+                     double* partial = nullptr) {
+    *rows = 0;
+    if (!a || !env_flag("KNP_FUSE_APPLY_DOT", true)) return dist_apply(c, which, x, coef, y);
+    return dist_apply_dot(c, which, x, coef, y, a, with_yy, rows, partial);
+}
+
 template <int NV>
 static int emi_precondition_residual(knp_ctx* c, const VecDims& d, const KrylovVecs& kv, AmgHierarchy* H) {
     const dim3 g((unsigned)grid_for(c->m.nc_owned)), b(KNP_BLOCK);
@@ -611,7 +624,9 @@
     const StopTest stop{rtol, atol, kv.r_abs, 0, d.d8};
     const dim3 g((unsigned)grid_for(c->m.nc_owned)), b(KNP_BLOCK);
     int rc;
-    if ((rc = dist_apply(c, 0, kv.x, kv.coef, kv.w))) return rc;
+    double* xa_partial = c->partial + c->partial_blocks * KNP_MAX_RED;
+    int64_t xa_rows = 0, rows = 0;
+    if ((rc = apply_dot(c, 0, kv.x, kv.coef, kv.w, kv.r_abs > 0.0 ? kv.x : nullptr, false, &xa_rows, xa_partial))) return rc;
     AmgHierarchy* H = (c->amg.size() && c->amg[0].ready) ? &c->amg[0] : nullptr;
     hipLaunchKernelGGL(k_cg_init<NV>, g, b, 0, c->stream, d, kv.b, kv.w, kv.binv, kv.r, kv.z, kv.p, c->partial);
     if (H) {
@@ -631,9 +646,10 @@
     }
     if ((rc = finalize(c, OP_CG_INIT, 1, 4, stop))) return rc;
     if (kv.r_abs > 0.0) {
-        hipLaunchKernelGGL(k_dot2<NV>, dim3(g.x, 1), b, 0, c->stream, d, kv.x, kv.w, (const double*)nullptr, (const double*)nullptr, c->partial,
-                           c->status);
-        if ((rc = finalize(c, OP_CG_XA, 1, 1, stop))) return rc;
+        if (!xa_rows)
+            hipLaunchKernelGGL(k_dot2<NV>, dim3(g.x, 1), b, 0, c->stream, d, kv.x, kv.w, (const double*)nullptr, (const double*)nullptr, c->partial,
+                               c->status);
+        if ((rc = finalize(c, OP_CG_XA, 1, 1, stop, 0, xa_rows, xa_rows ? xa_partial : nullptr))) return rc;
     }
     int hs[2] = {0, 0};
     int it = 0;
@@ -641,10 +657,11 @@
     while (!hs[0] && it < maxit) {
         const int chunk = next_chunk(it, maxit, check_every, c->last_it_emi);
         for (int k = 0; k < chunk; ++k) {
-            if ((rc = dist_apply(c, 0, kv.p, kv.coef, kv.w))) return rc;
-            hipLaunchKernelGGL(k_dot2<NV>, dim3(g.x, 1), b, 0, c->stream, d, kv.p, kv.w, (const double*)nullptr,
-                               (const double*)nullptr, c->partial, c->status);
-            if ((rc = finalize(c, OP_CG_ALPHA, 1, 1, stop))) return rc;
+            if ((rc = apply_dot(c, 0, kv.p, kv.coef, kv.w, kv.p, false, &rows))) return rc;
+            if (!rows)
+                hipLaunchKernelGGL(k_dot2<NV>, dim3(g.x, 1), b, 0, c->stream, d, kv.p, kv.w, (const double*)nullptr,
+                                   (const double*)nullptr, c->partial, c->status);
+            if ((rc = finalize(c, OP_CG_ALPHA, 1, 1, stop, 0, rows))) return rc;
             if ((rc = emi_precondition_residual<NV>(c, d, kv, H))) return rc;
             if ((rc = finalize(c, OP_CG_BETA, 1, 3, stop))) return rc;
             hipLaunchKernelGGL(k_cg_p<NV>, g, b, 0, c->stream, d, c->scal, c->status, kv.z, kv.p);
@@ -652,8 +669,7 @@
         it += chunk;
         if ((rc = poll_status(c, 1, hs))) return rc;
     }
-    double hscal[KS_N];
-    HIPCHK(c, hipMemcpy(hscal, krylov_scal(c), sizeof(double) * KS_N, hipMemcpyDeviceToHost));
+    const double* hscal = polled_scalars(c);
     *niter = hs[1];
     c->last_it_emi = hs[1];
     res[0] = kv.r_abs > 0.0 ? hscal[KS_CG_RN0] : hscal[KS_RES0];
@@ -738,8 +754,7 @@
 }
 
 static int knp_solve_epilogue(knp_ctx* c, int ns, const int* hs, int* niter, double* res, const char* method) {
-    double hscal[KNP_MAX_SYS * KS_N];
-    HIPCHK(c, hipMemcpy(hscal, krylov_scal(c), sizeof(double) * KS_N * ns, hipMemcpyDeviceToHost));
+    const double* hscal = polled_scalars(c);
     int bad = 0;
     for (int s = 0; s < ns; ++s) {
         const double* S = scal_row(hscal, s);
@@ -772,6 +787,7 @@
     else hipLaunchKernelGGL((k_bi_init<NV, true>), g, b, 0, c->stream, d, kv.b, kv.w, kv.r, kv.rhat, kv.p, kv.v, c->partial);
     if ((rc = finalize(c, OP_BI_INIT, ns, 3, stop))) return rc;
     int hs[2 * KNP_MAX_SYS];
+    int64_t rows = 0;
     auto all_done = [&]() { for (int s = 0; s < ns; ++s) if (!hs[2 * s]) return false; return true; };
     if ((rc = poll_status(c, ns, hs))) return rc;
     int it = 0;
@@ -783,15 +799,16 @@
             else
                 hipLaunchKernelGGL((k_bi_p<NV, false>), g, b, 0, c->stream, d, c->scal, c->status, kv.r, kv.v, kv.binv, kv.p, kv.y);
             if ((rc = knp_precondition<NV>(c, d, kv, kv.p, kv.y))) return rc;
-            if ((rc = dist_apply(c, 1, kv.y, kv.coef, kv.v))) return rc;
-            hipLaunchKernelGGL(k_dot2<NV>, g, b, 0, c->stream, d, kv.rhat, kv.v, (const double*)nullptr, (const double*)nullptr,
-                               c->partial, c->status);
-            if ((rc = finalize(c, OP_BI_ALPHA, ns, 1, stop))) return rc;
+            if ((rc = apply_dot(c, 1, kv.y, kv.coef, kv.v, kv.rhat, false, &rows))) return rc;
+            if (!rows)
+                hipLaunchKernelGGL(k_dot2<NV>, g, b, 0, c->stream, d, kv.rhat, kv.v, (const double*)nullptr, (const double*)nullptr,
+                                   c->partial, c->status);
+            if ((rc = finalize(c, OP_BI_ALPHA, ns, 1, stop, 0, rows))) return rc;
             hipLaunchKernelGGL(k_bi_s<NV>, g, b, 0, c->stream, d, c->scal, c->status, kv.v, kv.binv, kv.r, kv.z);
             if ((rc = knp_precondition<NV>(c, d, kv, kv.r, kv.z))) return rc;
-            if ((rc = dist_apply(c, 1, kv.z, kv.coef, kv.w))) return rc;
-            hipLaunchKernelGGL(k_dot2<NV>, g, b, 0, c->stream, d, kv.w, kv.r, kv.w, kv.w, c->partial, c->status);
-            if ((rc = finalize(c, OP_BI_OMEGA, ns, 2, stop))) return rc;
+            if ((rc = apply_dot(c, 1, kv.z, kv.coef, kv.w, kv.r, true, &rows))) return rc;
+            if (!rows) hipLaunchKernelGGL(k_dot2<NV>, g, b, 0, c->stream, d, kv.w, kv.r, kv.w, kv.w, c->partial, c->status);
+            if ((rc = finalize(c, OP_BI_OMEGA, ns, 2, stop, 0, rows))) return rc;
             hipLaunchKernelGGL(k_bi_x<NV>, g, b, 0, c->stream, d, c->scal, c->status, kv.y, kv.z, kv.w, kv.rhat, kv.x, kv.r,
                                c->partial);
             if ((rc = finalize(c, OP_BI_RHO, ns, 2, stop))) return rc;
@@ -1018,6 +1035,30 @@
     return 0;
 }
 
+int debug_apply_dot(knp_ctx* c, int which, double* x, const double* coef, double* y, const double* a, bool with_yy, double* out) {
+    const int ns = which == 0 ? 1 : c->p.n_sys;
+    return dispatch_nd(c, "apply_dot: unsupported dofs per cell", [&](auto nv) {
+        constexpr int NV = decltype(nv)::value;
+        VecDims d{c->m.nc_owned, c->m.nc, ns, nullptr, nullptr, nullptr, 0};
+        int64_t rows = 0;
+        int rc;
+        HIPCHK(c, hipMemsetAsync(c->status, 0, sizeof(int) * 2 * ns, c->stream));
+        if ((rc = dist_apply_dot(c, which, x, coef, y, a, with_yy, &rows))) return rc;
+        if (!rows)
+            hipLaunchKernelGGL(k_dot2<NV>, dim3((unsigned)grid_for(c->m.nc_owned), (unsigned)ns), dim3(KNP_BLOCK), 0, c->stream, d, (const double*)y, a,
+                               with_yy ? (const double*)y : (const double*)nullptr, with_yy ? (const double*)y : (const double*)nullptr, c->partial,
+                               (const int*)c->status);
+        if ((rc = finalize(c, OP_SUM_ONLY, ns, 2, StopTest{}, 0, rows))) return rc;
+        double h[KNP_MAX_SYS * KNP_MAX_RED];
+        HIPCHK(c, hipMemcpyAsync(h, krylov_red(c), sizeof(double) * (size_t)ns * KNP_MAX_RED, hipMemcpyDeviceToHost, c->stream));
+        HIPCHK(c, hipStreamSynchronize(c->stream));
+        out[0] = (double)rows;
+        out[1] = (double)c->partial_blocks;
+        for (int s = 0; s < ns; ++s) { out[2 + 2 * s] = h[s * KNP_MAX_RED]; out[3 + 2 * s] = with_yy ? h[s * KNP_MAX_RED + 1] : 0.0; }
+        return 0;
+    });
+}
+
 int bicgstab_solve(knp_ctx* c, KrylovVecs& kv, double rtol, double atol, int maxit, int min_it, int check_every, int* niter,
                    double* res) {
     if (check_every < 1) check_every = 1;
diff --git a/knp-emi-dg_amd/csrc/krylov.hpp b/knp-emi-dg_amd/csrc/krylov.hpp
--- a/knp-emi-dg_amd/csrc/krylov.hpp
+++ b/knp-emi-dg_amd/csrc/krylov.hpp
@@ -21,6 +21,8 @@
 };
 #define KNP_GM_STRIDE (GmLayout::SIZE)
 
+#define KNP_STATUS_DOUBLES (KNP_STATUS_WORDS / 2)
+static_assert(KNP_STATUS_WORDS % 2 == 0, "the scalars behind the status words are 8-byte aligned");
 #define KNP_RED_OFFSET (KNP_MAX_SYS * KS_N)
 #define KNP_GM_OFFSET (KNP_RED_OFFSET + KNP_MAX_SYS * KNP_MAX_RED)
 #define KNP_SCAL_DOUBLES (KNP_GM_OFFSET + KNP_MAX_SYS * KNP_GM_STRIDE)
diff --git a/knp-emi-dg_amd/csrc/krylov_reduce.hpp b/knp-emi-dg_amd/csrc/krylov_reduce.hpp
--- a/knp-emi-dg_amd/csrc/krylov_reduce.hpp
+++ b/knp-emi-dg_amd/csrc/krylov_reduce.hpp
@@ -1,12 +1,6 @@
 #pragma once
 #include "cell_geom.hpp"
 #include "krylov_scalar.hpp"
-
-__device__ __forceinline__ double wave_sum(double v) {
-#pragma unroll
-    for (int off = 32; off > 0; off >>= 1) v += __shfl_down(v, off, 64);
-    return v;
-}
 
 template <int NR> __device__ __forceinline__ void block_sum(double* v, double* out) {
     __shared__ double lds[KNP_BLOCK / 64][NR];
diff --git a/knp-emi-dg_amd/csrc/ring_common.hpp b/knp-emi-dg_amd/csrc/ring_common.hpp
--- a/knp-emi-dg_amd/csrc/ring_common.hpp
+++ b/knp-emi-dg_amd/csrc/ring_common.hpp
@@ -68,6 +68,29 @@
     return src >= 0 ? (int64_t)(src >> 2) : 0;
 }
 
+struct RingNoDot {};
+template <bool DOT> using RingDotArg = typename std::conditional<DOT, RingDot, RingNoDot>::type;
+
+__device__ __forceinline__ void ring_dot_add(const double* y, const double* a, int with_yy, double* sum) {
+    double ya = 0.0, yy = 0.0;
+#pragma unroll
+    for (int k = 0; k < 4; ++k) ya += y[k] * a[k];
+    sum[0] += ya;
+    if (with_yy) {
+#pragma unroll
+        for (int k = 0; k < 4; ++k) yy += y[k] * y[k];
+        sum[1] += yy;
+    }
+}
+__device__ __forceinline__ void ring_dot_write(const RingDot& d, int64_t row, int s, const double* sum) {
+    const double ya = wave_sum(sum[0]), yy = wave_sum(sum[1]);
+    if ((threadIdx.x & 63) == 0) {
+        double* p = d.partial + (row * d.nsys + s) * KNP_MAX_RED;
+        p[0] = ya;
+        p[1] = yy;
+    }
+}
+
 constexpr size_t RING_MAX_LDS = 160 * 1024;
 inline int device_cus(int device) {
     static int ncu = 0;
diff --git a/knp-emi-dg_amd/knpemidg/_abi.py b/knp-emi-dg_amd/knpemidg/_abi.py
--- a/knp-emi-dg_amd/knpemidg/_abi.py
+++ b/knp-emi-dg_amd/knpemidg/_abi.py
@@ -10,7 +10,7 @@
     F_FACET_TMP = range(14)
 
 FACET_TMP_SLOTS = 4
-DT_CELLS, DT_NBR, DT_FLAG, DT_CFACET, DT_MF, DT_HB_SRC, DT_HB_LOC, DT_META = range(8)
+DT_CELLS, DT_NBR, DT_FLAG, DT_CFACET, DT_MF, DT_HB_SRC, DT_HB_LOC, DT_META, DT_KRYLOV_SCAL = range(9)
 
 _f64p = C.POINTER(C.c_double)
 _i32p = C.POINTER(C.c_int32)
@@ -62,6 +62,8 @@
     "knp_apply_timing": (C.c_int, [_ctxp, C.c_int]),
     "knp_apply_timing_read": (C.c_int, [_ctxp, C.c_int, C.POINTER(C.c_float), C.POINTER(C.c_int)]),
     "knp_apply_variant": (C.c_int, [_ctxp, C.c_int]),
+    "knp_fused_dot_count": (C.c_int64, [_ctxp]),
+    "knp_debug_apply_dot": (C.c_int, [_ctxp, C.c_int, C.c_int, C.c_int, C.c_int, C.c_int, _f64p]),
     "knp_host_spgemm": (C.c_int, [C.c_int64, C.c_int64, _i32p, _i32p, _f64p, _i32p, _i32p, _f64p, _i32p, C.POINTER(_i32p),
                                   C.POINTER(_f64p), C.c_int]),
     "knp_host_spmv": (C.c_int, [C.c_int64, _i32p, _i32p, _f64p, _f64p, _f64p, C.c_int]),
@@ -533,7 +535,7 @@
             out = np.ascontiguousarray(out.reshape(nb, self.nc, self.nd)[:, self.cell_rank]).ravel()
         return out
 
-    _DT_DTYPE = {0: np.int32, 1: np.int32, 2: np.uint32, 3: np.int32, 4: np.int32, 5: np.int32, 6: np.uint16, 7: np.int64}
+    _DT_DTYPE = {0: np.int32, 1: np.int32, 2: np.uint32, 3: np.int32, 4: np.int32, 5: np.int32, 6: np.uint16, 7: np.int64, 8: np.float64}
 
     def debug_table(self, which):
         n = int(self.lib.knp_debug_table_size(self.ctx, which))
@@ -636,6 +638,15 @@
 
     def apply_variant(self, which):
         return int(self.lib.knp_apply_variant(self.ctx, which))
+
+    def fused_dot_count(self):
+        return int(self.lib.knp_fused_dot_count(self.ctx))
+
+    def debug_apply_dot(self, which, fx, fy, fa, with_yy):
+        out = np.zeros(16)
+        self._chk(self.lib.knp_debug_apply_dot(self.ctx, which, fx, fy, fa, int(bool(with_yy)), _p(out, _f64p)), "knp_debug_apply_dot")
+        ns = 1 if which == 0 else self.n_sys
+        return int(out[0]), int(out[1]), out[2:2 + 2 * ns:2].copy(), out[3:3 + 2 * ns:2].copy()
 
     def apply_timing_read(self, which):
         ms, n = C.c_float(0), C.c_int(0)
@@ -895,7 +906,7 @@
 for _name in ("close", "set_params", "set_mms", "upload", "download", "copy_field", "update_kappa", "update_dnphi", "emi_apply",
               "knp_apply", "emi_rhs", "knp_rhs", "emi_solve", "knp_solve", "step_updates", "picard_updates", "max_abs_diff",
               "nernst", "sync", "timer_begin", "timer_end", "bench_apply", "ode_table", "ode_step", "ode_set_stimulus",
-              "amg_upload", "amg_interface", "halo_exchange", "knp_load_measure", "apply_timing_read", "comm_init", "set_interior", "rec_sample",
+              "amg_upload", "amg_interface", "halo_exchange", "knp_load_measure", "apply_timing_read", "debug_apply_dot", "comm_init", "set_interior", "rec_sample",
               "rec_read", "rec_add_states", "rec_map_arm", "rec_map_read", "state_save", "state_load"):
     setattr(Device, _name, _flushing(getattr(Device, _name)))
 
```

After: 2.472 billion DoF/s. About the same (-0.7%).
